# hwaranlee/kaldi-cnn

Measured on AMD Instinct MI355X. Metric: frames/sec fwd+bwd, Conv+Maxpool+FC stack, 4096-frame batch @1/2/4/8 GPU, higher is better.
Workload: dtype f32; 1 GPU; c2: Conv(40x11x3, 8x1, 128) -> Maxpool(1x1x4) -> FC(11616->1024), fwd+bwd+update; frames_per_gpu=4096, parallelism=dp1, global_batch=4096, conv_maxpool_fusion=True, conv_output_stored=False

## Files before the change

### experiments/fc_shapes.py

```python
import os, sys
ROOT = os.path.dirname(os.path.dirname(os.path.abspath(__file__)))
sys.path.insert(0, os.path.join(ROOT, "kaldi-cnn_amd"))
import torch
import kcnn

SHAPES = [("fwd", 4096, 1024, 11616, False, True),
          ("dgrad", 4096, 11616, 1024, False, False),
          ("wgrad", 1024, 11616, 4096, True, False)]


def main():
    calls = int(sys.argv[1]) if len(sys.argv) > 1 else 20
    kcnn.init(0)
    kcnn.set_gemm_mode(2)
    g = torch.Generator(device="cuda").manual_seed(5)
    for name, m, n, k, ta, tb in SHAPES:
        a = torch.randn((k, m) if ta else (m, k), device="cuda", generator=g)
        b = torch.randn((n, k) if tb else (k, n), device="cuda", generator=g) * 0.01
        c = torch.zeros(m, n, device="cuda")
        for _ in range(3):
            kcnn.gemm(a, b, c, ta, tb)
        torch.cuda.synchronize()
        e0, e1 = torch.cuda.Event(enable_timing=True), torch.cuda.Event(enable_timing=True)
        e0.record()
        for _ in range(calls):
            kcnn.gemm(a, b, c, ta, tb)
        e1.record()
        torch.cuda.synchronize()
        us = e0.elapsed_time(e1) * 1e3 / calls
        print(f"{name} {m}x{n}x{k}: {us:.1f} us per call, "
              f"{2 * m * n * k / us / 1e6:.1f} TFLOP/s", flush=True)


if __name__ == "__main__":
    main()
```

### include/kcnn.h

```cpp
#ifndef KCNN_KCNN_H_
#define KCNN_KCNN_H_

#include <stddef.h>
#include <stdint.h>

#include "cnsl-hip-kernels.h"

#ifdef __cplusplus
extern "C" {
#endif

const char *kcnn_last_error(void);
const char *kcnn_version(void);
unsigned long long kcnn_device_malloc_calls(void);
int kcnn_conv_fix_counts(unsigned long long *out, int reset);
int kcnn_init(int device);
int kcnn_set_stream(kcnn_stream_t stream);
int kcnn_synchronize(void);
int kcnn_set_literal_path(int literal);
int kcnn_set_profiling(int on);
int kcnn_set_fusion(int mode);
int kcnn_set_gemm_mode(int mode);
int kcnn_set_kernel_family(const char *name, int value);
int kcnn_get_kernel_family(const char *name);
int kcnn_gemm(int trans_a, int trans_b, int m, int n, int k, float alpha,
              const float *a, int lda, const float *b, int ldb, float beta,
              float *c, int ldc);
int kcnn_split_planes(const float *src, int rows, int cols, int ld, uint16_t *dst, int ldp,
                      int64_t ps);
int kcnn_gemm_planes(int trans_a, int trans_b, int m, int n, int k, float alpha,
                     const uint16_t *a, int lda, int64_t aps, const uint16_t *b, int ldb,
                     int64_t bps, float beta, float *c, int ldc);
int kcnn_profile_string(char *buf, size_t len);
int kcnn_reset_profile(void);
void kcnn_set_randn_seed(uint64_t seed);
int kcnn_selftest_fastdiv(void);

int kcnn_mat_conv2d(const float *in, MatrixDim in_dim, const float *kernel,
                    MatrixDim kernel_dim, int in_height, int in_width,
                    int in_channel, int kernel_height, int kernel_width,
                    int group, float *out, MatrixDim out_dim, int concat);
int kcnn_mat_add_mat_rep_vec(float *m, MatrixDim dim, const float *vec,
                             int vec_dim, int rep);
int kcnn_mat_flip_mat(const float *m, MatrixDim dim, int kernel_height,
                      int kernel_width, int in_channel, int group, float *flip,
                      MatrixDim flip_dim);
int kcnn_mat_padding_zero(const float *m, MatrixDim dim, int orig_height,
                          int orig_width, int orig_channel, int kernel_height,
                          int kernel_width, float *padmat, MatrixDim pad_dim);
int kcnn_mat_tp_block(const float *m, MatrixDim dim, int in_channel,
                      int block_size, float *out, MatrixDim out_dim);
int kcnn_mat_tp_inside_block(const float *m, MatrixDim dim, int group,
                             int block_size, float *out, MatrixDim out_dim);
int kcnn_mat_mod_permute_row(const float *m, MatrixDim dim, int in_channel,
                             int block_size, float *out, MatrixDim out_dim);
int kcnn_mat_mod_permute_channel(float *comp, MatrixDim dim, int comp_idx,
                                 int num_component, int in_height, int in_width,
                                 float *container, MatrixDim container_dim,
                                 int from_comp_to_container);
int kcnn_mat_maxpool_prop(const float *in, MatrixDim in_dim, int in_height,
                          int in_width, int pool_height_dim,
                          int pool_width_dim, int pool_channel_dim,
                          int overlap, int overlap2D, float *out,
                          MatrixDim out_dim);
int kcnn_mat_maxpool_backprop(const float *in_value, MatrixDim in_dim,
                              const float *out_value, MatrixDim ov_dim,
                              const float *out_deriv, MatrixDim od_dim,
                              float *in_deriv, MatrixDim id_dim, int in_height,
                              int in_width, int pool_height_dim,
                              int pool_width_dim, int pool_channel_dim,
                              int overlap, int overlap2D);

typedef struct kcnn_component kcnn_component;

kcnn_component *kcnn_component_new_from_string(const char *initializer_line);
kcnn_component *kcnn_component_read(const char *path);
int kcnn_component_write(const kcnn_component *c, const char *path, int binary);
kcnn_component *kcnn_component_copy(const kcnn_component *c);
void kcnn_component_free(kcnn_component *c);
int kcnn_component_type(const kcnn_component *c, char *buf, size_t len);
int kcnn_component_info(const kcnn_component *c, char *buf, size_t len);
int kcnn_component_input_dim(const kcnn_component *c);
int kcnn_component_output_dim(const kcnn_component *c);
int kcnn_component_context(const kcnn_component *c, int *offsets, int max_len);
int kcnn_component_nonlinear_stats(const kcnn_component *c, double *value_sum,
                                   double *deriv_sum, int max_len, int *len,
                                   double *count);
int kcnn_component_backprop_needs_input(const kcnn_component *c);
int kcnn_component_backprop_needs_output(const kcnn_component *c);
int kcnn_component_propagate(const kcnn_component *c, const float *in,
                             MatrixDim in_dim, float *out, MatrixDim out_dim,
                             int num_chunks);
int kcnn_component_backprop(kcnn_component *c, const float *in_value,
                            MatrixDim in_dim, const float *out_value,
                            MatrixDim ov_dim, const float *out_deriv,
                            MatrixDim od_dim, float *in_deriv,
                            MatrixDim id_dim, int num_chunks, int update);
int kcnn_component_param_dim(const kcnn_component *c, int which, int *rows,
                             int *cols);
int kcnn_component_get_param(const kcnn_component *c, int which, float *dst,
                             MatrixDim dst_dim);
int kcnn_component_set_param(kcnn_component *c, int which, const float *src,
                             MatrixDim src_dim);
float kcnn_component_learning_rate(const kcnn_component *c);
int kcnn_component_set_learning_rate(kcnn_component *c, float lr);
int kcnn_component_dot_product(const kcnn_component *a, const kcnn_component *b,
                               float *out);
int kcnn_component_set_zero(kcnn_component *c, int treat_as_gradient);
int kcnn_component_scale(kcnn_component *c, float scale);
int kcnn_component_add(kcnn_component *c, float alpha,
                       const kcnn_component *other);
int kcnn_component_perturb_params(kcnn_component *c, float stddev);
int kcnn_component_num_gradient_params(const kcnn_component *c);
int kcnn_component_compute_gradient(const kcnn_component *c,
                                    const float *in_value, MatrixDim in_dim,
                                    const float *out_deriv, MatrixDim od_dim,
                                    float *grad);
int kcnn_component_apply_gradient(kcnn_component *c, const float *grad,
                                  int num_sample);
int kcnn_component_backprop_gradient(const kcnn_component *c,
                                     const float *in_value, MatrixDim in_dim,
                                     const float *out_deriv, MatrixDim od_dim,
                                     float *in_deriv, MatrixDim id_dim,
                                     float *grad);
int kcnn_component_conv_flip_branch(const kcnn_component *c);
int kcnn_component_set_dropout_scale(kcnn_component *c, float scale);
int kcnn_component_dropout_seed(const kcnn_component *c, uint64_t *seed);
int kcnn_component_set_dropout_seed(kcnn_component *c, uint64_t seed);

int kcnn_comp_objf_and_deriv(const int32_t *rows, const int32_t *cols, const float *weights,
                             int num, const float *probs, MatrixDim p_dim, float *deriv,
                             MatrixDim d_dim, double *tot_objf, double *tot_weight);

int kcnn_comp_objf_accuracy(const int32_t *rows, const int32_t *cols, const float *weights,
                            int num, const float *probs, MatrixDim p_dim, double out[3]);

typedef struct kcnn_nnet kcnn_nnet;
kcnn_nnet *kcnn_nnet_new(const char *config);
kcnn_nnet *kcnn_nnet_read(const char *path);
int kcnn_nnet_write(const kcnn_nnet *n, const char *path, int binary);
kcnn_nnet *kcnn_nnet_copy(const kcnn_nnet *n, const float *scales, int num_scales,
                          int remove_dropout);
void kcnn_nnet_free(kcnn_nnet *n);
int kcnn_nnet_num_components(const kcnn_nnet *n);
kcnn_component *kcnn_nnet_component(kcnn_nnet *n, int i);
int kcnn_nnet_propagate(kcnn_nnet *n, const float *in, MatrixDim in_dim);
int kcnn_nnet_output(const kcnn_nnet *n, int i, const float **data,
                     MatrixDim *dim);
int kcnn_nnet_input_deriv(const kcnn_nnet *n, int i, const float **data,
                          MatrixDim *dim);
int kcnn_nnet_backprop_component(kcnn_nnet *n, int i, const float *out_deriv,
                                 MatrixDim od_dim, int mode, float *grad,
                                 int skip_first_dx);
int kcnn_nnet_backprop_split(kcnn_nnet *n, int i, const float *out_deriv, MatrixDim od_dim,
                             float *grad, int skip_first_dx, void (*between)(void *),
                             void *ctx);
int kcnn_nnet_backprop(kcnn_nnet *n, const float *out_deriv, MatrixDim od_dim);
int kcnn_nnet_backprop_xent(kcnn_nnet *n, const int32_t *rows, const int32_t *cols,
                            const float *weights, int num, int skip_first_dx);
int kcnn_nnet_objf_total(kcnn_nnet *n, double *out, int reset);
int kcnn_nnet_compute_prob(kcnn_nnet *n, const float *in, MatrixDim in_dim,
                           const int32_t *rows, const int32_t *cols,
                           const float *weights, int num);
int kcnn_nnet_prob_total(kcnn_nnet *n, double out[3], int reset);

int kcnn_nnet_left_context(const kcnn_nnet *n);
int kcnn_nnet_right_context(const kcnn_nnet *n);
int kcnn_nnet_compute(kcnn_nnet *n, const float *in, MatrixDim in_dim, const int32_t *lengths,
                      int num_utts, int pad_input, const float *priors, int num_priors,
                      float prior_scale, int apply_log, const float **data, MatrixDim *dim);

#ifdef __cplusplus
}
#endif
#endif
```

### kaldi-cnn_amd/kcnn.py

```python
from __future__ import annotations

import ctypes
import os

_HERE = os.path.dirname(os.path.abspath(__file__))
LIB_PATH = os.environ.get("KCNN_LIB") or os.path.join(_HERE, "libkcnn.so")
INCLUDE_DIR = os.path.join(os.path.dirname(_HERE), "include")


class KcnnError(RuntimeError):
    """A KALDI_ASSERT / KALDI_ERR / HIP error raised inside libkcnn.so."""


class MatrixDim(ctypes.Structure):
    _fields_ = [("rows", ctypes.c_int32), ("cols", ctypes.c_int32),
                ("stride", ctypes.c_int32)]

    def __repr__(self):
        return f"MatrixDim({self.rows}, {self.cols}, {self.stride})"


_lib = None


def lib():
    global _lib
    if _lib is None:
        import torch
        if not os.path.exists(LIB_PATH):
            raise KcnnError(f"{LIB_PATH} not built (run `make -C kaldi-cnn_amd` "
                            "or __graft_entry__.build())")
        L = ctypes.CDLL(LIB_PATH)
        L.kcnn_last_error.restype = ctypes.c_char_p
        L.kcnn_version.restype = ctypes.c_char_p
        if hasattr(L, "kcnn_device_malloc_calls"):
            L.kcnn_device_malloc_calls.restype = ctypes.c_ulonglong
        for name in ("kcnn_component_new_from_string", "kcnn_component_read",
                     "kcnn_component_copy"):
            getattr(L, name).restype = ctypes.c_void_p
        L.kcnn_component_new_from_string.argtypes = [ctypes.c_char_p]
        L.kcnn_component_read.argtypes = [ctypes.c_char_p]
        L.kcnn_component_copy.argtypes = [ctypes.c_void_p]
        L.kcnn_component_free.argtypes = [ctypes.c_void_p]
        L.kcnn_component_learning_rate.restype = ctypes.c_float
        L.kcnn_nnet_new.restype = ctypes.c_void_p
        L.kcnn_nnet_new.argtypes = [ctypes.c_char_p]
        if hasattr(L, "kcnn_nnet_read"):
            L.kcnn_nnet_read.restype = ctypes.c_void_p
            L.kcnn_nnet_read.argtypes = [ctypes.c_char_p]
            L.kcnn_nnet_write.argtypes = [ctypes.c_void_p, ctypes.c_char_p, ctypes.c_int]
            L.kcnn_nnet_copy.restype = ctypes.c_void_p
            L.kcnn_nnet_copy.argtypes = [ctypes.c_void_p, ctypes.c_void_p, ctypes.c_int,
                                         ctypes.c_int]
        L.kcnn_nnet_free.argtypes = [ctypes.c_void_p]
        L.kcnn_nnet_component.restype = ctypes.c_void_p
        L.kcnn_nnet_component.argtypes = [ctypes.c_void_p, ctypes.c_int]
        L.kcnn_set_stream.argtypes = [ctypes.c_void_p]
        L.kcnn_set_randn_seed.argtypes = [ctypes.c_uint64]
        _lib = L
    return _lib


def check(rc):
    if rc != 0:
        raise KcnnError(lib().kcnn_last_error().decode(errors="replace"))
    return rc


def declared_symbols():
    import re
    names = []
    for fn in sorted(os.listdir(INCLUDE_DIR)):
        if not fn.endswith(".h"):
            continue
        src = open(os.path.join(INCLUDE_DIR, fn)).read()
        src = re.sub(r"/\*.*?\*/", "", src, flags=re.S)
        names += re.findall(r"\b((?:hipF|kcnn)_[A-Za-z0-9_]+)\s*\(", src)
    return sorted(set(names))


_initialized_device = None


def init(device: int = 0):
    global _initialized_device
    import torch
    if not torch.cuda.is_available():
        raise KcnnError("no GPU: the kcnn product path has no CPU fallback")
    torch.cuda.set_device(device)
    check(lib().kcnn_init(device))
    sync_stream()
    _initialized_device = device


def sync_stream():
    import torch
    check(lib().kcnn_set_stream(ctypes.c_void_p(torch.cuda.current_stream().cuda_stream)))


def _ensure_init():
    if _initialized_device is None:
        import torch
        init(torch.cuda.current_device() if torch.cuda.is_available() else 0)


def set_literal_path(on: bool):
    check(lib().kcnn_set_literal_path(int(bool(on))))


def set_profiling(on: bool):
    check(lib().kcnn_set_profiling(int(bool(on))))


def set_fusion(mode):
    check(lib().kcnn_set_fusion(int(mode)))


def device_malloc_calls() -> int:
    return int(lib().kcnn_device_malloc_calls())


def conv_fix_counts(reset=False):
    if not hasattr(lib(), "kcnn_conv_fix_counts"):
        return None
    out = (ctypes.c_ulonglong * 3)()
    check(lib().kcnn_conv_fix_counts(out, int(bool(reset))))
    return tuple(int(v) for v in out)


def profile_string() -> str:
    buf = ctypes.create_string_buffer(1 << 16)
    check(lib().kcnn_profile_string(buf, len(buf)))
    return buf.value.decode()


def set_gemm_mode(mode: int):
    check(lib().kcnn_set_gemm_mode(int(mode)))


def set_kernel_family(name: str, value: int):
    check(lib().kcnn_set_kernel_family(name.encode(), int(value)))


def get_kernel_family(name: str) -> int:
    v = lib().kcnn_get_kernel_family(name.encode())
    if v < 0:
        raise KcnnError(f"unknown kernel family {name!r}")
    return v


def gemm(a, b, c, trans_a=False, trans_b=False, alpha=1.0, beta=0.0):
    m, n = c.shape
    am, k = (a.shape[1], a.shape[0]) if trans_a else (a.shape[0], a.shape[1])
    bk, bn = (b.shape[1], b.shape[0]) if trans_b else (b.shape[0], b.shape[1])
    if am != m or bk != k or bn != n:
        raise KcnnError(f"gemm: op(a) {am}x{k}, op(b) {bk}x{bn} do not make c {m}x{n}")
    for t in (a, b, c):
        dim(t)
    check(lib().kcnn_gemm(int(bool(trans_a)), int(bool(trans_b)), m, n, k,
                          ctypes.c_float(alpha), ctypes.c_void_p(a.data_ptr()), a.stride(0),
                          ctypes.c_void_p(b.data_ptr()), b.stride(0), ctypes.c_float(beta),
                          ctypes.c_void_p(c.data_ptr()), c.stride(0)))


def split_planes(x):
    import torch
    rows, cols = x.shape
    ldp = (cols + 7) // 8 * 8
    out = torch.zeros((3, rows, ldp), dtype=torch.int16, device=x.device)
    check(lib().kcnn_split_planes(ctypes.c_void_p(x.data_ptr()), rows, cols, x.stride(0),
                                  ctypes.c_void_p(out.data_ptr()), ldp,
                                  ctypes.c_int64(rows * ldp)))
    return out


def gemm_planes(ap, bp, c, k, trans_a=False, trans_b=False, alpha=1.0, beta=0.0):
    m, n = c.shape
    check(lib().kcnn_gemm_planes(int(bool(trans_a)), int(bool(trans_b)), m, n, k,
                                 ctypes.c_float(alpha), ctypes.c_void_p(ap.data_ptr()),
                                 ap.stride(1), ctypes.c_int64(ap.stride(0)),
                                 ctypes.c_void_p(bp.data_ptr()), bp.stride(1),
                                 ctypes.c_int64(bp.stride(0)), ctypes.c_float(beta),
                                 ctypes.c_void_p(c.data_ptr()), c.stride(0)))


def reset_profile():
    check(lib().kcnn_reset_profile())


def set_randn_seed(seed: int):
    lib().kcnn_set_randn_seed(ctypes.c_uint64(seed))


def synchronize():
    check(lib().kcnn_synchronize())


def dim(t) -> MatrixDim:
    assert t.dim() == 2, "matrices are 2-D"
    assert t.dtype.is_floating_point and t.element_size() == 4, t.dtype
    assert t.is_cuda, "device tensors only"
    assert t.shape[1] <= 1 or t.stride(1) == 1, "rows must be contiguous"
    stride = t.stride(0) if t.shape[0] > 1 else max(t.shape[1], 1)
    return MatrixDim(t.shape[0], t.shape[1], stride)


def ptr(t):
    return ctypes.c_void_p(t.data_ptr()) if t is not None else None


def empty(rows, cols, device=None):
    import torch
    return torch.empty((rows, cols), dtype=torch.float32,
                       device=device or "cuda")


def zeros(rows, cols, device=None):
    import torch
    return torch.zeros((rows, cols), dtype=torch.float32,
                       device=device or "cuda")



def Conv2D(this, kernel, in_height, in_width, in_channel, kernel_height,
           kernel_width, group, out=None, concat=True):
    _ensure_init()
    oh, ow = in_height - kernel_height + 1, in_width - kernel_width + 1
    if out is None:
        out = (empty(this.shape[0], oh * ow * group) if concat
               else empty(oh * ow * this.shape[0], group))
    check(lib().kcnn_mat_conv2d(ptr(this), dim(this), ptr(kernel), dim(kernel),
                                in_height, in_width, in_channel, kernel_height,
                                kernel_width, group, ptr(out), dim(out),
                                int(concat)))
    return out


def AddMatRepVec(this, vec, rep):
    _ensure_init()
    check(lib().kcnn_mat_add_mat_rep_vec(ptr(this), dim(this), ptr(vec),
                                         vec.numel(), rep))
    return this


def FlipMat(this, kernel_height, kernel_width, in_channel, group, flip=None):
    _ensure_init()
    if flip is None:
        flip = zeros(kernel_height * kernel_width * group, in_channel)
    check(lib().kcnn_mat_flip_mat(ptr(this), dim(this), kernel_height,
                                  kernel_width, in_channel, group, ptr(flip),
                                  dim(flip)))
    return flip


def PaddingZero(this, orig_height, orig_width, orig_channel, kernel_height,
                kernel_width, padmat=None):
    _ensure_init()
    ph, pw = orig_height + 2 * (kernel_height - 1), orig_width + 2 * (kernel_width - 1)
    if padmat is None:
        padmat = zeros(this.shape[0], ph * pw * orig_channel)
    check(lib().kcnn_mat_padding_zero(ptr(this), dim(this), orig_height,
                                      orig_width, orig_channel, kernel_height,
                                      kernel_width, ptr(padmat), dim(padmat)))
    return padmat


def TpBlock(this, in_channel, block_size, out=None):
    _ensure_init()
    if out is None:
        out = zeros(in_channel, this.shape[0] * block_size)
    check(lib().kcnn_mat_tp_block(ptr(this), dim(this), in_channel, block_size,
                                  ptr(out), dim(out)))
    return out


def TpInsideBlock(this, group, block_size, out=None):
    _ensure_init()
    if out is None:
        out = zeros(block_size * this.shape[0], group)
    check(lib().kcnn_mat_tp_inside_block(ptr(this), dim(this), group,
                                         block_size, ptr(out), dim(out)))
    return out


def ModPermuteRow(this, in_channel, block_size, out=None):
    _ensure_init()
    if out is None:
        out = zeros(this.shape[0], this.shape[1])
    check(lib().kcnn_mat_mod_permute_row(ptr(this), dim(this), in_channel,
                                         block_size, ptr(out), dim(out)))
    return out


def ModPermuteChannel(this, comp_idx, num_component, in_height, in_width,
                      container, from_comp_to_container):
    _ensure_init()
    check(lib().kcnn_mat_mod_permute_channel(
        ptr(this), dim(this), comp_idx, num_component, in_height, in_width,
        ptr(container), dim(container), int(bool(from_comp_to_container))))
    return container if from_comp_to_container else this


def Maxpool_prop(this, in_height, in_width, pool_height_dim, pool_width_dim,
                 pool_channel_dim, overlap, overlap2D, out):
    _ensure_init()
    check(lib().kcnn_mat_maxpool_prop(ptr(this), dim(this), in_height, in_width,
                                      pool_height_dim, pool_width_dim,
                                      pool_channel_dim, int(overlap),
                                      int(overlap2D), ptr(out), dim(out)))
    return out


def Maxpool_backprop(this, out_value, out_deriv, in_deriv, in_height, in_width,
                     pool_height_dim, pool_width_dim, pool_channel_dim,
                     overlap=False, overlap2D=False):
    _ensure_init()
    check(lib().kcnn_mat_maxpool_backprop(
        ptr(this), dim(this), ptr(out_value), dim(out_value), ptr(out_deriv),
        dim(out_deriv), ptr(in_deriv), dim(in_deriv), in_height, in_width,
        pool_height_dim, pool_width_dim, pool_channel_dim, int(overlap),
        int(overlap2D)))
    return in_deriv



PARAM_LINEAR, PARAM_BIAS, PARAM_PREV_GRAD = 0, 1, 2


class Component:

    def __init__(self, handle, owned=True, keep=None):
        if not handle:
            raise KcnnError(lib().kcnn_last_error().decode(errors="replace"))
        self._h = ctypes.c_void_p(handle)
        self._owned = owned
        self._keep = keep

    @classmethod
    def NewFromString(cls, initializer_line: str) -> "Component":
        _ensure_init()
        return cls(lib().kcnn_component_new_from_string(initializer_line.encode()))

    @classmethod
    def ReadNew(cls, path: str) -> "Component":
        _ensure_init()
        return cls(lib().kcnn_component_read(str(path).encode()))

    def Write(self, path: str, binary: bool = True):
        check(lib().kcnn_component_write(self._h, str(path).encode(), int(binary)))

    def Copy(self) -> "Component":
        return Component(lib().kcnn_component_copy(self._h))

    def __del__(self):
        try:
            if getattr(self, "_owned", False) and self._h:
                lib().kcnn_component_free(self._h)
                self._h = None
        except Exception:
            pass

    def _str(self, fn) -> str:
        buf = ctypes.create_string_buffer(4096)
        check(fn(self._h, buf, len(buf)))
        return buf.value.decode()

    def SplitGradient(self) -> bool:
        return self.Type() != "ConvolutionComponent"

    def Type(self) -> str:
        return self._str(lib().kcnn_component_type)

    def Info(self) -> str:
        return self._str(lib().kcnn_component_info)

    def InputDim(self) -> int:
        return lib().kcnn_component_input_dim(self._h)

    def OutputDim(self) -> int:
        return lib().kcnn_component_output_dim(self._h)

    def BackpropNeedsInput(self) -> bool:
        return bool(lib().kcnn_component_backprop_needs_input(self._h))

    def BackpropNeedsOutput(self) -> bool:
        return bool(lib().kcnn_component_backprop_needs_output(self._h))

    def Context(self):
        buf = (ctypes.c_int * 256)()
        n = lib().kcnn_component_context(self._h, buf, 256)
        if n < 0:
            check(1)
        return list(buf[:n])

    def _span(self):
        ctx = self.Context()
        return ctx[-1] - ctx[0]

    def Propagate(self, inp, out=None, num_chunks=None):
        span = self._span()
        if num_chunks is None:
            num_chunks = inp.shape[0] // (span + 1)
        if out is None:
            out = empty(inp.shape[0] - num_chunks * span, self.OutputDim())
        check(lib().kcnn_component_propagate(self._h, ptr(inp), dim(inp),
                                             ptr(out), dim(out), num_chunks))
        return out

    def NonlinearStats(self):
        import numpy as np
        n = self.InputDim()
        vs, ds = np.zeros(n, np.float64), np.zeros(n, np.float64)
        cnt = ctypes.c_double()
        k = ctypes.c_int()
        check(lib().kcnn_component_nonlinear_stats(
            self._h, vs.ctypes.data_as(ctypes.c_void_p), ds.ctypes.data_as(ctypes.c_void_p),
            n, ctypes.byref(k), ctypes.byref(cnt)))
        return vs[:k.value], ds[:k.value], cnt.value

    def Backprop(self, in_value, out_value, out_deriv, in_deriv=None,
                 update=True, num_chunks=None, need_in_deriv=True):
        span = self._span()
        if num_chunks is None:
            num_chunks = out_deriv.shape[0]
        if in_deriv is None and need_in_deriv:
            in_deriv = empty(out_deriv.shape[0] + num_chunks * span, self.InputDim())
        if out_value is None:
            out_value = out_deriv
        if in_value is None:
            in_value = in_deriv if in_deriv is not None else out_deriv
        idim = dim(in_deriv) if in_deriv is not None else MatrixDim(0, 0, 0)
        check(lib().kcnn_component_backprop(
            self._h, ptr(in_value), dim(in_value), ptr(out_value),
            dim(out_value), ptr(out_deriv), dim(out_deriv), ptr(in_deriv), idim,
            num_chunks, int(update)))
        return in_deriv

    def ParamDim(self, which):
        r, c = ctypes.c_int(), ctypes.c_int()
        check(lib().kcnn_component_param_dim(self._h, which, ctypes.byref(r),
                                             ctypes.byref(c)))
        return r.value, c.value
# ... 295 lines not shown
```

### kaldi-cnn_amd/src/capi/kcnn-capi.cc

```cpp
#include "kcnn.h"

#include <stdlib.h>
#include <string.h>

#include <algorithm>
#include <fstream>
#include <sstream>
#include <string>
#include <utility>
#include <vector>

#include "../cnslmat/hip-util.h"
#include "../kaldi-lite/cu-device.h"
#include "../kaldi-lite/cu-kernels-lite.h"
#include "../kaldi-lite/cu-matrix.h"
#include "../kaldi-lite/kaldi-io.h"
#include "../nnet0/nnet-component-nnet0.h"
#include "../nnet2/nnet-component.h"
#include "../nnet2/nnet-kernels.h"
#include "nnet-stack.h"
#include "xent-labels.h"

using namespace kaldi;
using namespace kaldi::nnet2;

struct kcnn_nnet {
  kcnn::NnetStack stack;
  template <typename... Args>
  explicit kcnn_nnet(Args &&...args) : stack(std::forward<Args>(args)...) {}
};

namespace {
thread_local std::string g_err;

int fail(const char *what) {
  g_err = what;
  return -1;
}

template <typename F>
int guard(F f) {
  try {
    f();
    return 0;
  } catch (const std::exception &e) {
    return fail(e.what());
  } catch (...) {
    return fail("unknown C++ exception");
  }
}

CuSubMatrix<BaseFloat> view(const float *p, MatrixDim d) {
  return CuSubMatrix<BaseFloat>(const_cast<float *>(p), d.rows, d.cols, d.stride);
}

void borrow(CuMatrix<BaseFloat> *m, const float *p, MatrixDim d) {
  m->Borrow(const_cast<float *>(p), d.rows, d.cols, d.stride);
}

ChunkInfo chunk_info(int cols, int rows, int num_chunks) {
  if (num_chunks <= 0) num_chunks = rows;
  KALDI_ASSERT(rows > 0 && rows % num_chunks == 0);
  return ChunkInfo(cols, num_chunks, 0, rows / num_chunks - 1);
}

void component_chunks(const Component *c, MatrixDim in_dim, MatrixDim out_dim,
                      int num_chunks, ChunkInfo *ii, ChunkInfo *oi) {
  const std::vector<int32> ctx = c->Context();
  if (num_chunks <= 0) num_chunks = out_dim.rows;
  KALDI_ASSERT(out_dim.rows > 0 && out_dim.rows % num_chunks == 0 &&
               in_dim.rows % num_chunks == 0);
  const int ocs = out_dim.rows / num_chunks;
  KALDI_ASSERT(in_dim.rows / num_chunks == ocs + ctx.back() - ctx.front());
  *oi = ChunkInfo(out_dim.cols, num_chunks, 0, ocs - 1);
  if (ctx.front() == 0 && ctx.back() == 0) {
    *ii = ChunkInfo(in_dim.cols, num_chunks, 0, ocs - 1);
  } else {
    *oi = ChunkInfo(out_dim.cols, num_chunks, -ctx.front(), ocs - 1 - ctx.front());
    *ii = ChunkInfo(in_dim.cols, num_chunks, 0, ocs - 1 + ctx.back() - ctx.front());
  }
}

void copy_out(std::string s, char *buf, size_t len) {
  if (!buf || !len) return;
  strncpy(buf, s.c_str(), len - 1);
  buf[len - 1] = '\0';
}

UpdatableComponent *updatable(const kcnn_component *c) {
  KALDI_ASSERT(c && c->c);
  UpdatableComponent *u = dynamic_cast<UpdatableComponent *>(c->c);
  if (!u) KALDI_ERR << c->c->Type() << " has no parameters";
  return u;
}

void param_ref(const kcnn_component *c, int which, float **data, MatrixDim *dim) {
  using cnsl::nnet0::ConvolutionComponent;
  using cnsl::nnet0::FullyConnectedComponent;
  CuMatrixBase<BaseFloat> *m = nullptr;
  CuVectorBase<BaseFloat> *v = nullptr;
  if (auto *cc = dynamic_cast<ConvolutionComponent *>(c->c)) {
    if (which == 0) m = &cc->LinearParamsMutable();
    else if (which == 1) v = &cc->BiasParamsMutable();
    else if (which == 2) m = &cc->PrevGradMutable();
  } else if (auto *fc = dynamic_cast<FullyConnectedComponent *>(c->c)) {
    if (which == 0) m = &fc->LinearParamsMutable();
    else if (which == 1) v = &fc->BiasParamsMutable();
    else if (which == 2) m = &fc->PrevGradMutable();
  } else if (auto *af = dynamic_cast<AffineComponent *>(c->c)) {
    if (which == 0) m = &af->LinearParamsMutable();
    else if (which == 1) v = &af->BiasParamsMutable();
  }
  if (m) {
    *data = m->Data();
    *dim = m->Dim();
  } else if (v) {
    *data = v->Data();
    dim->rows = 1; dim->cols = v->Dim(); dim->stride = v->Dim();
  } else {
    KALDI_ERR << c->c->Type() << " has no parameter #" << which;
  }
}

void copy2d(float *dst, MatrixDim dd, const float *src, MatrixDim sd) {
  KALDI_ASSERT(dd.rows == sd.rows && dd.cols == sd.cols);
  if (dd.rows == 0 || dd.cols == 0) return;
  CU_SAFE_CALL(hipMemcpy2DAsync(dst, sizeof(float) * dd.stride, src,
                                sizeof(float) * sd.stride,
                                sizeof(float) * dd.cols, dd.rows,
                                hipMemcpyDeviceToDevice,
                                CuDevice::Instantiate().Stream()));
}

kcnn::NnetStack &stack(const kcnn_nnet *n) { return const_cast<kcnn_nnet *>(n)->stack; }

void matrix_out(const CuMatrix<BaseFloat> &m, const float **data, MatrixDim *dim) {
  *data = m.Data();
  *dim = m.Dim();
}
}

extern "C" {

const char *kcnn_last_error(void) { return g_err.c_str(); }
const char *kcnn_version(void) { return "kcnn-mi355x 0.1 (gfx950)"; }
unsigned long long kcnn_device_malloc_calls(void) {
  return (unsigned long long)CuDevice::Instantiate().MallocCalls();
}

int kcnn_init(int device) {
  return guard([&] { CuDevice::Instantiate().SelectGpuId("yes", device); });
}
int kcnn_set_stream(kcnn_stream_t stream) {
  return guard([&] {
    CuDevice::Instantiate().SetStream(reinterpret_cast<hipStream_t>(stream));
  });
}
int kcnn_synchronize(void) {
  return guard([&] { CuDevice::Instantiate().Synchronize(); });
}
int kcnn_set_literal_path(int literal) {
  cnsl::nnet0::SetLiteralPath(literal != 0);
  return 0;
}
int kcnn_set_fusion(int on) {
  if (on < 0 || on > 2) return fail("kcnn_set_fusion: mode is 0, 1 or 2");
  kcnn::set_fusion_mode(on);
  return 0;
}
int kcnn_set_gemm_mode(int mode) {
  if (mode < 0 || mode > 2) return fail("kcnn_set_gemm_mode: mode is 0, 1 or 2");
  CuDevice::Instantiate().SetGemmMode(mode);
  return 0;
}
int kcnn_set_kernel_family(const char *name, int value) {
  const int f = kcnn::family_by_name(name);
  if (f < 0) return fail("kcnn_set_kernel_family: unknown family");
  if (kcnn::set_family(static_cast<kcnn::Family>(f), value) != 0)
    return fail("kcnn_set_kernel_family: value out of range");
  return 0;
}
int kcnn_get_kernel_family(const char *name) {
  const int f = kcnn::family_by_name(name);
  return f < 0 ? -1 : kcnn::family(static_cast<kcnn::Family>(f));
}
int kcnn_gemm(int trans_a, int trans_b, int m, int n, int k, float alpha,
              const float *a, int lda, const float *b, int ldb, float beta,
              float *c, int ldc) {
  return guard([&] {
    if (m < 0 || n < 0 || k < 0) KALDI_ERR << "kcnn_gemm: negative dimension";
    const int ar = trans_a ? k : m, ac = trans_a ? m : k;
    const int br = trans_b ? n : k, bc = trans_b ? k : n;
    if (lda < ac || ldb < bc || ldc < n) KALDI_ERR << "kcnn_gemm: leading dimension too small";
    CuSubMatrix<BaseFloat> A(const_cast<float *>(a), ar, ac, lda);
    CuSubMatrix<BaseFloat> B(const_cast<float *>(b), br, bc, ldb);
    CuSubMatrix<BaseFloat> C(c, m, n, ldc);
    C.AddMatMat(alpha, A, trans_a ? kTrans : kNoTrans, B, trans_b ? kTrans : kNoTrans, beta);
  });
}
int kcnn_split_planes(const float *src, int rows, int cols, int ld, uint16_t *dst, int ldp,
                      int64_t ps) {
  return guard([&] {
    CuDevice &d = CuDevice::Instantiate();
    const int rc = kl_split_planes(src, rows, cols, ld, dst, ldp, ps,
                                   reinterpret_cast<kcnn_stream_t>(d.Stream()));
    if (rc) KALDI_ERR << "kcnn_split_planes: " << hipGetErrorString((hipError_t)rc);
  });
}
int kcnn_gemm_planes(int trans_a, int trans_b, int m, int n, int k, float alpha,
                     const uint16_t *a, int lda, int64_t aps, const uint16_t *b, int ldb,
                     int64_t bps, float beta, float *c, int ldc) {
  return guard([&] {
    CuDevice &d = CuDevice::Instantiate();
    const size_t wsb = kl_gemm_planes_workspace_bytes(m, n, k);
    CuScratch ws_s(wsb);
    void *ws = ws_s.p;
    const int rc = kl_gemm_planes(trans_a, trans_b, m, n, k, alpha, a, lda, aps, b, ldb, bps,
                                  beta, c, ldc, ws, wsb,
                                  reinterpret_cast<kcnn_stream_t>(d.Stream()));
    if (rc) KALDI_ERR << "kcnn_gemm_planes: " << hipGetErrorString((hipError_t)rc);
  });
}
int kcnn_set_profiling(int on) {
  CuDevice::Instantiate().SetProfiling(on != 0);
  return 0;
}
int kcnn_profile_string(char *buf, size_t len) {
  return guard([&] { copy_out(CuDevice::Instantiate().ProfileString(), buf, len); });
}
int kcnn_reset_profile(void) {
  return guard([&] {
    CuDevice &d = CuDevice::Instantiate();
    (void)d.ProfileString();
    d.ResetProfile();
  });
}
void kcnn_set_randn_seed(uint64_t seed) { SetRandnSeed(seed); }

int kcnn_selftest_fastdiv(void) {
  const uint32_t divs[] = {1, 2, 3, 5, 7, 8, 11, 24, 33, 40, 128, 363, 440,
                           1320, 11616, 46464, 65535, 1000003, 0x7fffffffu};
  uint64_t state = 12345;
  for (uint32_t d : divs) {
    kcnn::FastDiv f(d);
    for (int t = 0; t < 20000; t++) {
      state = state * 6364136223846793005ull + 1442695040888963407ull;
      uint32_t n = (uint32_t)(state >> 33);
      if (t < 64) n = (uint32_t)t;
      if (t >= 64 && t < 128) n = 0x7fffffffu - (uint32_t)(t - 64);
      uint32_t q, r;
      f.divmod(n, q, r);
      if (q != n / d || r != n % d) {
        std::ostringstream ss;
        ss << "FastDiv(" << d << ") failed at n=" << n << ": " << q << "," << r;
        return fail(ss.str().c_str());
      }
    }
  }
  return 0;
}

int kcnn_mat_conv2d(const float *in, MatrixDim in_dim, const float *kernel,
                    MatrixDim kernel_dim, int in_height, int in_width,
                    int in_channel, int kernel_height, int kernel_width,
                    int group, float *out, MatrixDim out_dim, int concat) {
  return guard([&] {
    auto x = view(in, in_dim), k = view(kernel, kernel_dim), o = view(out, out_dim);
    x.Conv2D(k, in_height, in_width, in_channel, kernel_height, kernel_width,
             group, &o, concat != 0);
  });
}
int kcnn_mat_add_mat_rep_vec(float *m, MatrixDim dim, const float *vec,
                             int vec_dim, int rep) {
  return guard([&] {
    auto x = view(m, dim);
    CuSubVector<BaseFloat> v(const_cast<float *>(vec), vec_dim);
    x.AddMatRepVec(v, rep);
  });
}
int kcnn_mat_flip_mat(const float *m, MatrixDim dim, int kernel_height,
                      int kernel_width, int in_channel, int group, float *flip,
                      MatrixDim flip_dim) {
  return guard([&] {
    auto x = view(m, dim);
    CuMatrix<BaseFloat> f;
    borrow(&f, flip, flip_dim);
    x.FlipMat(kernel_height, kernel_width, in_channel, group, &f);
  });
}
int kcnn_mat_padding_zero(const float *m, MatrixDim dim, int orig_height,
                          int orig_width, int orig_channel, int kernel_height,
                          int kernel_width, float *padmat, MatrixDim pad_dim) {
  return guard([&] {
    auto x = view(m, dim);
    CuMatrix<BaseFloat> p;
    borrow(&p, padmat, pad_dim);
    x.PaddingZero(orig_height, orig_width, orig_channel, kernel_height,
                  kernel_width, &p);
  });
}
int kcnn_mat_tp_block(const float *m, MatrixDim dim, int in_channel,
                      int block_size, float *out, MatrixDim out_dim) {
  return guard([&] {
    auto x = view(m, dim);
    CuMatrix<BaseFloat> o;
    borrow(&o, out, out_dim);
    x.TpBlock(in_channel, block_size, &o);
  });
}
int kcnn_mat_tp_inside_block(const float *m, MatrixDim dim, int group,
                             int block_size, float *out, MatrixDim out_dim) {
  return guard([&] {
    auto x = view(m, dim);
    CuMatrix<BaseFloat> o;
    borrow(&o, out, out_dim);
    x.TpInsideBlock(group, block_size, &o);
  });
}
int kcnn_mat_mod_permute_channel(float *comp, MatrixDim dim, int comp_idx,
                                 int num_component, int in_height, int in_width,
                                 float *container, MatrixDim container_dim,
                                 int from_comp_to_container) {
  return guard([&] {
    auto c = view(comp, dim);
    auto k = view(container, container_dim);
    c.ModPermuteChannel(comp_idx, num_component, in_height, in_width, &k,
                        from_comp_to_container != 0);
  });
}
int kcnn_mat_mod_permute_row(const float *m, MatrixDim dim, int in_channel,
                             int block_size, float *out, MatrixDim out_dim) {
  return guard([&] {
    auto x = view(m, dim);
    CuMatrix<BaseFloat> o;
    borrow(&o, out, out_dim);
    x.ModPermuteRow(in_channel, block_size, &o);
  });
}
int kcnn_mat_maxpool_prop(const float *in, MatrixDim in_dim, int in_height,
                          int in_width, int pool_height_dim, int pool_width_dim,
                          int pool_channel_dim, int overlap, int overlap2D,
                          float *out, MatrixDim out_dim) {
  return guard([&] {
    auto x = view(in, in_dim), o = view(out, out_dim);
    x.Maxpool_prop(in_height, in_width, pool_height_dim, pool_width_dim,
                   pool_channel_dim, overlap != 0, overlap2D != 0, &o);
  });
}
int kcnn_mat_maxpool_backprop(const float *in_value, MatrixDim in_dim,
                              const float *out_value, MatrixDim ov_dim,
                              const float *out_deriv, MatrixDim od_dim,
                              float *in_deriv, MatrixDim id_dim, int in_height,
                              int in_width, int pool_height_dim,
                              int pool_width_dim, int pool_channel_dim,
                              int overlap, int overlap2D) {
  return guard([&] {
    auto x = view(in_value, in_dim), y = view(out_value, ov_dim),
         dy = view(out_deriv, od_dim);
    CuMatrix<BaseFloat> dx;
    borrow(&dx, in_deriv, id_dim);
    x.Maxpool_backprop(y, dy, &dx, in_height, in_width, pool_height_dim,
                       pool_width_dim, pool_channel_dim, overlap != 0,
                       overlap2D != 0);
  });
}

kcnn_component *kcnn_component_new_from_string(const char *line) {
  kcnn_component *h = nullptr;
  guard([&] { h = new kcnn_component{Component::NewFromString(line)}; });
  return h;
}
kcnn_component *kcnn_component_read(const char *path) {
  kcnn_component *h = nullptr;
  guard([&] {
    std::ifstream is(path, std::ios::binary);
    if (!is) KALDI_ERR << "cannot open " << path;
    bool binary = false;
    if (!InitKaldiInputStream(is, &binary)) KALDI_ERR << "bad Kaldi header in " << path;
    h = new kcnn_component{Component::ReadNew(is, binary)};
  });
  return h;
}
int kcnn_component_write(const kcnn_component *c, const char *path, int binary) {
  return guard([&] {
    std::ofstream os(path, std::ios::binary);
    if (!os) KALDI_ERR << "cannot open " << path << " for writing";
    InitKaldiOutputStream(os, binary != 0);
    c->c->Write(os, binary != 0);
    if (!os) KALDI_ERR << "write failed: " << path;
  });
}
kcnn_component *kcnn_component_copy(const kcnn_component *c) {
  kcnn_component *h = nullptr;
  guard([&] { h = new kcnn_component{c->c->Copy()}; });
  return h;
}
void kcnn_component_free(kcnn_component *c) {
  if (!c) return;
  delete c->c;
  delete c;
}
int kcnn_component_type(const kcnn_component *c, char *buf, size_t len) {
  return guard([&] { copy_out(c->c->Type(), buf, len); });
}
int kcnn_component_info(const kcnn_component *c, char *buf, size_t len) {
  return guard([&] { copy_out(c->c->Info(), buf, len); });
}
int kcnn_component_input_dim(const kcnn_component *c) { return c->c->InputDim(); }
int kcnn_component_output_dim(const kcnn_component *c) { return c->c->OutputDim(); }
int kcnn_component_context(const kcnn_component *c, int *offsets, int max_len) {
  int n = -1;
  guard([&] {
    const std::vector<int32> ctx = c->c->Context();
    n = (int)ctx.size();
    for (int k = 0; k < n && k < max_len; k++) offsets[k] = ctx[k];
  });
  return n;
}
int kcnn_component_nonlinear_stats(const kcnn_component *c, double *value_sum,
                                   double *deriv_sum, int max_len, int *len,
                                   double *count) {
  return guard([&] {
    auto *nl = dynamic_cast<const kaldi::nnet2::NonlinearComponent *>(c->c);
    if (!nl) KALDI_ERR << c->c->Type() << " is not a NonlinearComponent";
    Vector<double> v, d;
    nl->GetValueSum(&v);
    nl->GetDerivSum(&d);
    *len = v.Dim();
    for (int k = 0; k < v.Dim() && k < max_len; k++) {
      value_sum[k] = v(k);
      deriv_sum[k] = d(k);
    }
    *count = nl->Count();
  });
}
int kcnn_component_backprop_needs_input(const kcnn_component *c) {
  return c->c->BackpropNeedsInput();
}
int kcnn_component_backprop_needs_output(const kcnn_component *c) {
  return c->c->BackpropNeedsOutput();
}

int kcnn_component_propagate(const kcnn_component *c, const float *in,
                             MatrixDim in_dim, float *out, MatrixDim out_dim,
                             int num_chunks) {
  return guard([&] {
    auto x = view(in, in_dim), y = view(out, out_dim);
    ChunkInfo ii, oi;
    component_chunks(c->c, in_dim, out_dim, num_chunks, &ii, &oi);
    c->c->Propagate(ii, oi, x, &y);
  });
}

int kcnn_component_backprop(kcnn_component *c, const float *in_value,
                            MatrixDim in_dim, const float *out_value,
                            MatrixDim ov_dim, const float *out_deriv,
                            MatrixDim od_dim, float *in_deriv,
                            MatrixDim id_dim, int num_chunks, int update) {
  return guard([&] {
    auto x = view(in_value, in_dim), y = view(out_value, ov_dim),
         dy = view(out_deriv, od_dim);
    ChunkInfo ii, oi;
    component_chunks(c->c, in_dim, od_dim, num_chunks, &ii, &oi);
    CuMatrix<BaseFloat> dx;
    if (in_deriv) borrow(&dx, in_deriv, id_dim);
    Component *to_update = update ? c->c : nullptr;
    c->c->Backprop(ii, oi, x, y, dy, to_update, in_deriv ? &dx : nullptr);
  });
}

int kcnn_component_param_dim(const kcnn_component *c, int which, int *rows,
                             int *cols) {
  return guard([&] {
    float *p;
    MatrixDim d;
// ... 269 lines not shown
```

### kaldi-cnn_amd/src/kaldi-lite/cu-gemm-f16x3.hip

```cpp
#include <atomic>
#include <hip/hip_runtime.h>
#include <stdint.h>

#include <algorithm>
#include <mutex>
#include <type_traits>

#include "cnslmat/f16-split.h"
#include "cnslmat/hip-util.h"
#include "cnslmat/momentum-step.h"
#include "cnslmat/pool-stats-dev.h"
#include "cnslmat/pool-stats.h"
#include "kaldi-lite/cu-kernels-lite.h"

namespace {

using kcnn::COLMAX_ROWS;
using kcnn::PoolCountSmem;
using kcnn::pool_colmax_block;
using kcnn::pool_count_block;
using kcnn::f16x3::f16x8;
using kcnn::f16x3::f32x16;
using kcnn::f16x3::NONFINITE;
using kcnn::f16x3::SKIP;
using kcnn::f16x3::scale_exp;
using kcnn::f16x3::split2h;
using kcnn::f16x3::mfma;
typedef short s16x4 __attribute__((ext_vector_type(4)));
typedef short s16x8 __attribute__((ext_vector_type(8)));
typedef __attribute__((address_space(3))) s16x4 lds_s16x4;

constexpr int BM = 256, BN = 128, BK = 32, NT = 512;
constexpr int ROWB = BK * 2;
constexpr int A_PLANE = BM * ROWB;
constexpr int B_PLANE = BN * ROWB;
constexpr int BUF = 2 * (A_PLANE + B_PLANE);
constexpr int LDS_BYTES = 2 * BUF + (BM + BN) * 8;

struct GemmF16Args {
  const float *A, *B;
  float *C;
  float *part;
  uint32_t *rflag;
  uint32_t gen;
  const uint32_t *amax, *bmax;
  const uint32_t *amin, *bmin;
  const uint32_t *acnt, *bcnt;
  const float *bias;
  int M, N, K, lda, ldb, ldc;
  int bvec;
  MomentumEpi mom;
  int kps, ksplit, tiles_m, tiles_n;
  int nwhole;
  int fix_local;
  uint32_t *fix_report;
  float alpha, beta;
};

constexpr int GM = 4;
__device__ __forceinline__ void tile_rc(const GemmF16Args &p, int t, int &tm, int &tn) {
  const int gsz = GM * p.tiles_n;
  const int g = t / gsz, r = t - g * gsz;
  const int m0 = g * GM;
  const int gm = min(p.tiles_m - m0, GM);
  tm = m0 + r % gm;
  tn = r / gm;
}
__device__ __forceinline__ int tile_index(const GemmF16Args &p, int tm, int tn) {
  const int g = tm / GM, m0 = g * GM;
  const int gm = min(p.tiles_m - m0, GM);
  return g * GM * p.tiles_n + tn * gm + (tm - m0);
}
__device__ __forceinline__ bool block_tile(const GemmF16Args &p, int &split, int &tm, int &tn) {
  const bool whole = (int)blockIdx.x < p.nwhole;
  const int b = whole ? (int)blockIdx.x : (int)blockIdx.x - p.nwhole;
  const int nb = whole ? p.nwhole : (int)gridDim.x - p.nwhole;
  const int ks = whole ? 1 : p.ksplit;
  const int xcd = b & 7, q = nb >> 3, rr = nb & 7;
  const int lid = (xcd < rr ? xcd * (q + 1) : rr * (q + 1) + (xcd - rr) * q) + (b >> 3);
  split = lid % ks;
  tile_rc(p, (whole ? 0 : p.nwhole) + lid / ks, tm, tn);
  return whole;
}
__device__ __forceinline__ bool in_split_tile(const GemmF16Args &p, int r, int c) {
  return p.nwhole == 0 || tile_index(p, r / BM, c / BN) >= p.nwhole;
}

__device__ __forceinline__ int swz(int r, int c) {
  return r * ROWB + ((c ^ ((r >> 2) & 3)) << 4);
}
template <int R>
__device__ __forceinline__ int tswz(int k, int col) {
  return k * (R * 2) + ((((col >> 3) ^ ((k & 3) << 2))) << 4) + ((col & 7) << 1);
}

enum { LK = 0, LR = 1, LT = 2 };

template <int R, int MODE>
struct Loader {
  static constexpr int KPT = MODE == LK ? 8 : MODE == LR ? R * BK / NT : R * BK / (NT * 4);
  static constexpr int UNITS = MODE == LK ? R * 4 : MODE == LR ? R * BK / KPT : NT;
  static constexpr int UPT = (UNITS + NT - 1) / NT;
  static constexpr int NE = MODE == LT ? 4 : UPT;
  static_assert(UNITS % NT == 0, "tile shape");
  static_assert(MODE != LR || KPT % 8 == 0, "tile shape");
  static_assert(MODE != LT || (R / 4) * (BK / KPT) == NT, "tile shape");
  static constexpr int NV = MODE == LT ? 4 * KPT : KPT;
  float v[UPT][NV];
  int e[NE];

  __device__ static __forceinline__ int row_of(int i, int tid) {
    if constexpr (MODE == LT) return 4 * (tid % (R / 4)) + i;
    const int unit = tid + i * NT;
    return MODE == LK ? unit >> 2 : unit % R;
  }
  __device__ __forceinline__ void init_exp(const int *sexp, int tid) {
#pragma unroll
    for (int i = 0; i < NE; ++i) {
      const int s = sexp[row_of(i, tid)];
      e[i] = s == SKIP ? 0 : s;
    }
  }

  __device__ __forceinline__ void load(__amdgpu_buffer_rsrc_t rs, int ld, int vrows, int kk,
                                       int tid) {
    constexpr unsigned OOB = 0x80000000u;
#pragma unroll
    for (int u = 0; u < UPT; ++u) {
      const int unit = tid + u * NT;
      if constexpr (MODE == LK) {
        const int r = unit >> 2, k = kk + (unit & 3) * 8;
        const unsigned off = r < vrows ? (unsigned)(r * ld + k) * 4u : OOB;
        const auto a = __builtin_amdgcn_raw_buffer_load_b128(rs, off, 0, 0);
        const auto b = __builtin_amdgcn_raw_buffer_load_b128(rs, off + 16u, 0, 0);
#pragma unroll
        for (int j = 0; j < 4; ++j) {
          v[u][j] = __uint_as_float(a[j]);
          v[u][4 + j] = __uint_as_float(b[j]);
        }
      } else if constexpr (MODE == LR) {
        const int r = unit % R, k = kk + (unit / R) * KPT;
#pragma unroll
        for (int j = 0; j < KPT; ++j) {
          const unsigned off = r < vrows ? (unsigned)((k + j) * ld + r) * 4u : OOB;
          v[u][j] = __uint_as_float(__builtin_amdgcn_raw_buffer_load_b32(rs, off, 0, 0));
        }
      } else {
        const int rq = unit % (R / 4), k = kk + (unit / (R / 4)) * KPT;
#pragma unroll
        for (int j = 0; j < KPT; ++j) {
          const unsigned off = 4 * rq < vrows ? (unsigned)((k + j) * ld + 4 * rq) * 4u : OOB;
          const auto a = __builtin_amdgcn_raw_buffer_load_b128(rs, off, 0, 0);
#pragma unroll
          for (int i = 0; i < 4; ++i) v[u][4 * j + i] = __uint_as_float(a[i]);
        }
      }
    }
  }

  template <int PL, bool RAG>
  __device__ __forceinline__ void store(char *lds, int tid, int kv, float m1) const {
#pragma unroll
    for (int u = 0; u < UPT; ++u) {
      const int unit = tid + u * NT;
      float x[NV];
#pragma unroll
      for (int j = 0; j < NV; ++j) x[j] = v[u][j];
      if constexpr (MODE == LT) {
        const int rq = unit % (R / 4), kq = unit / (R / 4);
        if (RAG && kv < BK) {
#pragma unroll
          for (int j = 0; j < KPT; ++j)
            if (kq * KPT + j >= kv)
#pragma unroll
              for (int i = 0; i < 4; ++i) x[4 * j + i] = 0.0f;
        }
#pragma unroll
        for (int j = 0; j < KPT; ++j) {
          uint32_t h0, l0, h1, l1;
          split2h(x[4 * j], x[4 * j + 1], e[0], e[1], h0, l0, m1);
          split2h(x[4 * j + 2], x[4 * j + 3], e[2], e[3], h1, l1, m1);
          const int o = tswz<R>(kq * KPT + j, 4 * rq);
          *reinterpret_cast<uint2 *>(lds + o) = make_uint2(h0, h1);
          *reinterpret_cast<uint2 *>(lds + PL + o) = make_uint2(l0, l1);
        }
      } else {
        int r, c0, kb;
        if constexpr (MODE == LK) {
          r = unit >> 2;
          c0 = unit & 3;
          kb = c0 * 8;
        } else {
          r = unit % R;
          c0 = (unit / R) * (KPT / 8);
          kb = (unit / R) * KPT;
        }
        if (RAG && kv < BK) {
#pragma unroll
          for (int j = 0; j < KPT; ++j)
            if (kb + j >= kv) x[j] = 0.0f;
        }
#pragma unroll
        for (int cc = 0; cc < KPT / 8; ++cc) {
          uint32_t h[4], l[4];
#pragma unroll
          for (int i = 0; i < 4; ++i)
            split2h(x[cc * 8 + 2 * i], x[cc * 8 + 2 * i + 1], e[u], e[u], h[i], l[i], m1);
          const int off = swz(r, c0 + cc);
          *reinterpret_cast<uint4 *>(lds + off) = make_uint4(h[0], h[1], h[2], h[3]);
          *reinterpret_cast<uint4 *>(lds + PL + off) = make_uint4(l[0], l[1], l[2], l[3]);
        }
      }
    }
  }

  static constexpr int NPIECE = MODE == LT ? 2 * KPT : UPT * (KPT / 2);
  template <int PL, bool RAG>
  __device__ __forceinline__ void piece(char *lds, int tid, int pc, int kv, uint32_t (&ph)[4],
                                        uint32_t (&pl)[4], float m1) const {
    if constexpr (MODE == LT) {
      const int j = pc >> 1, hf = pc & 1;
      const int unit = tid;
      const int rq = unit % (R / 4), kq = unit / (R / 4);
      float x0 = v[0][4 * j + 2 * hf], x1 = v[0][4 * j + 2 * hf + 1];
      if (RAG && kv < BK) {
        asm volatile("");
        if (kq * KPT + j >= kv) x0 = x1 = 0.0f;
      }
      split2h(x0, x1, e[2 * hf], e[2 * hf + 1], ph[hf], pl[hf], m1);
      if (hf == 1) {
        const int o = tswz<R>(kq * KPT + j, 4 * rq);
        *reinterpret_cast<uint2 *>(lds + o) = make_uint2(ph[0], ph[1]);
        *reinterpret_cast<uint2 *>(lds + PL + o) = make_uint2(pl[0], pl[1]);
      }
    } else {
      constexpr int PPU = KPT / 2;
      const int u = pc / PPU, q = pc % PPU;
      const int unit = tid + u * NT;
      int r, c0, kb;
      if constexpr (MODE == LK) {
        r = unit >> 2;
        c0 = unit & 3;
        kb = c0 * 8;
      } else {
        r = unit % R;
        c0 = (unit / R) * (KPT / 8);
        kb = (unit / R) * KPT;
      }
      float x0 = v[u][2 * q], x1 = v[u][2 * q + 1];
      if (RAG && kv < BK) {
        asm volatile("");
        if (kb + 2 * q >= kv) x0 = 0.0f;
        if (kb + 2 * q + 1 >= kv) x1 = 0.0f;
      }
      split2h(x0, x1, e[u], e[u], ph[q & 3], pl[q & 3], m1);
      if ((q & 3) == 3) {
        const int off = swz(r, c0 + (q >> 2));
        *reinterpret_cast<uint4 *>(lds + off) = make_uint4(ph[0], ph[1], ph[2], ph[3]);
        *reinterpret_cast<uint4 *>(lds + PL + off) = make_uint4(pl[0], pl[1], pl[2], pl[3]);
      }
    }
  }
  static constexpr int NRD = MODE == LT ? 2 : 1;

  __device__ static __forceinline__ f16x8 frag(const char *plane, int rb, int s, int lane) {
    if constexpr (MODE != LT) {
      return *reinterpret_cast<const f16x8 *>(plane + swz(rb + (lane & 31), 2 * s + (lane >> 5)));
    } else {
      const int g = lane >> 4, q = (lane >> 2) & 3, pp = lane & 3;
      const int k = 16 * s + 8 * (g >> 1) + q;
      const int col = rb + 16 * (g & 1) + 4 * pp;
      const s16x4 lo = __builtin_amdgcn_ds_read_tr16_b64_v4i16(
          (lds_s16x4 *)(plane + tswz<R>(k, col)));
      const s16x4 hi = __builtin_amdgcn_ds_read_tr16_b64_v4i16(
          (lds_s16x4 *)(plane + tswz<R>(k + 4, col)));
      const s16x8 c = __builtin_shufflevector(lo, hi, 0, 1, 2, 3, 4, 5, 6, 7);
      return __builtin_bit_cast(f16x8, c);
    }
  }
};


__device__ __forceinline__ int tile_scales(const GemmF16Args &p, int *sexp, float *sw, int row0,
                                           int col0, int tid) {
  int skip = 0, spr = 0;
  for (int i = tid; i < BM + BN; i += NT) {
    int s = 0;
    float w = 0.0f;
    if (i < BM) {
      if (row0 + i < p.M) {
        const uint32_t m = p.amax[row0 + i];
        s = scale_exp(m);
        w = m == 0 ? -__builtin_inff() : kcnn::f16x3::spread_weight(p.acnt[row0 + i]);
      }
    } else if (col0 + i - BM < p.N) {
      const uint32_t m = p.bmax[col0 + i - BM];
      s = scale_exp(m);
      w = m == 0 ? -__builtin_inff() : kcnn::f16x3::spread_weight(p.bcnt[col0 + i - BM]);
    }
    sexp[i] = s;
    sw[i] = w;
    skip |= s == SKIP;
    spr |= w > 0.0f;
  }
  const int any_skip = __syncthreads_or(skip) != 0;
  return any_skip | (__syncthreads_or(spr) != 0 ? 2 : 0);
}

__device__ __forceinline__ float wave_dot(const GemmF16Args &p, bool a_kc, bool b_kc, int row,
                                          int col, int lane) {
  const int64_t sa = a_kc ? 1 : p.lda, sb = b_kc ? 1 : p.ldb;
  const float *qa = (a_kc ? p.A + (int64_t)row * p.lda : p.A + row) + lane * sa;
  const float *qb = (b_kc ? p.B + (int64_t)col * p.ldb : p.B + col) + lane * sb;
  const int64_t da = 64 * sa, db = 64 * sb;
  float s[4] = {0.0f, 0.0f, 0.0f, 0.0f};
  int k = lane;
#pragma unroll 1
  for (; k + 192 < p.K; k += 256) {
    float x[4], y[4];
#pragma unroll
    for (int j = 0; j < 4; ++j) {
      x[j] = qa[j * da];
      y[j] = qb[j * db];
    }
#pragma unroll
    for (int j = 0; j < 4; ++j) s[j] = fmaf(x[j], y[j], s[j]);
    qa += 4 * da;
    qb += 4 * db;
  }
#pragma unroll 1
  for (; k < p.K; k += 64) {
    s[0] = fmaf(*qa, *qb, s[0]);
    qa += da;
    qb += db;
  }
  float t = (s[0] + s[1]) + (s[2] + s[3]);
#pragma unroll
  for (int d = 32; d >= 1; d >>= 1) t += __shfl_xor(t, d);
  return t;
}
__device__ __forceinline__ float store_value(const GemmF16Args &p, float v, float *o, int col) {
  float r = p.beta == 0.0f ? p.alpha * v : p.alpha * v + p.beta * *o;
  if (p.bias) r += p.bias[col];
  return r;
}
__device__ __forceinline__ void emit(const GemmF16Args &p, int row, int col, float v) {
  if (p.mom.W) {
    float *w = p.mom.W + (int64_t)row * p.mom.ldw + col;
    float *q = p.mom.prev + (int64_t)row * p.mom.ldp + col;
    float wv = *w, pv = *q;
    kcnn::momentum_step(p.alpha * v, pv, wv, p.mom.momentum, p.mom.a_wd, p.mom.a_g);
    *q = pv;
    *w = wv;
    return;
  }
  float *o = p.C + (int64_t)row * p.ldc + col;
  *o = store_value(p, v, o, col);
}
template <typename Decode, typename Put>
__device__ __forceinline__ void fix_rejected(const GemmF16Args &p, bool a_kc, bool b_kc,
                                             uint64_t mine, int lane, Decode decode, Put put) {
  for (;;) {
    const uint64_t who = __ballot(mine != 0);
    if (who == 0) break;
    const int l = __builtin_ctzll(who);
    const uint32_t lo = __builtin_amdgcn_readlane((uint32_t)mine, l);
    const uint32_t hi = __builtin_amdgcn_readlane((uint32_t)(mine >> 32), l);
    const uint64_t bits = ((uint64_t)hi << 32) | lo;
    const int n = __builtin_ctzll(bits);
    int row, col;
    decode(l, n, row, col);
    const float v = wave_dot(p, a_kc, b_kc, row, col, lane);
    if (lane == 0) put(l, n, row, col, v);
    if (lane == l) mine &= mine - 1;
  }
}
template <typename Decode>
__device__ __forceinline__ void fix_rejected(const GemmF16Args &p, bool a_kc, bool b_kc,
                                             uint64_t mine, int lane, Decode decode) {
  fix_rejected(p, a_kc, b_kc, mine, lane, decode,
               [&](int, int, int row, int col, float v) { emit(p, row, col, v); });
}

template <bool A_KC, bool B_KC>
__device__ __forceinline__ void tile_epilogue(const GemmF16Args &p, const int *sexp,
                                              const float *sw, const f32x16 (&acc)[2][2],
                                              int split, bool whole, int row0, int col0,
                                              int flags, int tid, char *lds) {
  const int lane = tid & 63, wave = tid >> 6, wm = wave >> 1, wn = wave & 1;
  const int half2 = lane >> 5;
  const bool partial = p.ksplit > 1 && !whole;
  const bool skip = flags & 1;
  const bool check = (flags & 2) && !partial;
  const int np4 = (p.N + 3) & ~3;
  float *slab = partial ? p.part + (int64_t)split * p.M * np4 : p.C;
  const int ldo = partial ? np4 : p.ldc;
  uint64_t rej = 0;
  auto fix = [&]() {
    fix_rejected(p, A_KC, B_KC, rej, lane, [&](int l, int n, int &row, int &col) {
      const int i = n >> 5, j = (n >> 4) & 1, g = n & 15;
      row = row0 + wm * 64 + i * 32 + (g & 3) + 8 * (g >> 2) + 4 * (l >> 5);
      col = col0 + wn * 64 + j * 32 + (l & 31);
    });
  };
  const bool staged = row0 + BM <= p.M && col0 + BN <= p.N && !skip &&
                      (partial || p.mom.W || ((ldo & 3) | ((uintptr_t)slab & 15)) == 0);
  if (staged) {
    __syncthreads();
    constexpr int SR = 68;
    float *st = reinterpret_cast<float *>(lds) + wave * 32 * SR;
#pragma unroll
    for (int i = 0; i < 2; ++i) {
#pragma unroll
      for (int j = 0; j < 2; ++j) {
        const int cl = wn * 64 + j * 32 + (lane & 31);
        const int ec = sexp[BM + cl];
        const float wc = check ? sw[BM + cl] : 0.0f;
        const bool bcheck =
            check && (__ballot(wc > 0.0f || sw[wm * 64 + i * 32 + (lane & 31)] > 0.0f) != 0);
#pragma unroll
        for (int g = 0; g < 16; ++g) {
          const int rr = (g & 3) + 8 * (g >> 2) + 4 * half2;
          const int rl = wm * 64 + i * 32 + rr;
          if (bcheck) {
            const float thr = wc + sw[rl];
            if (thr != 0.0f && !(fabsf(acc[i][j][g]) >= thr))
              rej |= (uint64_t)1 << ((2 * i + j) * 16 + g);
          }
          st[rr * SR + j * 32 + (lane & 31)] =
              __builtin_amdgcn_ldexpf(acc[i][j][g], -(sexp[rl] + ec));
        }
      }
      if (check) {
        const uint64_t mine = (rej >> (32 * i)) & 0xffffffffull;
        fix_rejected(
            p, A_KC, B_KC, mine, lane,
            [&](int l, int n, int &row, int &col) {
              const int j = (n >> 4) & 1, g = n & 15;
              row = row0 + wm * 64 + i * 32 + (g & 3) + 8 * (g >> 2) + 4 * (l >> 5);
              col = col0 + wn * 64 + j * 32 + (l & 31);
            },
            [&](int l, int n, int, int, float v) {
              const int j = (n >> 4) & 1, g = n & 15;
              const int rr = (g & 3) + 8 * (g >> 2) + 4 * (l >> 5);
              st[rr * SR + j * 32 + (l & 31)] = v;
            });
      }
#pragma unroll
      for (int k = 0; k < 8; ++k) {
        const int f = lane + 64 * k, rr = f >> 4, c4 = f & 15;
        const float4 v = *reinterpret_cast<const float4 *>(st + rr * SR + 4 * c4);
        const int row = row0 + wm * 64 + i * 32 + rr, col = col0 + wn * 64 + 4 * c4;
        if (!partial && p.mom.W) {
          float4 *wq = reinterpret_cast<float4 *>(p.mom.W + (int64_t)row * p.mom.ldw + col);
          float4 *pq = reinterpret_cast<float4 *>(p.mom.prev + (int64_t)row * p.mom.ldp + col);
          float4 w4 = *wq, q4 = *pq;
          const MomentumEpi &m = p.mom;
          kcnn::momentum_step(p.alpha * v.x, q4.x, w4.x, m.momentum, m.a_wd, m.a_g);
          kcnn::momentum_step(p.alpha * v.y, q4.y, w4.y, m.momentum, m.a_wd, m.a_g);
          kcnn::momentum_step(p.alpha * v.z, q4.z, w4.z, m.momentum, m.a_wd, m.a_g);
          kcnn::momentum_step(p.alpha * v.w, q4.w, w4.w, m.momentum, m.a_wd, m.a_g);
          *pq = q4;
          *wq = w4;
          continue;
        }
        float4 *o = reinterpret_cast<float4 *>(slab + (int64_t)row * ldo + col);
        if (partial) {
          *o = v;
          continue;
        }
        float4 w = make_float4(p.alpha * v.x, p.alpha * v.y, p.alpha * v.z, p.alpha * v.w);
        if (p.beta != 0.0f) {
          const float4 c = *o;
          w = make_float4(p.alpha * v.x + p.beta * c.x, p.alpha * v.y + p.beta * c.y,
                          p.alpha * v.z + p.beta * c.z, p.alpha * v.w + p.beta * c.w);
        }
        if (p.bias) {
          w.x += p.bias[col];
          w.y += p.bias[col + 1];
          w.z += p.bias[col + 2];
          w.w += p.bias[col + 3];
        }
        *o = w;
      }
    }
    return;
  }
#pragma unroll
  for (int i = 0; i < 2; ++i)
#pragma unroll
    for (int j = 0; j < 2; ++j) {
      const int cl = wn * 64 + j * 32 + (lane & 31);
      const int col = col0 + cl;
      const int ec = sexp[BM + cl];
      if (col >= p.N || ec == SKIP) continue;
      const float wc = check ? sw[BM + cl] : 0.0f;
      const bool bcheck =
          check && (__ballot(wc > 0.0f || sw[wm * 64 + i * 32 + (lane & 31)] > 0.0f) != 0);
#pragma unroll
      for (int g = 0; g < 16; ++g) {
        const int rl = wm * 64 + i * 32 + (g & 3) + 8 * (g >> 2) + 4 * half2;
        const int row = row0 + rl;
        const int er = sexp[rl];
        if (row >= p.M || er == SKIP) continue;
        if (bcheck) {
          const float thr = wc + sw[rl];
          if (thr != 0.0f && !(fabsf(acc[i][j][g]) >= thr)) {
            rej |= (uint64_t)1 << ((2 * i + j) * 16 + g);
            continue;
          }
        }
        const float v = __builtin_amdgcn_ldexpf(acc[i][j][g], -(er + ec));
        if (partial) slab[(int64_t)row * ldo + col] = v;
        else emit(p, row, col, v);
      }
    }
  if (check) fix();
  if (skip && split == 0) {
    for (int e = tid; e < BM * BN; e += NT) {
      const int rl = e / BN, cl = e - rl * BN;
      const int row = row0 + rl, col = col0 + cl;
      if (row >= p.M || col >= p.N) continue;
      if (sexp[rl] != SKIP && sexp[BM + cl] != SKIP) continue;
      float sum = 0.0f;
      for (int k = 0; k < p.K; ++k) {
        const float a = A_KC ? p.A[(int64_t)row * p.lda + k] : p.A[(int64_t)k * p.lda + row];
        const float b = B_KC ? p.B[(int64_t)col * p.ldb + k] : p.B[(int64_t)k * p.ldb + col];
        sum = fmaf(a, b, sum);
      }
      emit(p, row, col, sum);
    }
  }
}

template <int AM, int BMODE, bool RAG>
__global__ __launch_bounds__(NT, 1) void gemm_f16x3_kernel(GemmF16Args p) {
  constexpr bool A_KC = AM == LK, B_KC = BMODE == LK;
  extern __shared__ __attribute__((aligned(16))) char lds[];
  int *sexp = reinterpret_cast<int *>(lds + 2 * BUF);
  float *sw = reinterpret_cast<float *>(sexp + BM + BN);
  const int tid = threadIdx.x;
  const float m1 = kcnn::f16x3::opaque_m1();
  const int lane = tid & 63, wave = __builtin_amdgcn_readfirstlane(tid >> 6);
  const int wm = wave >> 1, wn = wave & 1;
  int split, tm, tn;
  const bool whole = block_tile(p, split, tm, tn);
  const int row0 = tm * BM, col0 = tn * BN;
  const int kbeg = whole ? 0 : split * p.kps;
  const int kend = whole ? p.K : min(p.K, kbeg + p.kps);
  const int T = kend > kbeg ? (kend - kbeg + BK - 1) / BK : 0;
  const int klast = kend - kbeg - (T - 1) * BK;

  const int flags = tile_scales(p, sexp, sw, row0, col0, tid);

  const float *baseA = A_KC ? p.A + (int64_t)row0 * p.lda : p.A + (int64_t)kbeg * p.lda + row0;
  const float *baseB = B_KC ? p.B + (int64_t)col0 * p.ldb : p.B + (int64_t)kbeg * p.ldb + col0;
  const int vra = p.M - row0, vrb = p.N - col0;
  const int64_t endA = A_KC ? ((int64_t)(vra - 1) * p.lda + p.K) * 4
                            : ((int64_t)(p.K - 1 - kbeg) * p.lda + vra) * 4;
  const int64_t endB = B_KC ? ((int64_t)(vrb - 1) * p.ldb + p.K) * 4
                            : ((int64_t)(p.K - 1 - kbeg) * p.ldb + vrb) * 4;
  const __amdgpu_buffer_rsrc_t rsA = __builtin_amdgcn_make_buffer_rsrc(
      (void *)baseA, (short)0, (int)(endA < 0x7fffffff ? endA : 0x7fffffff), 0x00020000);
  const __amdgpu_buffer_rsrc_t rsB = __builtin_amdgcn_make_buffer_rsrc(
      (void *)baseB, (short)0, (int)(endB < 0x7fffffff ? endB : 0x7fffffff), 0x00020000);
  auto kk = [&](int t, bool kc) { return (kc ? kbeg : 0) + min(t, T - 1) * BK; };

  using LA = Loader<BM, AM>;
  using LB = Loader<BN, BMODE>;
  LA la[2];
  LB lb[2];
  f32x16 acc[2][2];
#pragma unroll
  for (int i = 0; i < 2; ++i)
#pragma unroll
    for (int j = 0; j < 2; ++j)
#pragma unroll
      for (int g = 0; g < 16; ++g) acc[i][j][g] = 0.0f;
  la[0].init_exp(sexp, tid);
  la[1].init_exp(sexp, tid);
  lb[0].init_exp(sexp + BM, tid);
  lb[1].init_exp(sexp + BM, tid);

  if (T > 0) {
    la[0].load(rsA, p.lda, vra, kk(0, A_KC), tid);
    lb[0].load(rsB, p.ldb, vrb, kk(0, B_KC), tid);
    la[0].template store<A_PLANE, RAG>(lds, tid, T == 1 ? klast : BK, m1);
    lb[0].template store<B_PLANE, RAG>(lds + 2 * A_PLANE, tid, T == 1 ? klast : BK, m1);
    __builtin_amdgcn_sched_barrier(0);
    la[1].load(rsA, p.lda, vra, kk(1, A_KC), tid);
    lb[1].load(rsB, p.ldb, vrb, kk(1, B_KC), tid);
    __builtin_amdgcn_sched_barrier(0);
    la[0].load(rsA, p.lda, vra, kk(2, A_KC), tid);
    lb[0].load(rsB, p.ldb, vrb, kk(2, B_KC), tid);
    __syncthreads();

    const int ar = wm * 64, br = wn * 64;
    auto half_step = [&](const char *bufA, int s) {
      const char *bufB = bufA + 2 * A_PLANE;
      f16x8 a[2][2], bb[2][2];
#pragma unroll
      for (int i = 0; i < 2; ++i)
#pragma unroll
        for (int pl = 0; pl < 2; ++pl) {
          a[i][pl] = LA::frag(bufA + pl * A_PLANE, ar + 32 * i, s, lane);
          bb[i][pl] = LB::frag(bufB + pl * B_PLANE, br + 32 * i, s, lane);
        }
#pragma unroll
      for (int i = 0; i < 2; ++i)
#pragma unroll
        for (int j = 0; j < 2; ++j) {
          f32x16 x = acc[i][j];
          x = mfma(a[i][1], bb[j][0], x);
          x = mfma(a[i][0], bb[j][1], x);
          x = mfma(a[i][0], bb[j][0], x);
          acc[i][j] = x;
        }
    };
    const bool late = wave < 4;
    auto step = [&](int t, LA &lan, LB &lbn) {
      if (t < T) {
        const char *buf = lds + (t & 1) * BUF;
        char *nA = lds + ((t + 1) & 1) * BUF;
        const int kv = t + 2 == T ? klast : BK;
        half_step(buf, 0);
        if (!late && t + 1 < T) {
          lan.template store<A_PLANE, RAG>(nA, tid, kv, m1);
          lbn.template store<B_PLANE, RAG>(nA + 2 * A_PLANE, tid, kv, m1);
        }
        half_step(buf, 1);
        if (late && t + 1 < T) {
          lan.template store<A_PLANE, RAG>(nA, tid, kv, m1);
          lbn.template store<B_PLANE, RAG>(nA + 2 * A_PLANE, tid, kv, m1);
        }
      }
      lan.load(rsA, p.lda, vra, kk(t + 3, A_KC), tid);
      lbn.load(rsB, p.ldb, vrb, kk(t + 3, B_KC), tid);
      __syncthreads();
    };
    for (int t = 0; t < T; t += 2) {
      step(t, la[1], lb[1]);
      step(t + 1, la[0], lb[0]);
    }
  }

  tile_epilogue<A_KC, B_KC>(p, sexp, sw, acc, split, whole, row0, col0, flags, tid, lds);
}

template <int AM, int BMODE, bool RAG>
__global__ __launch_bounds__(NT, 1) void gemm_f16x3_fast_kernel(GemmF16Args p) {
  constexpr bool A_KC = AM == LK, B_KC = BMODE == LK;
  extern __shared__ __attribute__((aligned(16))) char lds[];
  int *sexp = reinterpret_cast<int *>(lds + 2 * BUF);
  float *sw = reinterpret_cast<float *>(sexp + BM + BN);
  const int tid = threadIdx.x;
  const float m1 = kcnn::f16x3::opaque_m1();
  const int lane = tid & 63, wave = __builtin_amdgcn_readfirstlane(tid >> 6);
  const int wm = wave >> 1, wn = wave & 1;
  int split, tm, tn;
  const bool whole = block_tile(p, split, tm, tn);
  const int row0 = tm * BM, col0 = tn * BN;
  const int kbeg = whole ? 0 : split * p.kps;
  const int kend = whole ? p.K : min(p.K, kbeg + p.kps);
  const int T = kend > kbeg ? (kend - kbeg + BK - 1) / BK : 0;
  const int klast = kend - kbeg - (T - 1) * BK;

  const float *baseA = A_KC ? p.A + (int64_t)row0 * p.lda : p.A + (int64_t)kbeg * p.lda + row0;
  const float *baseB = B_KC ? p.B + (int64_t)col0 * p.ldb : p.B + (int64_t)kbeg * p.ldb + col0;
  const int vra = p.M - row0, vrb = p.N - col0;
  const int64_t endA = A_KC ? ((int64_t)(vra - 1) * p.lda + p.K) * 4
                            : ((int64_t)(p.K - 1 - kbeg) * p.lda + vra) * 4;
  const int64_t endB = B_KC ? ((int64_t)(vrb - 1) * p.ldb + p.K) * 4
                            : ((int64_t)(p.K - 1 - kbeg) * p.ldb + vrb) * 4;
  const __amdgpu_buffer_rsrc_t rsA = __builtin_amdgcn_make_buffer_rsrc(
      (void *)baseA, (short)0, (int)(endA < 0x7fffffff ? endA : 0x7fffffff), 0x00020000);
  const __amdgpu_buffer_rsrc_t rsB = __builtin_amdgcn_make_buffer_rsrc(
      (void *)baseB, (short)0, (int)(endB < 0x7fffffff ? endB : 0x7fffffff), 0x00020000);
  auto kk = [&](int t, bool kc) { return (kc ? kbeg : 0) + min(t, T - 1) * BK; };

  using LA = Loader<BM, AM>;
  using LB = Loader<BN, BMODE>;
  LA la[2];
  LB lb[2];
  f32x16 acc[2][2];
#pragma unroll
  for (int i = 0; i < 2; ++i)
#pragma unroll
    for (int j = 0; j < 2; ++j)
#pragma unroll
      for (int g = 0; g < 16; ++g) acc[i][j][g] = 0.0f;

  const int ar = wm * 64, br = wn * 64;
  f16x8 fa0[2][2], fb0[2][2], fa1[2][2], fb1[2][2];
  auto read_frag = [&](const char *buf, int s, int r, f16x8 (&fa)[2][2], f16x8 (&fb)[2][2]) {
    if (r < 4) {
      const int i = r >> 1, pl = r & 1;
      fa[i][pl] = LA::frag(buf + pl * A_PLANE, ar + 32 * i, s, lane);
    } else {
      const int i = (r - 4) >> 1, pl = (r - 4) & 1;
      fb[i][pl] = LB::frag(buf + 2 * A_PLANE + pl * B_PLANE, br + 32 * i, s, lane);
    }
  };
  auto mfma_n = [&](int n, const f16x8 (&fa)[2][2], const f16x8 (&fb)[2][2]) {
    const int i = n / 6, j = (n / 3) & 1, pr = n % 3;
    constexpr int PA[3] = {1, 0, 0}, PB[3] = {0, 1, 0};
    acc[i][j] = mfma(fa[i][PA[pr]], fb[j][PB[pr]], acc[i][j]);
  };

  constexpr int PRIO = 1;
  if (PRIO && wave >= 4) __builtin_amdgcn_s_setprio(1);
  if (T > 0) {
    la[0].load(rsA, p.lda, vra, kk(0, A_KC), tid);
    lb[0].load(rsB, p.ldb, vrb, kk(0, B_KC), tid);
    la[1].load(rsA, p.lda, vra, kk(1, A_KC), tid);
    lb[1].load(rsB, p.ldb, vrb, kk(1, B_KC), tid);
  }
  __builtin_amdgcn_sched_barrier(0);
  const int flags = tile_scales(p, sexp, sw, row0, col0, tid);
  la[0].init_exp(sexp, tid);
  la[1].init_exp(sexp, tid);
  lb[0].init_exp(sexp + BM, tid);
  lb[1].init_exp(sexp + BM, tid);
  if (T > 0) {
    la[0].template store<A_PLANE, RAG>(lds, tid, T == 1 ? klast : BK, m1);
    lb[0].template store<B_PLANE, RAG>(lds + 2 * A_PLANE, tid, T == 1 ? klast : BK, m1);
    __builtin_amdgcn_sched_barrier(0);
    la[0].load(rsA, p.lda, vra, kk(2, A_KC), tid);
    lb[0].load(rsB, p.ldb, vrb, kk(2, B_KC), tid);
    __syncthreads();
#pragma unroll
    for (int r = 0; r < 8; ++r) read_frag(lds, 0, r, fa0, fb0);

    auto step = [&](int t, LA &lan, LB &lbn, auto more_c) {
      const char *buf = lds + (t & 1) * BUF;
      char *nbuf = lds + ((t + 1) & 1) * BUF;
      constexpr bool more = decltype(more_c)::value;
      const int kv = t + 2 == T ? klast : BK;
      uint32_t ph[4], pl[4];
#pragma unroll
      for (int n = 0; n < 12; ++n) {
        mfma_n(n, fa0, fb0);
        if (more) {
          if (n < LA::NPIECE)
            lan.template piece<A_PLANE, RAG>(nbuf, tid, n, kv, ph, pl, m1);
          else if (n - LA::NPIECE < LB::NPIECE)
            lbn.template piece<B_PLANE, RAG>(nbuf + 2 * A_PLANE, tid, n - LA::NPIECE, kv, ph, pl, m1);
        }
        if (n >= 2 && n < 10) read_frag(buf, 1, n - 2, fa1, fb1);
        __builtin_amdgcn_sched_barrier(0);
      }
      __syncthreads();
#pragma unroll
      for (int n = 0; n < 12; ++n) {
        mfma_n(n, fa1, fb1);
        if (n == 1) lan.load(rsA, p.lda, vra, kk(t + 3, A_KC), tid);
        if (n == 3) lbn.load(rsB, p.ldb, vrb, kk(t + 3, B_KC), tid);
        if (more && n >= 2 && n < 10) read_frag(nbuf, 0, n - 2, fa0, fb0);
        __builtin_amdgcn_sched_barrier(0);
      }
    };
    int t = 0;
    for (; t + 2 < T; t += 2) {
      step(t, la[1], lb[1], std::true_type{});
      step(t + 1, la[0], lb[0], std::true_type{});
    }
    if (t + 1 < T) {
      step(t, la[1], lb[1], std::true_type{});
      step(t + 1, la[0], lb[0], std::false_type{});
    } else {
      step(t, la[1], lb[1], std::false_type{});
    }
  }

  tile_epilogue<A_KC, B_KC>(p, sexp, sw, acc, split, whole, row0, col0, flags, tid, lds);
}

struct StatOp {
  const float *X;
  uint32_t *out;
  uint32_t *part;
  int rows, cols, ld, mode, vec;
  int blocks;
  int rpb;
  int cb, rbk, rb;
  int fblocks;
  uint32_t *clear;
};
__device__ __forceinline__ const float *X_row(const StatOp &o, int r) {
  return o.X + (int64_t)r * o.ld;
}

__device__ __forceinline__ void mm4(uint32_t &m, uint32_t &n, float4 q) {
  const uint32_t a = __float_as_uint(q.x) & 0x7fffffffu, b = __float_as_uint(q.y) & 0x7fffffffu,
                 c = __float_as_uint(q.z) & 0x7fffffffu, d = __float_as_uint(q.w) & 0x7fffffffu;
  m = max(max(m, a), max(max(b, c), d));
  n = min(min(n, a - 1u), min(min(b - 1u, c - 1u), d - 1u));
}
__device__ __forceinline__ void mm1(uint32_t &m, uint32_t &n, float x) {
  const uint32_t a = __float_as_uint(x) & 0x7fffffffu;
  m = max(m, a);
  n = min(n, a - 1u);
}

__device__ __forceinline__ uint32_t count_small_row(const StatOp &o, const float *x, float bound,
                                                    int c, int step) {
  uint32_t n = 0;
  for (; c < o.cols; c += step)
#pragma unroll
    for (int i = 0; i < 4; ++i)
      if (c + i < o.cols) {
        const float a = fabsf(x[c + i]);
        n += (a < bound && a != 0.0f) ? 1u : 0u;
      }
  return n;
}

constexpr int RV = 18;
__device__ __forceinline__ void stats_rows(const StatOp &o, int blk, uint32_t *red) {
  const int lane = threadIdx.x & 63, wave = threadIdx.x >> 6;
  const bool wide = o.rpb == 1;
  const int r = wide ? blk : blk * 4 + wave;
  if (r >= o.rows) return;
  const float *x = X_row(o, r);
  const int step = wide ? 1024 : 256;
  const int c0 = (wide ? threadIdx.x : lane) * 4;
  const bool held = o.vec && o.cols <= RV * step;
  float4 q[RV];
  uint32_t m = 0, n = 0xffffffffu;
  if (held) {
#pragma unroll
    for (int j = 0; j < RV; ++j) {
      const int c = c0 + j * step;
      if (c + 4 <= o.cols) {
        q[j] = *reinterpret_cast<const float4 *>(x + c);
      } else {
        q[j].x = c < o.cols ? x[c] : 0.0f;
        q[j].y = c + 1 < o.cols ? x[c + 1] : 0.0f;
        q[j].z = c + 2 < o.cols ? x[c + 2] : 0.0f;
        q[j].w = 0.0f;
      }
    }
#pragma unroll
    for (int j = 0; j < RV; ++j) mm4(m, n, q[j]);
  } else {
    int c = c0;
    if (o.vec) {
      for (; c + 3 * step + 4 <= o.cols; c += 4 * step) {
        float4 v[4];
#pragma unroll
        for (int j = 0; j < 4; ++j) v[j] = *reinterpret_cast<const float4 *>(x + c + j * step);
#pragma unroll
        for (int j = 0; j < 4; ++j) mm4(m, n, v[j]);
      }
      for (; c + 4 <= o.cols; c += step) mm4(m, n, *reinterpret_cast<const float4 *>(x + c));
    }
    for (; c < o.cols; c += step)
#pragma unroll
      for (int i = 0; i < 4; ++i)
        if (c + i < o.cols) mm1(m, n, x[c + i]);
  }
#pragma unroll
  for (int d = 32; d >= 1; d >>= 1) {
    m = max(m, (uint32_t)__shfl_xor((int)m, d));
    n = min(n, (uint32_t)__shfl_xor((int)n, d));
  }
  if (wide) {
    if (lane == 0) {
      red[wave] = m;
      red[4 + wave] = n;
    }
    __syncthreads();
    m = max(max(red[0], red[1]), max(red[2], red[3]));
    n = min(min(red[4], red[5]), min(red[6], red[7]));
  }
  uint32_t cnt = 0;
  if (kcnn::f16x3::spread(m, n + 1u)) {
    const float bound = kcnn::f16x3::small_bound(m);
    if (held) {
      auto small = [&](float v) { return (fabsf(v) < bound && v != 0.0f) ? 1u : 0u; };
#pragma unroll
      for (int j = 0; j < RV; ++j)
        cnt += small(q[j].x) + small(q[j].y) + small(q[j].z) + small(q[j].w);
    } else {
      cnt = count_small_row(o, x, bound, c0, step);
    }
#pragma unroll
    for (int d = 32; d >= 1; d >>= 1) cnt += (uint32_t)__shfl_xor((int)cnt, d);
    if (wide) {
      __syncthreads();
      if (lane == 0) red[8 + wave] = cnt;
      __syncthreads();
      cnt = red[8] + red[9] + red[10] + red[11];
    }
  }
  if (wide ? threadIdx.x == 0 : lane == 0) {
    o.out[r] = m;
    o.out[o.rows + r] = n + 1u;
    o.out[2 * (size_t)o.rows + r] = cnt;
  }
}

__device__ __forceinline__ void stats_cols(const StatOp &o, int blk) {
  const int cbi = blk % o.cb, rci = blk / o.cb;
  const int c0 = cbi * 1024 + threadIdx.x * 4;
  const int r0 = rci * o.rb, rend = min(o.rows, r0 + o.rb);
  if (c0 >= o.cols) return;
  const bool v4 = o.vec && c0 + 4 <= o.cols;
  uint32_t cm[4] = {0u, 0u, 0u, 0u};
  uint32_t cn[4] = {0xffffffffu, 0xffffffffu, 0xffffffffu, 0xffffffffu};
  auto load = [&](int r) {
    const float *x = X_row(o, r) + c0;
    if (v4) return *reinterpret_cast<const float4 *>(x);
    float4 q;
    q.x = x[0];
    q.y = c0 + 1 < o.cols ? x[1] : 0.0f;
    q.z = c0 + 2 < o.cols ? x[2] : 0.0f;
    q.w = c0 + 3 < o.cols ? x[3] : 0.0f;
    return q;
  };
  auto take = [&](float4 q) {
    mm1(cm[0], cn[0], q.x);
    mm1(cm[1], cn[1], q.y);
    mm1(cm[2], cn[2], q.z);
    mm1(cm[3], cn[3], q.w);
  };
  int r = r0;
  for (; r + 8 <= rend; r += 8) {
    float4 q[8];
#pragma unroll
    for (int j = 0; j < 8; ++j) q[j] = load(r + j);
#pragma unroll
    for (int j = 0; j < 8; ++j) take(q[j]);
  }
  for (; r < rend; ++r) take(load(r));
  uint32_t *dst = o.part + (size_t)rci * o.cols + c0;
  uint32_t *dsn = dst + (size_t)o.rbk * o.cols;
#pragma unroll
  for (int i = 0; i < 4; ++i)
    if (c0 + i < o.cols) {
      dst[i] = cm[i];
      dsn[i] = cn[i];
    }
}

struct StatOps {
  StatOp o[3];
  PoolColDeferred pc;
  int pcx, pcy, pcn;
};
template <typename Count>
__device__ __forceinline__ int pick_op(const StatOps &s, int blk, Count count, int &local) {
  const int n0 = count(s.o[0]), n1 = count(s.o[1]);
  if (blk < n0) { local = blk; return 0; }
  if (blk < n0 + n1) { local = blk - n0; return 1; }
  local = blk - n0 - n1;
  return 2;
}
__host__ __device__ inline int ncount_blocks(const StatOp &o);
__host__ __device__ inline int nfinal_blocks(const StatOp &o) {
  return o.mode == 1 && o.blocks ? o.fblocks : 0;
}

__global__ __launch_bounds__(256) void stats_kernel(StatOps s) {
  __shared__ uint32_t red[12];
  if (s.o[0].clear && blockIdx.x == 0 && threadIdx.x < 2) s.o[0].clear[threadIdx.x] = 0u;
  const int nb3 = s.o[0].blocks + s.o[1].blocks + s.o[2].blocks;
  if ((int)blockIdx.x >= nb3) {
    const int k = blockIdx.x - nb3;
    pool_colmax_block(s.pc.pcol, s.pc.nblk, s.pc.npool, s.pc.colblk, k % s.pcx, k / s.pcx);
    return;
  }
  int blk;
  const int w = pick_op(s, blockIdx.x, [](const StatOp &o) { return o.blocks; }, blk);
  const StatOp &o = s.o[w];
  if (o.mode == 0) stats_rows(o, blk, red);
  else stats_cols(o, blk);
}

__global__ __launch_bounds__(256) void stats_finalize_kernel(StatOps s) {
  __shared__ uint32_t red[2][4][64];
  __shared__ PoolCountSmem psm;
  const int nf3 = nfinal_blocks(s.o[0]) + nfinal_blocks(s.o[1]) + nfinal_blocks(s.o[2]);
  if ((int)blockIdx.x >= nf3) {
    pool_count_block(s.pc.P, s.pc.ps, s.pc.R, s.pc.npool, s.pc.vec, s.pc.rowblk, s.pc.colblk,
                     blockIdx.x - nf3, s.pcn, psm);
    return;
  }
  int blk;
  const StatOp &o = s.o[pick_op(s, blockIdx.x, [](const StatOp &q) { return nfinal_blocks(q); }, blk)];
  const int lane = threadIdx.x & 63, grp = threadIdx.x >> 6;
  const int c = blk * 64 + lane;
  uint32_t m = 0, n = 0xffffffffu;
  if (c < o.cols) {
    const uint32_t *pm = o.part + c, *pn = o.part + (size_t)o.rbk * o.cols + c;
    int q = grp;
    for (; q + 28 < o.rbk; q += 32) {
      uint32_t a[8], b[8];
#pragma unroll
      for (int j = 0; j < 8; ++j) {
        a[j] = pm[(size_t)(q + 4 * j) * o.cols];
        b[j] = pn[(size_t)(q + 4 * j) * o.cols];
      }
#pragma unroll
      for (int j = 0; j < 8; ++j) {
        m = max(m, a[j]);
        n = min(n, b[j]);
      }
    }
    for (; q < o.rbk; q += 4) {
      m = max(m, pm[(size_t)q * o.cols]);
      n = min(n, pn[(size_t)q * o.cols]);
    }
  }
  red[0][grp][lane] = m;
  red[1][grp][lane] = n;
  __syncthreads();
  m = max(max(red[0][0][lane], red[0][1][lane]), max(red[0][2][lane], red[0][3][lane]));
  n = min(min(red[1][0][lane], red[1][1][lane]), min(red[1][2][lane], red[1][3][lane]));
  if (grp == 0 && c < o.cols) {
    o.out[c] = m;
    o.out[o.cols + c] = n + 1u;
    o.out[2 * (size_t)o.cols + c] = 0;
  }
}

constexpr int CNT_ROWS = 64;
__host__ __device__ inline int ncount_blocks(const StatOp &o) {
  return o.mode == 1 && o.blocks ? ((o.cols + 63) / 64) * ((o.rows + CNT_ROWS - 1) / CNT_ROWS) : 0;
}
__global__ __launch_bounds__(256) void stats_count_kernel(StatOps s) {
  int blk;
  const StatOp &o = s.o[pick_op(s, blockIdx.x, [](const StatOp &q) { return ncount_blocks(q); }, blk)];
  const int ncb = (o.cols + 63) / 64;
  const int cb = blk % ncb, rc = blk / ncb;
  const int lane = threadIdx.x & 63, wave = threadIdx.x >> 6;
  const int c = cb * 64 + lane;
  bool spr = false;
  float bound = 0.0f;
  if (c < o.cols) {
    const uint32_t mx = o.out[c];
    spr = kcnn::f16x3::spread(mx, o.out[o.cols + c]);
    if (spr) bound = kcnn::f16x3::small_bound(mx);
  }
  if (__ballot(spr) == 0) return;
  const int r0 = rc * CNT_ROWS, r1 = min(o.rows, r0 + CNT_ROWS);
  uint32_t cnt = 0;
  if (spr) {
    float v[CNT_ROWS / 4];
#pragma unroll
    for (int i = 0; i < CNT_ROWS / 4; ++i) {
      const int r = r0 + wave + 4 * i;
      v[i] = r < r1 ? fabsf(X_row(o, r)[c]) : 0.0f;
    }
#pragma unroll
    for (int i = 0; i < CNT_ROWS / 4; ++i) cnt += (v[i] < bound && v[i] != 0.0f) ? 1u : 0u;
  }
  if (cnt) atomicAdd(o.out + 2 * (size_t)o.cols + c, cnt);
}

StatOp stat_op(const float *X, int rows, int cols, int ld, int mode, uint32_t *out,
               uint32_t *part) {
  StatOp o{};
  o.X = X; o.out = out; o.part = part;
  o.rows = rows; o.cols = cols; o.ld = ld; o.mode = mode;
  o.vec = ld % 4 == 0 && (uintptr_t)X % 16 == 0;
  if (rows <= 0 || cols <= 0) return o;
  if (mode == 0) {
    o.rpb = cols >= 2048 ? 1 : 4;
    o.blocks = (rows + o.rpb - 1) / o.rpb;
  } else {
    o.cb = (cols + 1023) / 1024;
    o.rbk = std::max(1, std::min(256, std::min((rows + 15) / 16, (1024 + o.cb - 1) / o.cb)));
    o.rb = (rows + o.rbk - 1) / o.rbk;
    o.rbk = (rows + o.rb - 1) / o.rb;
    o.blocks = o.cb * o.rbk;
    o.fblocks = (cols + 63) / 64;
  }
  return o;
}
size_t stat_part_words(int rows, int cols, int mode) {
  if (mode == 0) return 0;
  const StatOp o = stat_op(nullptr, rows, cols, cols, 1, nullptr, nullptr);
  return 2 * (size_t)o.rbk * cols;
}
int stats_launch3(const StatOps &ops, hipStream_t st) {
  for (const StatOp &o : ops.o)
    if (o.blocks == 0 && o.out) {
      const size_t n = o.mode == 0 ? (size_t)std::max(o.rows, 0) : (size_t)std::max(o.cols, 0);
      if (n && hipMemsetAsync(o.out, 0, 3 * n * 4, st) != hipSuccess) return (int)hipGetLastError();
    }
  int nb = 0, nf = 0, nc = 0;
  for (const StatOp &o : ops.o) {
    nb += o.blocks;
    nf += nfinal_blocks(o);
    nc += ncount_blocks(o);
  }
  nb += ops.pcx * ops.pcy;
  nf += ops.pcn;
  if (nb == 0) return 0;
  hipLaunchKernelGGL(stats_kernel, dim3(nb), dim3(256), 0, st, ops);
  int rc = kcnn::launch_status();
  if (rc || nf == 0) return rc;
  hipLaunchKernelGGL(stats_finalize_kernel, dim3(nf), dim3(256), 0, st, ops);
  rc = kcnn::launch_status();
  if (rc || nc == 0) return rc;
  hipLaunchKernelGGL(stats_count_kernel, dim3(nc), dim3(256), 0, st, ops);
  return kcnn::launch_status();
}
int stats_launch(const StatOp &a, const StatOp &b, hipStream_t st) {
  StatOps ops{};
  ops.o[0] = a;
  ops.o[1] = b;
  ops.o[2] = StatOp{};
  return stats_launch3(ops, st);
}

constexpr int REJ_LOCAL = 4;
__device__ __forceinline__ uint32_t reduce_quad(const GemmF16Args &p, int64_t e, int nq, int np4,
                                                int64_t plane, int &r, int &c, bool store) {
  const int N = p.N;
  r = (int)(e / nq);
  c = (int)(e - (int64_t)r * nq) * 4;
  const float *q = p.part + (int64_t)r * np4 + c;
  float4 v = *reinterpret_cast<const float4 *>(q);
  float4 w = p.ksplit > 1 ? *reinterpret_cast<const float4 *>(q + plane) : v;
  const uint32_t ar = p.amax[r], cr = p.acnt[r];
  uint32_t bm[4], cc[4];
  if (p.bvec) {
    const uint4 x = *reinterpret_cast<const uint4 *>(p.bmax + c);
    const uint4 y = *reinterpret_cast<const uint4 *>(p.bcnt + c);
    bm[0] = x.x; bm[1] = x.y; bm[2] = x.z; bm[3] = x.w;
    cc[0] = y.x; cc[1] = y.y; cc[2] = y.z; cc[3] = y.w;
  } else {
#pragma unroll
    for (int i = 0; i < 4; ++i) {
      bm[i] = c + i < N ? p.bmax[c + i] : NONFINITE;
      cc[i] = c + i < N ? p.bcnt[c + i] : 0u;
    }
  }
  float4 w4 = make_float4(0.0f, 0.0f, 0.0f, 0.0f), q4 = w4;
  float4 *wp = nullptr, *qp = nullptr;
  if (p.mom.W && store) {
    wp = reinterpret_cast<float4 *>(p.mom.W + (int64_t)r * p.mom.ldw + c);
    qp = reinterpret_cast<float4 *>(p.mom.prev + (int64_t)r * p.mom.ldp + c);
    if (c + 4 <= N) {
      w4 = *wp;
      q4 = *qp;
    }
  }
  float bv[4] = {0.0f, 0.0f, 0.0f, 0.0f};
  if (p.bias && store) {
    if (c + 4 <= N && ((uintptr_t)p.bias & 15) == 0) {
      const float4 b4 = *reinterpret_cast<const float4 *>(p.bias + c);
      bv[0] = b4.x; bv[1] = b4.y; bv[2] = b4.z; bv[3] = b4.w;
    } else {
#pragma unroll
      for (int i = 0; i < 4; ++i) bv[i] = c + i < N ? p.bias[c + i] : 0.0f;
    }
  }
  if (p.ksplit > 1) {
    v.x += w.x; v.y += w.y; v.z += w.z; v.w += w.w;
    for (int k = 2; k < p.ksplit; ++k) {
      w = *reinterpret_cast<const float4 *>(q + k * plane);
      v.x += w.x; v.y += w.y; v.z += w.z; v.w += w.w;
    }
  }
  if (ar >= NONFINITE) return 0;
  const float sv[4] = {v.x, v.y, v.z, v.w};
  const bool any = (cr | cc[0] | cc[1] | cc[2] | cc[3]) != 0 && ar != 0;
  float *o = p.C + (int64_t)r * p.ldc + c;
  const bool fin = max(max(bm[0], bm[1]), max(bm[2], bm[3])) < NONFINITE;
  if (p.mom.W && !any && fin) {
    if (store) {
      const MomentumEpi &m = p.mom;
      kcnn::momentum_step(p.alpha * sv[0], q4.x, w4.x, m.momentum, m.a_wd, m.a_g);
      kcnn::momentum_step(p.alpha * sv[1], q4.y, w4.y, m.momentum, m.a_wd, m.a_g);
      kcnn::momentum_step(p.alpha * sv[2], q4.z, w4.z, m.momentum, m.a_wd, m.a_g);
      kcnn::momentum_step(p.alpha * sv[3], q4.w, w4.w, m.momentum, m.a_wd, m.a_g);
      *qp = q4;
      *wp = w4;
    }
    return 0;
  }
  if (!p.mom.W && !any && fin && ((p.ldc & 3) | ((uintptr_t)p.C & 15)) == 0) {
    if (store) {
      float4 ov = make_float4(0.0f, 0.0f, 0.0f, 0.0f);
      if (p.beta != 0.0f) ov = *reinterpret_cast<const float4 *>(o);
      const float oi[4] = {ov.x, ov.y, ov.z, ov.w};
      float wv[4];
#pragma unroll
      for (int i = 0; i < 4; ++i) {
        wv[i] = p.beta == 0.0f ? p.alpha * sv[i] : p.alpha * sv[i] + p.beta * oi[i];
        if (p.bias) wv[i] += bv[i];
      }
      *reinterpret_cast<float4 *>(o) = make_float4(wv[0], wv[1], wv[2], wv[3]);
    }
    return 0;
  }
  float thr[4] = {0.0f, 0.0f, 0.0f, 0.0f};
  if (any) {
    const int er = scale_exp(ar);
#pragma unroll
    for (int i = 0; i < 4; ++i) {
      if (bm[i] >= NONFINITE || bm[i] == 0 || (cr | cc[i]) == 0) continue;
      thr[i] = __builtin_amdgcn_ldexpf(
          kcnn::f16x3::spread_weight(cr) + kcnn::f16x3::spread_weight(cc[i]),
          -(er + scale_exp(bm[i])));
    }
  }
  uint32_t rej = 0;
#pragma unroll
  for (int i = 0; i < 4; ++i) {
    if (bm[i] >= NONFINITE) continue;
    if (thr[i] != 0.0f && !(fabsf(sv[i]) >= thr[i])) {
      rej |= 1u << i;
      continue;
    }
    if (store) emit(p, r, c + i, sv[i]);
  }
  return rej;
}

__global__ __launch_bounds__(256) void gemm_f16x3_reduce_kernel(GemmF16Args p, int a_kc,
                                                                int b_kc) {
  const int np4 = (p.N + 3) & ~3, nq = np4 >> 2;
  const int64_t total = (int64_t)p.M * nq;
  const int64_t plane = (int64_t)p.M * np4;
  const int lane = threadIdx.x & 63;
  for (int64_t e = blockIdx.x * (int64_t)blockDim.x + threadIdx.x; e < total;
       e += (int64_t)gridDim.x * blockDim.x) {
    int r = (int)(e / nq), c = (int)(e - (int64_t)r * nq) * 4;
    const uint32_t rej = in_split_tile(p, r, c) ? reduce_quad(p, e, nq, np4, plane, r, c, true) : 0u;
    const int n = __builtin_popcountll(__ballot(rej & 1)) + __builtin_popcountll(__ballot(rej & 2)) +
                  __builtin_popcountll(__ballot(rej & 4)) + __builtin_popcountll(__ballot(rej & 8));
    const bool defer = n > REJ_LOCAL && !p.fix_local;
    if (lane == 0) {
      p.rflag[e >> 6] = defer ? 1u : 0u;
      if (defer) p.rflag[(total + 63) >> 6] = p.gen;
      if (n > REJ_LOCAL && p.fix_report) *p.fix_report = 1u;
    }
    if (n == 0 || defer) continue;
    fix_rejected(p, a_kc != 0, b_kc != 0, rej, lane, [&](int l, int bit, int &row, int &col) {
      row = __builtin_amdgcn_readlane(r, l);
      col = __builtin_amdgcn_readlane(c, l) + bit;
    });
  }
}

constexpr int FIX_DEPTH = 16;
constexpr int FIX_GRID = 1024;
__global__ __launch_bounds__(256) void gemm_f16x3_fixup_kernel(GemmF16Args p, int a_kc,
                                                               int b_kc, int rows) {
  __shared__ int list[256];
  __shared__ int nlist;
  __shared__ float4 quarter[4][64];
  const int np4 = (p.N + 3) & ~3, nq = np4 >> 2;
  const int64_t total = (int64_t)p.M * nq;
  const int64_t plane = (int64_t)p.M * np4;
  const int64_t nslots = (total + 63) >> 6;
  const int lane = threadIdx.x & 63, wave = threadIdx.x >> 6;
  if (p.rflag[nslots] != p.gen) return;
  for (int64_t base = 0; base < nslots; base += (int64_t)gridDim.x * blockDim.x) {
    if (threadIdx.x == 0) nlist = 0;
    __syncthreads();
    const int64_t slot = base + (int64_t)threadIdx.x * gridDim.x + blockIdx.x;
    if (slot < nslots && p.rflag[slot] != 0) list[atomicAdd(&nlist, 1)] = (int)threadIdx.x;
    __syncthreads();
    const int n = nlist;
    for (int j = 0; j < n; ++j) {
      const int64_t e0 = (base + (int64_t)list[j] * gridDim.x + blockIdx.x) << 6;
      const int64_t e = e0 + lane;
      int r = e < total ? (int)(e / nq) : 0;
      int c = e < total ? (int)(e - (int64_t)r * nq) * 4 : 0;
      const bool valid = e < total && in_split_tile(p, r, c);
      const uint32_t rej = valid ? reduce_quad(p, e, nq, np4, plane, r, c, false) : 0u;
      if (!rows) {
        const uint64_t mine = (lane & 3) == wave ? rej : 0u;
        fix_rejected(p, a_kc != 0, b_kc != 0, mine, lane, [&](int l, int bit, int &row, int &col) {
          row = __builtin_amdgcn_readlane(r, l);
          col = __builtin_amdgcn_readlane(c, l) + bit;
        });
        __syncthreads();
        continue;
      }
      const int kq = (p.K + 3) >> 2;
      const int k0 = wave * kq, k1 = min(p.K, k0 + kq);
      const int64_t sa = a_kc ? 1 : p.lda;
      const float *qa = a_kc ? p.A + (int64_t)r * p.lda + k0 : p.A + (int64_t)k0 * p.lda + r;
      const float *qb = p.B + (int64_t)k0 * p.ldb + c;
      float4 acc[4];
#pragma unroll
      for (int i = 0; i < 4; ++i) acc[i] = make_float4(0.0f, 0.0f, 0.0f, 0.0f);
      int k = k0;
#pragma unroll 1
      for (; k + FIX_DEPTH <= k1; k += FIX_DEPTH) {
        float x[FIX_DEPTH];
        float4 y[FIX_DEPTH];
#pragma unroll
        for (int i = 0; i < FIX_DEPTH; ++i) {
          x[i] = qa[i * sa];
          y[i] = *reinterpret_cast<const float4 *>(qb + (int64_t)i * p.ldb);
        }
#pragma unroll
        for (int i = 0; i < FIX_DEPTH; ++i) {
          float4 &t = acc[i & 3];
          t.x = fmaf(x[i], y[i].x, t.x);
          t.y = fmaf(x[i], y[i].y, t.y);
          t.z = fmaf(x[i], y[i].z, t.z);
          t.w = fmaf(x[i], y[i].w, t.w);
        }
        qa += FIX_DEPTH * sa;
        qb += (int64_t)FIX_DEPTH * p.ldb;
      }
#pragma unroll 1
      for (; k < k1; ++k) {
        const float x = *qa;
        const float4 y = *reinterpret_cast<const float4 *>(qb);
        acc[0].x = fmaf(x, y.x, acc[0].x);
        acc[0].y = fmaf(x, y.y, acc[0].y);
        acc[0].z = fmaf(x, y.z, acc[0].z);
        acc[0].w = fmaf(x, y.w, acc[0].w);
        qa += sa;
        qb += p.ldb;
      }
      float4 q;
      q.x = (acc[0].x + acc[1].x) + (acc[2].x + acc[3].x);
      q.y = (acc[0].y + acc[1].y) + (acc[2].y + acc[3].y);
      q.z = (acc[0].z + acc[1].z) + (acc[2].z + acc[3].z);
      q.w = (acc[0].w + acc[1].w) + (acc[2].w + acc[3].w);
      quarter[wave][lane] = q;
      __syncthreads();
      if (wave == 0 && rej) {
        const float4 q0 = quarter[0][lane], q1 = quarter[1][lane], q2 = quarter[2][lane],
                     q3 = quarter[3][lane];
        const float v[4] = {((q0.x + q1.x) + q2.x) + q3.x, ((q0.y + q1.y) + q2.y) + q3.y,
                            ((q0.z + q1.z) + q2.z) + q3.z, ((q0.w + q1.w) + q2.w) + q3.w};
#pragma unroll
        for (int i = 0; i < 4; ++i)
          if (rej >> i & 1) emit(p, r, c + i, v[i]);
      }
      __syncthreads();
    }
    __syncthreads();
  }
}

int choose_ksplit(int64_t tiles, int M, int N, int K, int *nwhole = nullptr) {
  auto round = [](int k) { return 0.0458 * k + 11.1; };
  int best = 1, best_w = 0;
  double best_t = (double)((tiles + 255) / 256) * round(K);
  for (int s = 2; s <= 4 && K / s >= 1024; ++s) {
    const int ks = (K + s - 1) / s;
    for (int64_t w = 0; w < tiles; w += 256) {
      const int64_t rest = tiles - w;
      const double t = (double)(w / 256) * round(K) + (double)((rest * s + 255) / 256) * round(ks) +
                       (double)(s + 1) * M * N * 4.0 / 4.0e6 * (double)rest / (double)tiles;
      if (t < best_t) { best_t = t; best = s; best_w = (int)w; }
    }
  }
  if (nwhole) *nwhole = best > 1 ? best_w : 0;
  return best;
}

template <int AM, int BMODE, bool RAG>
void launch_t(const GemmF16Args &a, unsigned blocks, hipStream_t st) {
  if constexpr (AM != LR && BMODE != LR) {
    static bool attr = [] {
      return hipFuncSetAttribute(
                 reinterpret_cast<const void *>(&gemm_f16x3_fast_kernel<AM, BMODE, RAG>),
                 hipFuncAttributeMaxDynamicSharedMemorySize, LDS_BYTES) == hipSuccess;
    }();
    (void)attr;
    hipLaunchKernelGGL((gemm_f16x3_fast_kernel<AM, BMODE, RAG>), dim3(blocks), dim3(NT),
                       LDS_BYTES, st, a);
  } else {
    static bool attr = [] {
      return hipFuncSetAttribute(
                 reinterpret_cast<const void *>(&gemm_f16x3_kernel<AM, BMODE, RAG>),
                 hipFuncAttributeMaxDynamicSharedMemorySize, LDS_BYTES) == hipSuccess;
    }();
    (void)attr;
    hipLaunchKernelGGL((gemm_f16x3_kernel<AM, BMODE, RAG>), dim3(blocks), dim3(NT), LDS_BYTES,
                       st, a);
  }
}
template <bool RAG>
void launch_r(int am, int bm, const GemmF16Args &a, unsigned blocks, hipStream_t st) {
  if (am == LK && bm == LK) launch_t<LK, LK, RAG>(a, blocks, st);
  else if (am == LK && bm == LT) launch_t<LK, LT, RAG>(a, blocks, st);
  else if (am == LK) launch_t<LK, LR, RAG>(a, blocks, st);
  else if (am == LT && bm == LK) launch_t<LT, LK, RAG>(a, blocks, st);
  else if (am == LT && bm == LT) launch_t<LT, LT, RAG>(a, blocks, st);
  else if (am == LT) launch_t<LT, LR, RAG>(a, blocks, st);
  else if (bm == LK) launch_t<LR, LK, RAG>(a, blocks, st);
  else if (bm == LT) launch_t<LR, LT, RAG>(a, blocks, st);
  else launch_t<LR, LR, RAG>(a, blocks, st);
}
void launch(int am, int bm, const GemmF16Args &a, unsigned blocks, hipStream_t st) {
  if (a.K % BK) launch_r<true>(am, bm, a, blocks, st);
  else launch_r<false>(am, bm, a, blocks, st);
}

size_t align16(size_t b) { return (b + 15) & ~(size_t)15; }
size_t slab_bytes(int s, int M, int N) {
  return align16(sizeof(float) * (size_t)s * M * ((N + 3) & ~3));
}
size_t flag_bytes(int M, int N) {
  return align16(sizeof(uint32_t) * (((size_t)M * ((N + 3) / 4) + 63) / 64 + 1));
}
size_t partial_bytes(int M, int N, int K) {
  const int64_t tiles = (int64_t)((M + BM - 1) / BM) * ((N + BN - 1) / BN);
  const int s = choose_ksplit(tiles, M, N, K);
  return s > 1 ? slab_bytes(s, M, N) + flag_bytes(M, N) : 0;
}

}

extern "C" int kl_absmax_rows(const float *X, int rows, int cols, int ld, uint32_t *rmax,
                              kcnn_stream_t stream) {
  if (rows < 0 || cols < 0 || ld < cols || !rmax) return (int)hipErrorInvalidValue;
  return stats_launch(stat_op(X, rows, cols, ld, 0, rmax, nullptr), StatOp{},
                      kcnn::as_stream(stream));
}
extern "C" size_t kl_absmax_cols_words(int rows, int cols) {
  if (rows <= 0 || cols <= 0) return 0;
  return stat_part_words(rows, cols, 1);
}
extern "C" int kl_absmax_cols(const float *X, int rows, int cols, int ld, uint32_t *cmax,
                              uint32_t *part, kcnn_stream_t stream) {
  if (rows < 0 || cols < 0 || ld < cols || !cmax) return (int)hipErrorInvalidValue;
  if (rows > 0 && cols > 0 && !part) return (int)hipErrorInvalidValue;
  return stats_launch(stat_op(X, rows, cols, ld, 1, cmax, part), StatOp{},
                      kcnn::as_stream(stream));
}

extern "C" int kl_absmax_rows_cols(const float *R, int rows, int cols, int ld, uint32_t *rmax,
                                   const float *Q, int qrows, int qcols, int ldq, uint32_t *cmax,
                                   uint32_t *part, uint32_t *clear, kcnn_stream_t stream) {
  if (rows < 0 || cols < 0 || ld < cols || !rmax || qrows < 0 || qcols < 0 || ldq < qcols ||
      !cmax)
    return (int)hipErrorInvalidValue;
  if (qrows > 0 && qcols > 0 && !part) return (int)hipErrorInvalidValue;
  StatOp q = stat_op(Q, qrows, qcols, ldq, 1, cmax, part);
  q.clear = clear;
  const StatOp r = stat_op(R, rows, cols, ld, 0, rmax, nullptr);
  if (clear && q.blocks + r.blocks == 0) {
    const hipError_t e = hipMemsetAsync(clear, 0, 8, kcnn::as_stream(stream));
    if (e != hipSuccess) return (int)e;
  }
  return stats_launch(q, r, kcnn::as_stream(stream));
}

extern "C" int kl_gemm_stats3(const float *X0, int rows0, int cols0, int ld0, int mode0,
                              uint32_t *out0, uint32_t *part0, const float *X1, int rows1,
                              int cols1, int ld1, int mode1, uint32_t *out1, uint32_t *part1,
                              const float *X2, int rows2, int cols2, int ld2, int mode2,
                              uint32_t *out2, uint32_t *part2, void *pool_cols,
                              kcnn_stream_t stream) {
  StatOps ops{};
  if (pool_cols) {
    ops.pc = *static_cast<const PoolColDeferred *>(pool_cols);
    const int ncq = ops.pc.npool % 4 == 0 ? ops.pc.npool / 4 : ops.pc.npool;
    ops.pcx = (ncq + 255) / 256;
    ops.pcy = (ops.pc.nblk + COLMAX_ROWS - 1) / COLMAX_ROWS;
    ops.pcn = std::min(ops.pc.R, 256);
  }
  const float *X[3] = {X0, X1, X2};
  const int rows[3] = {rows0, rows1, rows2}, cols[3] = {cols0, cols1, cols2};
  const int ld[3] = {ld0, ld1, ld2}, mode[3] = {mode0, mode1, mode2};
  uint32_t *out[3] = {out0, out1, out2}, *part[3] = {part0, part1, part2};
  for (int i = 0; i < 3; ++i) {
    ops.o[i] = StatOp{};
    if (!X[i]) continue;
    if (rows[i] < 0 || cols[i] < 0 || ld[i] < cols[i] || !out[i] || (mode[i] != 0 && mode[i] != 1) ||
        (mode[i] == 1 && rows[i] > 0 && cols[i] > 0 && !part[i]))
      return (int)hipErrorInvalidValue;
    ops.o[i] = stat_op(X[i], rows[i], cols[i], ld[i], mode[i], out[i], mode[i] ? part[i] : nullptr);
  }
  return stats_launch3(ops, kcnn::as_stream(stream));
}

extern "C" size_t kl_gemm_f16x3_workspace_bytes(int M, int N, int K) {
  return partial_bytes(M, N, K);
}
constexpr int FIX_SITES = 256;
struct FixSites {
  std::mutex mu;
  uint32_t *flags = nullptr;
  uint32_t *dflags = nullptr;
  int64_t key[FIX_SITES][6];
  int n = 0;
  bool failed = false;
};
static uint32_t *fix_site(int M, int N, int K, int ta, int tb, int mom, uint32_t **dev) {
  static FixSites fs;
  std::lock_guard<std::mutex> lk(fs.mu);
  if (!fs.flags && !fs.failed) {
    void *h = nullptr, *d = nullptr;
    if (hipHostMalloc(&h, FIX_SITES * sizeof(uint32_t), hipHostMallocMapped | hipHostMallocCoherent) ==
            hipSuccess &&
        hipHostGetDevicePointer(&d, h, 0) == hipSuccess) {
      fs.flags = static_cast<uint32_t *>(h);
      fs.dflags = static_cast<uint32_t *>(d);
    } else {
      (void)hipGetLastError();
      fs.failed = true;
    }
  }
  if (!fs.flags) return nullptr;
  const int64_t k[6] = {M, N, K, ta, tb, mom};
  int i = 0;
  for (; i < fs.n; ++i)
    if (std::equal(k, k + 6, fs.key[i])) break;
  if (i == fs.n) {
    if (fs.n == FIX_SITES) return nullptr;
    std::copy(k, k + 6, fs.key[fs.n++]);
    __atomic_store_n(fs.flags + i, 1u, __ATOMIC_RELAXED);
  }
  *dev = fs.dflags + i;
  return fs.flags + i;
}

static int gemm_f16x3_st(int transA, int transB, int M, int N, int K, float alpha,
                         const float *A, int lda, const float *B, int ldb, float beta, float *C,
                         int ldc, const uint32_t *amax, const uint32_t *bmax, const float *bias,
                         void *ws, size_t ws_bytes, kcnn_stream_t stream,
                         const MomentumEpi *mom = nullptr) {
  if (M < 0 || N < 0 || K < 0) return (int)hipErrorInvalidValue;
  if (M == 0 || N == 0 || K == 0) return (int)hipErrorNotSupported;
  const bool a_kc = !transA, b_kc = transB != 0;
  if ((a_kc && (lda % 4 || (uintptr_t)A % 16)) || (b_kc && (ldb % 4 || (uintptr_t)B % 16)))
    return (int)hipErrorNotSupported;
  hipStream_t st = kcnn::as_stream(stream);
  GemmF16Args a{};
  a.A = A; a.B = B; a.C = C; a.amax = amax; a.bmax = bmax; a.bias = bias;
  if (mom) a.mom = *mom;
  a.amin = amax + M;
  a.acnt = amax + 2 * (size_t)M;
  a.bmin = bmax + N;
  a.bcnt = bmax + 2 * (size_t)N;
  a.bvec = N % 4 == 0 && (uintptr_t)a.bmax % 16 == 0 && (uintptr_t)a.bcnt % 16 == 0;
  a.M = M; a.N = N; a.K = K; a.lda = lda; a.ldb = ldb; a.ldc = ldc;
  a.alpha = alpha; a.beta = beta;
  a.tiles_m = (M + BM - 1) / BM;
  a.tiles_n = (N + BN - 1) / BN;
  const int64_t tiles = (int64_t)a.tiles_m * a.tiles_n;
  int nwhole = 0;
  int s = choose_ksplit(tiles, M, N, K, &nwhole);
  const size_t need = s > 1 ? slab_bytes(s, M, N) + flag_bytes(M, N) : 0;
  if (need > ws_bytes || !ws) s = 1;
  if (s > 1) {
    a.part = static_cast<float *>(ws);
    a.rflag = reinterpret_cast<uint32_t *>(static_cast<char *>(ws) + slab_bytes(s, M, N));
    static std::atomic<uint32_t> calls{0};
    a.gen = ++calls;
    if (a.gen == 0) a.gen = ++calls;
  }
  a.ksplit = s;
  a.kps = ((K + s - 1) / s + BK - 1) / BK * BK;
  auto fits = [&](bool kc, int ld, int R, int span) {
    if (kc) return (int64_t)R * ld * 4 + (int64_t)(K + 2 * BK) * 4 < ((int64_t)1 << 31);
    return (int64_t)(span + 2 * BK) * ld * 4 + (int64_t)R * 4 < ((int64_t)1 << 31);
  };
  if (!fits(a_kc, lda, BM, a.kps) || !fits(b_kc, ldb, BN, a.kps)) return (int)hipErrorNotSupported;
  if (s == 1 || !fits(a_kc, lda, BM, K) || !fits(b_kc, ldb, BN, K)) nwhole = 0;
  a.nwhole = nwhole;
  const int64_t nb = nwhole + (tiles - nwhole) * s;
  if (nb >= ((int64_t)1 << 31)) return (int)hipErrorNotSupported;
  auto mode = [](bool kc, const float *ptr, int ld) {
    if (kc) return (int)LK;
    return ld % 4 == 0 && (uintptr_t)ptr % 16 == 0 ? (int)LT : (int)LR;
  };
  bool fix_launch = true;
  if (s > 1) {
    uint32_t *dev = nullptr;
    uint32_t *site = fix_site(M, N, K, transA != 0, transB != 0, a.mom.W != nullptr, &dev);
    if (site) {
      fix_launch = __atomic_load_n(site, __ATOMIC_RELAXED) != 0;
      __atomic_store_n(site, 0u, __ATOMIC_RELAXED);
      a.fix_report = dev;
      a.fix_local = fix_launch ? 0 : 1;
    }
  }
  launch(mode(a_kc, A, lda), mode(b_kc, B, ldb), a, (unsigned)nb, st);
  int rc = kcnn::launch_status();
  if (rc || s == 1) return rc;
  hipLaunchKernelGGL(gemm_f16x3_reduce_kernel, dim3(kcnn::grid_for((int64_t)M * ((N + 3) / 4))),
                     dim3(256), 0, st, a, a_kc ? 1 : 0, b_kc ? 1 : 0);
  rc = kcnn::launch_status();
  if (rc || !fix_launch) return rc;
  const int rows = !b_kc && ldb % 4 == 0 && (uintptr_t)B % 16 == 0 && N % 4 == 0;
  const int64_t slots = ((int64_t)M * ((N + 3) / 4) + 63) / 64;
  hipLaunchKernelGGL(gemm_f16x3_fixup_kernel,
                     dim3((unsigned)std::min<int64_t>(FIX_GRID, (slots + 15) / 16)), dim3(256), 0, st,
                     a, a_kc ? 1 : 0, b_kc ? 1 : 0, rows);
  return kcnn::launch_status();
}
extern "C" int kl_gemm_f16x3_st(int transA, int transB, int M, int N, int K, float alpha,
                                const float *A, int lda, const float *B, int ldb, float beta,
                                float *C, int ldc, const uint32_t *amax, const uint32_t *bmax,
                                void *ws, size_t ws_bytes, kcnn_stream_t stream) {
  return gemm_f16x3_st(transA, transB, M, N, K, alpha, A, lda, B, ldb, beta, C, ldc, amax, bmax,
                       nullptr, ws, ws_bytes, stream);
}

namespace {
size_t stats_ws_words(int M, int N, int K, int transA, int transB) {
  const size_t pa = transA ? stat_part_words(K, M, 1) : 0;
  const size_t pb = transB ? 0 : stat_part_words(K, N, 1);
  return 3 * ((size_t)M + N) + 4 + pa + pb;
}
}
extern "C" size_t kl_gemm_f16x3_full_workspace_bytes(int M, int N, int K) {
  size_t w = 0;
  for (int ta = 0; ta < 2; ++ta)
    for (int tb = 0; tb < 2; ++tb) w = std::max(w, stats_ws_words(M, N, K, ta, tb));
  return partial_bytes(M, N, K) + align16(sizeof(uint32_t) * w);
}
extern "C" int kl_gemm_f16x3(int transA, int transB, int M, int N, int K, float alpha,
                             const float *A, int lda, const float *B, int ldb, float beta,
                             float *C, int ldc, void *ws, size_t ws_bytes,
                             kcnn_stream_t stream) {
  return kl_gemm_f16x3_given(transA, transB, M, N, K, alpha, A, lda, B, ldb, beta, C, ldc,
                             nullptr, nullptr, ws, ws_bytes, stream);
}
extern "C" int kl_gemm_f16x3_given(int transA, int transB, int M, int N, int K, float alpha,
                                   const float *A, int lda, const float *B, int ldb, float beta,
                                   float *C, int ldc, const uint32_t *amax_given,
                                   const uint32_t *bmax_given, void *ws, size_t ws_bytes,
                                   kcnn_stream_t stream) {
  return kl_gemm_f16x3_bias(transA, transB, M, N, K, alpha, A, lda, B, ldb, beta, C, ldc,
                            amax_given, bmax_given, nullptr, ws, ws_bytes, stream);
}
static int gemm_f16x3_full(int transA, int transB, int M, int N, int K, float alpha,
                           const float *A, int lda, const float *B, int ldb, float beta,
                           float *C, int ldc, const uint32_t *amax_given,
                           const uint32_t *bmax_given, const float *bias, void *ws,
                           size_t ws_bytes, kcnn_stream_t stream, const MomentumEpi *mom) {
  if (M < 0 || N < 0 || K < 0) return (int)hipErrorInvalidValue;
  if (M == 0 || N == 0 || K == 0) return (int)hipErrorNotSupported;
  const size_t pb = partial_bytes(M, N, K);
  if (!ws || ws_bytes < kl_gemm_f16x3_full_workspace_bytes(M, N, K))
    return (int)hipErrorInvalidValue;
  uint32_t *amax = reinterpret_cast<uint32_t *>(static_cast<char *>(ws) + pb);
  uint32_t *bmax = amax + 3 * (size_t)M;
  uint32_t *parta = bmax + 3 * (size_t)N + 4;
  uint32_t *partb = parta + (transA ? stat_part_words(K, M, 1) : 0);
  const StatOp sa = amax_given ? StatOp{}
                    : transA   ? stat_op(A, K, M, lda, 1, amax, parta)
                               : stat_op(A, M, K, lda, 0, amax, nullptr);
  const StatOp sb = bmax_given ? StatOp{}
                    : transB   ? stat_op(B, N, K, ldb, 0, bmax, nullptr)
                               : stat_op(B, K, N, ldb, 1, bmax, partb);
  if (!amax_given || !bmax_given) {
    const int rc = amax_given ? stats_launch(sb, StatOp{}, kcnn::as_stream(stream))
                              : stats_launch(sa, sb, kcnn::as_stream(stream));
    if (rc) return rc;
  }
  return gemm_f16x3_st(transA, transB, M, N, K, alpha, A, lda, B, ldb, beta, C, ldc,
                       amax_given ? amax_given : amax, bmax_given ? bmax_given : bmax, bias,
                       pb ? ws : nullptr, pb, stream, mom);
}
extern "C" int kl_gemm_f16x3_bias(int transA, int transB, int M, int N, int K, float alpha,
                                  const float *A, int lda, const float *B, int ldb, float beta,
                                  float *C, int ldc, const uint32_t *amax_given,
                                  const uint32_t *bmax_given, const float *bias, void *ws,
                                  size_t ws_bytes, kcnn_stream_t stream) {
  return gemm_f16x3_full(transA, transB, M, N, K, alpha, A, lda, B, ldb, beta, C, ldc,
                         amax_given, bmax_given, bias, ws, ws_bytes, stream, nullptr);
}
extern "C" int kl_gemm_f16x3_momentum(int transA, int transB, int M, int N, int K,
                                      const float *A, int lda, const float *B, int ldb,
                                      const uint32_t *amax_given, const uint32_t *bmax_given,
                                      float *W, int ldw, float *prev, int ldp, float momentum,
                                      float a_wd, float a_g, void *ws, size_t ws_bytes,
                                      kcnn_stream_t stream) {
  if (!W || !prev || ldw % 4 || ldp % 4 || (uintptr_t)W % 16 || (uintptr_t)prev % 16)
    return (int)hipErrorNotSupported;
  MomentumEpi m;
  m.W = W; m.prev = prev; m.ldw = ldw; m.ldp = ldp;
  m.momentum = momentum; m.a_wd = a_wd; m.a_g = a_g;
  return gemm_f16x3_full(transA, transB, M, N, K, 1.0f, A, lda, B, ldb, 0.0f, nullptr, ldw,
                         amax_given, bmax_given, nullptr, ws, ws_bytes, stream, &m);
}
```

### kaldi-cnn_amd/src/kaldi-lite/cu-kernels-lite.h

```cpp
#ifndef KCNN_KALDI_LITE_CU_KERNELS_LITE_H_
#define KCNN_KALDI_LITE_CU_KERNELS_LITE_H_

#include <stddef.h>
#include <stdint.h>

#include "cnsl-hip-kernels.h"

#ifdef __cplusplus
extern "C" {
#endif
int kl_set(float *d, MatrixDim dim, float v, kcnn_stream_t st);
int kl_scale(float *d, MatrixDim dim, float a, kcnn_stream_t st);
int kl_add(float *d, MatrixDim dim, float a, kcnn_stream_t st);
int kl_add_mat(float alpha, const float *A, MatrixDim ad, int transA,
               float beta, float *D, MatrixDim dd, kcnn_stream_t st);
int kl_copy_rows_from_vec(const float *v, float *D, MatrixDim dd,
                          kcnn_stream_t st);
int kl_sum_partials(const float *parts, int S, int m, int n, float beta,
                    float *C, MatrixDim cd, kcnn_stream_t st);
size_t kl_col_sum_workspace_bytes(MatrixDim md);
int kl_col_sum(const float *M, MatrixDim md, float alpha, float beta, float *v,
               void *ws, kcnn_stream_t st);
size_t kl_gemm_x6_workspace_bytes(int M, int N, int K);
int kl_gemm_x6(int transA, int transB, int M, int N, int K, float alpha,
               const float *A, int lda, const float *B, int ldb, float beta,
               float *C, int ldc, void *ws, size_t ws_bytes, kcnn_stream_t st);
int kl_absmax_rows(const float *X, int rows, int cols, int ld, uint32_t *rmax,
                   kcnn_stream_t st);
size_t kl_absmax_cols_words(int rows, int cols);
int kl_absmax_cols(const float *X, int rows, int cols, int ld, uint32_t *cmax, uint32_t *part,
                   kcnn_stream_t st);
int kl_absmax_rows_cols(const float *R, int rows, int cols, int ld, uint32_t *rmax,
                        const float *Q, int qrows, int qcols, int ldq, uint32_t *cmax,
                        uint32_t *part, uint32_t *clear, kcnn_stream_t stream);
int kl_gemm_stats3(const float *X0, int rows0, int cols0, int ld0, int mode0, uint32_t *out0,
                   uint32_t *part0, const float *X1, int rows1, int cols1, int ld1, int mode1,
                   uint32_t *out1, uint32_t *part1, const float *X2, int rows2, int cols2,
                   int ld2, int mode2, uint32_t *out2, uint32_t *part2, void *pool_cols,
                   kcnn_stream_t stream);
size_t kl_gemm_f16x3_workspace_bytes(int M, int N, int K);
int kl_gemm_f16x3_st(int transA, int transB, int M, int N, int K, float alpha,
                     const float *A, int lda, const float *B, int ldb, float beta, float *C,
                     int ldc, const uint32_t *amax, const uint32_t *bmax, void *ws,
                     size_t ws_bytes, kcnn_stream_t st);
size_t kl_gemm_f16x3_full_workspace_bytes(int M, int N, int K);
int kl_gemm_f16x3(int transA, int transB, int M, int N, int K, float alpha,
                  const float *A, int lda, const float *B, int ldb, float beta, float *C,
                  int ldc, void *ws, size_t ws_bytes, kcnn_stream_t st);
int kl_gemm_f16x3_given(int transA, int transB, int M, int N, int K, float alpha,
                        const float *A, int lda, const float *B, int ldb, float beta, float *C,
                        int ldc, const uint32_t *amax, const uint32_t *bmax, void *ws,
                        size_t ws_bytes, kcnn_stream_t st);
int kl_gemm_f16x3_bias(int transA, int transB, int M, int N, int K, float alpha,
                       const float *A, int lda, const float *B, int ldb, float beta, float *C,
                       int ldc, const uint32_t *amax_given, const uint32_t *bmax_given,
                       const float *bias, void *ws, size_t ws_bytes, kcnn_stream_t stream);
int kl_gemm_f16x3_momentum(int transA, int transB, int M, int N, int K, const float *A,
                           int lda, const float *B, int ldb, const uint32_t *amax_given,
                           const uint32_t *bmax_given, float *W, int ldw, float *prev, int ldp,
                           float momentum, float a_wd, float a_g, void *ws, size_t ws_bytes,
                           kcnn_stream_t stream);
int kl_split_planes(const float *src, int rows, int cols, int ld, uint16_t *dst, int ldp,
                    int64_t ps, kcnn_stream_t st);
size_t kl_gemm_planes_workspace_bytes(int M, int N, int K);
int kl_gemm_planes(int transA, int transB, int M, int N, int K, float alpha,
                   const uint16_t *A, int lda, int64_t aps, const uint16_t *B, int ldb,
                   int64_t bps, float beta, float *C, int ldc, void *ws, size_t ws_bytes,
                   kcnn_stream_t st);
int kl_dot(const float *A, MatrixDim ad, const float *B, MatrixDim bd,
           int transB, double *out_dev, kcnn_stream_t st);
#ifdef __cplusplus
}
#endif
#endif
```

### kaldi-cnn_amd/src/kaldi-lite/cu-matrix.cc

```cpp
#include "cu-matrix.h"

#include <math.h>
#include <stdint.h>
#include <stdlib.h>
#include <string.h>

#include <limits>
#include <mutex>
#include <sstream>

#include "cu-device.h"
#include "cu-kernels-lite.h"
#include "../cnslmat/pool-stats.h"
#include "kaldi-io.h"

namespace kaldi {

namespace {
inline kcnn_stream_t S() {
  return reinterpret_cast<kcnn_stream_t>(CuDevice::Instantiate().Stream());
}
inline MatrixIndexT PaddedStride(MatrixIndexT cols) {
  return (cols + 15) / 16 * 16;
}
::MatrixDim VecDim(MatrixIndexT n) {
  ::MatrixDim d;
  d.rows = 1; d.cols = n; d.stride = n;
  return d;
}

std::mutex g_rng_mu;
uint64_t g_rng_state = 20261015ull;
uint64_t splitmix64() {
  uint64_t z = (g_rng_state += 0x9E3779B97F4A7C15ull);
  z = (z ^ (z >> 30)) * 0xBF58476D1CE4E5B9ull;
  z = (z ^ (z >> 27)) * 0x94D049BB133111EBull;
  return z ^ (z >> 31);
}
}

void SetRandnSeed(uint64_t seed) {
  std::lock_guard<std::mutex> lk(g_rng_mu);
  g_rng_state = seed;
}

uint64_t RandU64() {
  std::lock_guard<std::mutex> lk(g_rng_mu);
  return splitmix64();
}

void RandnFill(float *dst, size_t n) {
  std::lock_guard<std::mutex> lk(g_rng_mu);
  for (size_t i = 0; i < n; i += 2) {
    const double u1 = ((splitmix64() >> 11) + 1.0) * (1.0 / 9007199254740993.0);
    const double u2 = (splitmix64() >> 11) * (1.0 / 9007199254740992.0);
    const double r = sqrt(-2.0 * log(u1));
    dst[i] = (float)(r * cos(2.0 * M_PI * u2));
    if (i + 1 < n) dst[i + 1] = (float)(r * sin(2.0 * M_PI * u2));
  }
}

template <typename Real>
void MatrixBase<Real>::Write(std::ostream &os, bool binary) const {
  if (binary) {
    WriteToken(os, binary, sizeof(Real) == 4 ? "FM" : "DM");
    WriteBasicType(os, binary, (int32)rows_);
    WriteBasicType(os, binary, (int32)cols_);
    os.write(reinterpret_cast<const char *>(data_.data()),
             sizeof(Real) * data_.size());
  } else {
    if (cols_ == 0) {
      os << " [ ]\n";
    } else {
      os << " [";
      os.precision(std::numeric_limits<Real>::max_digits10);
      for (MatrixIndexT i = 0; i < rows_; i++) {
        os << "\n  ";
        for (MatrixIndexT j = 0; j < cols_; j++) os << (*this)(i, j) << " ";
      }
      os << "]\n";
    }
  }
  if (os.fail()) KALDI_ERR << "failed to write matrix";
}

template <typename Real>
void MatrixBase<Real>::Read(std::istream &is, bool binary) {
  if (binary) {
    std::string tok;
    ReadToken(is, binary, &tok);
    if (tok != (sizeof(Real) == 4 ? "FM" : "DM"))
      KALDI_ERR << "expected matrix token FM, got " << tok;
    int32 r, c;
    ReadBasicType(is, binary, &r);
    ReadBasicType(is, binary, &c);
    if (r < 0 || c < 0) KALDI_ERR << "bad matrix size " << r << " x " << c;
    Resize(r, c);
    is.read(reinterpret_cast<char *>(data_.data()), sizeof(Real) * data_.size());
    if (is.fail()) KALDI_ERR << "failed to read matrix data";
    return;
  }
  std::string tok;
  is >> tok;
  if (tok != "[") KALDI_ERR << "expected '[' reading text matrix, got " << tok;
  std::vector<std::vector<Real>> rows;
  std::string line;
  std::getline(is, line);
  bool done = false;
  {
    std::istringstream ls(line);
    std::string t;
    while (ls >> t) {
      if (t == "]") { done = true; break; }
      KALDI_ERR << "unexpected '" << t << "' after '['";
    }
  }
  while (!done && std::getline(is, line)) {
    std::istringstream ls(line);
    std::vector<Real> row;
    std::string t;
    while (ls >> t) {
      if (t == "]") { done = true; break; }
      float v;
      if (!ConvertStringToReal(t, &v)) KALDI_ERR << "bad matrix element " << t;
      row.push_back((Real)v);
    }
    if (!row.empty()) rows.push_back(row);
  }
  if (!done) KALDI_ERR << "unterminated text matrix";
  const MatrixIndexT r = (MatrixIndexT)rows.size();
  const MatrixIndexT c = r ? (MatrixIndexT)rows[0].size() : 0;
  Resize(r, c);
  for (MatrixIndexT i = 0; i < r; i++) {
    if ((MatrixIndexT)rows[i].size() != c) KALDI_ERR << "ragged text matrix";
    for (MatrixIndexT j = 0; j < c; j++) (*this)(i, j) = rows[i][j];
  }
}

template <typename Real>
void VectorBase<Real>::Write(std::ostream &os, bool binary) const {
  if (binary) {
    WriteToken(os, binary, sizeof(Real) == 4 ? "FV" : "DV");
    WriteBasicType(os, binary, (int32)data_.size());
    os.write(reinterpret_cast<const char *>(data_.data()),
             sizeof(Real) * data_.size());
  } else {
    os.precision(std::numeric_limits<Real>::max_digits10);
    os << " [ ";
    for (auto v : data_) os << v << " ";
    os << "]\n";
  }
  if (os.fail()) KALDI_ERR << "failed to write vector";
}

template <typename Real>
void VectorBase<Real>::Read(std::istream &is, bool binary) {
  if (binary) {
    std::string tok;
    ReadToken(is, binary, &tok);
    if (tok != (sizeof(Real) == 4 ? "FV" : "DV"))
      KALDI_ERR << "expected vector token FV, got " << tok;
    int32 d;
    ReadBasicType(is, binary, &d);
    if (d < 0) KALDI_ERR << "bad vector size " << d;
    Resize(d);
    is.read(reinterpret_cast<char *>(data_.data()), sizeof(Real) * d);
    if (is.fail()) KALDI_ERR << "failed to read vector data";
    return;
  }
  std::string tok;
  is >> tok;
  if (tok != "[") KALDI_ERR << "expected '[' reading text vector, got " << tok;
  data_.clear();
  while (is >> tok) {
    if (tok == "]") return;
    char *end = nullptr;
    const double v = strtod(tok.c_str(), &end);
    if (tok.empty() || *end != '\0') KALDI_ERR << "bad vector element " << tok;
    data_.push_back((Real)v);
  }
  KALDI_ERR << "unterminated text vector";
}

template <typename Real>
void CuMatrixBase<Real>::SetZero() {
  if (num_rows_ == 0 || num_cols_ == 0) return;
  CU_SAFE_CALL(hipMemset2DAsync(data_, sizeof(Real) * stride_, 0,
                                sizeof(Real) * num_cols_, num_rows_,
                                CuDevice::Instantiate().Stream()));
}
template <typename Real>
void CuMatrixBase<Real>::Set(Real v) { CNSL_SAFE_CALL(kl_set(data_, Dim(), v, S())); }
template <typename Real>
void CuMatrixBase<Real>::Add(Real v) { CNSL_SAFE_CALL(kl_add(data_, Dim(), v, S())); }
template <typename Real>
void CuMatrixBase<Real>::Scale(Real v) { CNSL_SAFE_CALL(kl_scale(data_, Dim(), v, S())); }

template <typename Real>
void CuMatrixBase<Real>::SetRandn() {
  Matrix<Real> h(num_rows_, num_cols_);
  RandnFill(h.Data(), (size_t)num_rows_ * num_cols_);
  CopyFromMat(h);
}

template <typename Real>
void CuMatrixBase<Real>::CopyFromMat(const CuMatrixBase<Real> &src,
                                     MatrixTransposeType trans) {
  if (trans == kNoTrans) {
    KALDI_ASSERT(src.NumRows() == num_rows_ && src.NumCols() == num_cols_);
    if (num_rows_ == 0 || num_cols_ == 0) return;
    CU_SAFE_CALL(hipMemcpy2DAsync(data_, sizeof(Real) * stride_, src.Data(),
                                  sizeof(Real) * src.Stride(),
                                  sizeof(Real) * num_cols_, num_rows_,
                                  hipMemcpyDeviceToDevice,
                                  CuDevice::Instantiate().Stream()));
  } else {
    KALDI_ASSERT(src.NumCols() == num_rows_ && src.NumRows() == num_cols_);
    CNSL_SAFE_CALL(kl_add_mat(1.0f, src.Data(), src.Dim(), 1, 0.0f, data_, Dim(), S()));
  }
}

template <typename Real>
void CuMatrixBase<Real>::CopyFromMat(const MatrixBase<Real> &src) {
  KALDI_ASSERT(src.NumRows() == num_rows_ && src.NumCols() == num_cols_);
  if (num_rows_ == 0 || num_cols_ == 0) return;
  CU_SAFE_CALL(hipMemcpy2DAsync(data_, sizeof(Real) * stride_, src.Data(),
                                sizeof(Real) * src.Stride(),
                                sizeof(Real) * num_cols_, num_rows_,
                                hipMemcpyHostToDevice,
                                CuDevice::Instantiate().Stream()));
  CuDevice::Instantiate().Synchronize();
}

template <typename Real>
void CuMatrixBase<Real>::CopyToMat(MatrixBase<Real> *dst) const {
  if (dst->NumRows() != num_rows_ || dst->NumCols() != num_cols_)
    dst->Resize(num_rows_, num_cols_);
  if (num_rows_ == 0 || num_cols_ == 0) return;
  CU_SAFE_CALL(hipMemcpy2DAsync(dst->Data(), sizeof(Real) * dst->Stride(),
                                data_, sizeof(Real) * stride_,
                                sizeof(Real) * num_cols_, num_rows_,
                                hipMemcpyDeviceToHost,
                                CuDevice::Instantiate().Stream()));
  CuDevice::Instantiate().Synchronize();
}

template <typename Real>
void CuMatrixBase<Real>::AddMat(Real alpha, const CuMatrixBase<Real> &A,
                                MatrixTransposeType trans) {
  if (trans == kNoTrans)
    KALDI_ASSERT(A.NumRows() == num_rows_ && A.NumCols() == num_cols_);
  else
    KALDI_ASSERT(A.NumCols() == num_rows_ && A.NumRows() == num_cols_);
  CNSL_SAFE_CALL(kl_add_mat(alpha, A.Data(), A.Dim(), trans == kTrans, 1.0f,
                            data_, Dim(), S()));
}

static thread_local const CuGemmStatsHint *g_stats_hints = nullptr;

CuGemmStatsHint::CuGemmStatsHint(const float *data, MatrixIndexT rows, MatrixIndexT cols,
                                 MatrixIndexT stride, const uint32_t *rmax,
                                 const uint32_t *cmax)
    : rowmax(rmax), colmax(cmax), data_(data), rows_(rows), cols_(cols), stride_(stride),
      prev_(g_stats_hints) {
  g_stats_hints = this;
}
CuGemmStatsHint::~CuGemmStatsHint() { g_stats_hints = prev_; }
const CuGemmStatsHint *CuGemmStatsHint::Find(const float *data, MatrixIndexT rows,
                                             MatrixIndexT cols, MatrixIndexT stride) {
  for (const CuGemmStatsHint *h = g_stats_hints; h; h = h->prev_)
    if (h->data_ == data && h->rows_ == rows && h->cols_ == cols && h->stride_ == stride)
      return h;
  return nullptr;
}

static const uint32_t *hint_cols(const CuGemmStatsHint *h, kcnn_stream_t st) {
  if (h->pending) CNSL_SAFE_CALL(kcnn_pool_cols_complete(h->pending, st));
  return h->colmax;
}

CuGemmBackpropStats::CuGemmBackpropStats(const CuMatrixBase<float> &dy,
                                         const CuMatrixBase<float> &W, bool cols,
                                         const CuMatrixBase<float> *in) {
  CuDevice &dev = CuDevice::Instantiate();
  const int N = dy.NumRows(), O = dy.NumCols(), I = W.NumCols();
  if (dev.GemmMode() != 2 || N == 0 || O == 0 || I == 0 || W.NumRows() != O) return;
  {
    const CuGemmStatsHint *hd = CuGemmStatsHint::Find(dy.Data(), N, O, dy.Stride());
    const CuGemmStatsHint *hw = CuGemmStatsHint::Find(W.Data(), O, I, W.Stride());
    if (hd && hd->rowmax && (!cols || hd->colmax) && hw && hw->colmax && !hw->pending) return;
  }
  const size_t pd = cols ? kl_absmax_cols_words(N, O) : 0, pw = kl_absmax_cols_words(O, I);
  const size_t words = 3 * ((size_t)N + O + I) + pd + pw;
  ws_ = dev.Malloc(words * 4);
  uint32_t *rows_d = static_cast<uint32_t *>(ws_), *cols_d = rows_d + 3 * (size_t)N,
           *cols_w = cols_d + 3 * (size_t)O, *part_d = cols_w + 3 * (size_t)I,
           *part_w = part_d + pd;
  PoolColDeferred *pc = nullptr;
  if (cols && in) {
    const CuGemmStatsHint *h =
        CuGemmStatsHint::Find(in->Data(), in->NumRows(), in->NumCols(), in->Stride());
    if (h && h->pending && h->pending->pending) pc = h->pending;
  }
  CNSL_SAFE_CALL(kl_gemm_stats3(dy.Data(), N, O, dy.Stride(), 0, rows_d, nullptr,
                                cols ? dy.Data() : nullptr, N, O, dy.Stride(), 1, cols_d, part_d,
                                W.Data(), O, I, W.Stride(), 1, cols_w, part_w, pc,
                                reinterpret_cast<kcnn_stream_t>(dev.Stream())));
  if (pc) pc->pending = 0;
  hint_d_ = new CuGemmStatsHint(dy.Data(), N, O, dy.Stride(), rows_d, cols ? cols_d : nullptr);
  hint_w_ = new CuGemmStatsHint(W.Data(), O, I, W.Stride(), nullptr, cols_w);
}
CuGemmBackpropStats::~CuGemmBackpropStats() {
  delete hint_w_;
  delete hint_d_;
  if (ws_) CuDevice::Instantiate().Free(ws_);
}

template <typename Real>
bool CuMatrixBase<Real>::GemmF16x3(Real alpha, const CuMatrixBase<Real> &A,
                                   const CuMatrixBase<Real> &Ap, MatrixTransposeType transA,
                                   const CuMatrixBase<Real> &B, const CuMatrixBase<Real> &Bp,
                                   MatrixTransposeType transB, Real beta, const Real *bias) {
  const MatrixIndexT m = num_rows_, n = num_cols_;
  const MatrixIndexT k = transA == kNoTrans ? A.NumCols() : A.NumRows();
  CuDevice &dev0 = CuDevice::Instantiate();
  const CuGemmStatsHint *ha = CuGemmStatsHint::Find(A.Data(), A.NumRows(), A.NumCols(),
                                                    A.Stride());
  const CuGemmStatsHint *hb = CuGemmStatsHint::Find(B.Data(), B.NumRows(), B.NumCols(),
                                                    B.Stride());
  const uint32_t *ag = ha ? (transA == kNoTrans ? ha->rowmax : hint_cols(ha, S())) : nullptr;
  const uint32_t *bg = hb ? (transB == kNoTrans ? hint_cols(hb, S()) : hb->rowmax) : nullptr;
  const size_t wsf = kl_gemm_f16x3_full_workspace_bytes(m, n, k);
  void *wf = dev0.Malloc(wsf);
  const int rc = kl_gemm_f16x3_bias(transA == kTrans, transB == kTrans, m, n, k, alpha,
                                    Ap.Data(), Ap.Stride(), Bp.Data(), Bp.Stride(), beta, data_,
                                    stride_, ag, bg, bias, wf, wsf, S());
  dev0.Free(wf);
  if (rc == (int)hipErrorNotSupported) return false;
  CNSL_SAFE_CALL(rc);
  return true;
}

template <typename Real>
bool CuMatrixBase<Real>::AddMatMatMomentum(const CuMatrixBase<Real> &A,
                                           MatrixTransposeType transA,
                                           const CuMatrixBase<Real> &B,
                                           MatrixTransposeType transB, CuMatrixBase<Real> *prev,
                                           Real momentum, Real a_wd, Real a_g) {
  const MatrixIndexT m = num_rows_, n = num_cols_;
  const MatrixIndexT k = transA == kNoTrans ? A.NumCols() : A.NumRows();
  CuDevice &dev0 = CuDevice::Instantiate();
  auto aligned = [](const CuMatrixBase<Real> &X) {
    return X.Stride() % 4 == 0 && reinterpret_cast<uintptr_t>(X.Data()) % 16 == 0;
  };
  if (dev0.GemmMode() != 2 || m == 0 || n == 0 || k == 0 || !aligned(A) || !aligned(B) ||
      !aligned(*this) || !aligned(*prev))
    return false;
  KALDI_ASSERT((transA == kNoTrans ? A.NumRows() : A.NumCols()) == m &&
               (transB == kNoTrans ? B.NumCols() : B.NumRows()) == n &&
               (transB == kNoTrans ? B.NumRows() : B.NumCols()) == k &&
               prev->NumRows() == m && prev->NumCols() == n);
  CuProfileScope prof("AddMatMat");
  const CuGemmStatsHint *ha = CuGemmStatsHint::Find(A.Data(), A.NumRows(), A.NumCols(),
                                                    A.Stride());
  const CuGemmStatsHint *hb = CuGemmStatsHint::Find(B.Data(), B.NumRows(), B.NumCols(),
                                                    B.Stride());
  const uint32_t *ag = ha ? (transA == kNoTrans ? ha->rowmax : hint_cols(ha, S())) : nullptr;
  const uint32_t *bg = hb ? (transB == kNoTrans ? hint_cols(hb, S()) : hb->rowmax) : nullptr;
  const size_t wsf = kl_gemm_f16x3_full_workspace_bytes(m, n, k);
  void *wf = dev0.Malloc(wsf);
  const int rc = kl_gemm_f16x3_momentum(transA == kTrans, transB == kTrans, m, n, k, A.Data(),
                                        A.Stride(), B.Data(), B.Stride(), ag, bg, data_, stride_,
                                        prev->Data(), prev->Stride(), momentum, a_wd, a_g, wf,
                                        wsf, S());
  dev0.Free(wf);
  if (rc == (int)hipErrorNotSupported) return false;
  CNSL_SAFE_CALL(rc);
  return true;
}

template <typename Real>
void CuMatrixBase<Real>::AddMatMatBias(Real alpha, const CuMatrixBase<Real> &A,
                                       MatrixTransposeType transA, const CuMatrixBase<Real> &B,
                                       MatrixTransposeType transB,
                                       const CuVectorBase<Real> &bias) {
  const MatrixIndexT k = transA == kNoTrans ? A.NumCols() : A.NumRows();
  KALDI_ASSERT(bias.Dim() == num_cols_);
  CuDevice &dev0 = CuDevice::Instantiate();
  auto aligned = [](const CuMatrixBase<Real> &X) {
    return X.Stride() % 4 == 0 && reinterpret_cast<uintptr_t>(X.Data()) % 16 == 0;
  };
  if (dev0.GemmMode() == 2 && num_rows_ > 0 && num_cols_ > 0 && k > 0 && aligned(A) &&
      aligned(B)) {
    KALDI_ASSERT((transA == kNoTrans ? A.NumRows() : A.NumCols()) == num_rows_ &&
                 (transB == kNoTrans ? B.NumCols() : B.NumRows()) == num_cols_ &&
                 (transB == kNoTrans ? B.NumRows() : B.NumCols()) == k);
    CuProfileScope prof("AddMatMat");
    if (GemmF16x3(alpha, A, A, transA, B, B, transB, 0.0f, bias.Data())) return;
  }
  CopyRowsFromVec(bias);
  AddMatMat(alpha, A, transA, B, transB, 1.0f);
}

template <typename Real>
void CuMatrixBase<Real>::AddMatMat(Real alpha, const CuMatrixBase<Real> &A,
                                   MatrixTransposeType transA,
                                   const CuMatrixBase<Real> &B,
                                   MatrixTransposeType transB, Real beta) {
  const MatrixIndexT m = transA == kNoTrans ? A.NumRows() : A.NumCols();
  const MatrixIndexT k = transA == kNoTrans ? A.NumCols() : A.NumRows();
  const MatrixIndexT kb = transB == kNoTrans ? B.NumRows() : B.NumCols();
  const MatrixIndexT n = transB == kNoTrans ? B.NumCols() : B.NumRows();
  KALDI_ASSERT(k == kb && m == num_rows_ && n == num_cols_);
  if (m == 0 || n == 0) return;
  if (k == 0) { if (beta != 1.0f) Scale(beta); return; }
  CuProfileScope prof("AddMatMat");
  CuDevice &dev0 = CuDevice::Instantiate();
  const int mode = dev0.GemmMode();
  if (mode >= 1) {
    auto aligned = [](const CuMatrixBase<Real> &X) {
      return X.Stride() % 4 == 0 && reinterpret_cast<uintptr_t>(X.Data()) % 16 == 0;
    };
    CuMatrix<Real> Acopy, Bcopy;
    const CuMatrixBase<Real> *Ap = &A, *Bp = &B;
    if ((transA == kNoTrans || mode == 2) && !aligned(A)) { Acopy = A; Ap = &Acopy; }
    if ((transB == kTrans || mode == 2) && !aligned(B)) { Bcopy = B; Bp = &Bcopy; }
    if (mode == 2 && GemmF16x3(alpha, A, *Ap, transA, B, *Bp, transB, beta, nullptr)) return;
    const size_t wsb = kl_gemm_x6_workspace_bytes(m, n, k);
    void *ws = wsb ? dev0.Malloc(wsb) : nullptr;
    const int rc = kl_gemm_x6(transA == kTrans, transB == kTrans, m, n, k, alpha,
                              Ap->Data(), Ap->Stride(), Bp->Data(), Bp->Stride(), beta,
                              data_, stride_, ws, wsb, S());
    if (ws) dev0.Free(ws);
    if (rc == (int)hipErrorInvalidValue)
      KALDI_ERR << "AddMatMat: " << m << " x " << n << " x " << k
                << " is outside the bf16x6 GEMM's limits; select rocBLAS sgemm with "
                   "kcnn_set_kernel_family(\"gemm\", 0)";
    CNSL_SAFE_CALL(rc);
    return;
  }
  const rocblas_operation opB =
      transB == kTrans ? rocblas_operation_transpose : rocblas_operation_none;
  const rocblas_operation opA =
      transA == kTrans ? rocblas_operation_transpose : rocblas_operation_none;
  int nsplit = 1;
  const int64_t tiles = (int64_t)((m + 255) / 256) * ((n + 255) / 256);
  if (tiles < 128 && k >= 4096) {
    for (int s : {4, 2})
      if (k % s == 0 && k / s >= 1024 && tiles * s <= 512) { nsplit = s; break; }
  }
  if (nsplit > 1) {
    CuDevice &dev = CuDevice::Instantiate();
    const int S_ = nsplit;
    const int kc = k / S_;
    const rocblas_stride sA = transA == kNoTrans ? kc : (rocblas_stride)kc * A.Stride();
    const rocblas_stride sB = transB == kNoTrans ? (rocblas_stride)kc * B.Stride() : kc;
    float *part = static_cast<float *>(dev.Malloc(sizeof(float) * (size_t)S_ * m * n));
    const float zero = 0.0f;
    rocblas_status st = rocblas_sgemm_strided_batched(
        dev.GetBlasHandle(), opB, opA, n, m, kc, &alpha, B.Data(), B.Stride(),
        sB, A.Data(), A.Stride(), sA, &zero, part, n, (rocblas_stride)m * n, S_);
    int rc = st == rocblas_status_success
                 ? kl_sum_partials(part, S_, m, n, beta, data_, Dim(), S())
                 : -1;
    dev.Free(part);
    if (st != rocblas_status_success)
      KALDI_ERR << "rocblas_sgemm_strided_batched failed with status " << (int)st;
    CNSL_SAFE_CALL(rc);
    return;
  }
  rocblas_status st = rocblas_sgemm(
      CuDevice::Instantiate().GetBlasHandle(), opB, opA, n, m, k, &alpha,
      B.Data(), B.Stride(), A.Data(), A.Stride(), &beta, data_, stride_);
  if (st != rocblas_status_success)
    KALDI_ERR << "rocblas_sgemm failed with status " << (int)st;
}

template <typename Real>
void CuMatrixBase<Real>::CopyRowsFromVec(const CuVectorBase<Real> &v) {
  KALDI_ASSERT(v.Dim() == num_cols_);
  CNSL_SAFE_CALL(kl_copy_rows_from_vec(v.Data(), data_, Dim(), S()));
}
template <typename Real>
void CuMatrixBase<Real>::CopyRowsFromVec(const VectorBase<Real> &v) {
  CuVector<Real> tmp;
  tmp = v;
  CopyRowsFromVec(tmp);
}

template <typename Real>
Real CuMatrixBase<Real>::Sum() const {
  Matrix<Real> h;
  CopyToMat(&h);
  double s = 0;
  for (MatrixIndexT i = 0; i < h.NumRows(); i++)
    for (MatrixIndexT j = 0; j < h.NumCols(); j++) s += h(i, j);
  return (Real)s;
}

template <typename Real>
CuSubMatrix<Real> CuMatrixBase<Real>::Range(MatrixIndexT ro, MatrixIndexT nr,
                                            MatrixIndexT co,
                                            MatrixIndexT nc) const {
  KALDI_ASSERT(ro >= 0 && co >= 0 && nr >= 0 && nc >= 0 &&
               ro + nr <= num_rows_ && co + nc <= num_cols_);
  return CuSubMatrix<Real>(data_ + (int64)ro * stride_ + co, nr, nc, stride_);
}
template <typename Real>
CuSubMatrix<Real> CuMatrixBase<Real>::RowRange(MatrixIndexT ro,
                                               MatrixIndexT nr) const {
  return Range(ro, nr, 0, num_cols_);
}
template <typename Real>
CuSubMatrix<Real> CuMatrixBase<Real>::ColRange(MatrixIndexT co,
                                               MatrixIndexT nc) const {
  return Range(0, num_rows_, co, nc);
}

template <typename Real>
void CuMatrixBase<Real>::Write(std::ostream &os, bool binary) const {
  Matrix<Real> h;
  CopyToMat(&h);
  h.Write(os, binary);
}

template <typename Real>
void CuMatrix<Real>::Destroy() {
  if (this->data_ && !borrowed_) CuDevice::Instantiate().Free(this->data_);
  this->data_ = nullptr;
  this->num_rows_ = this->num_cols_ = this->stride_ = 0;
  borrowed_ = false;
}

template <typename Real>
void CuMatrix<Real>::Resize(MatrixIndexT rows, MatrixIndexT cols,
                            MatrixResizeType resize_type) {
  KALDI_ASSERT(rows >= 0 && cols >= 0);
  if (rows == this->num_rows_ && cols == this->num_cols_) {
    if (resize_type == kSetZero) this->SetZero();
    return;
  }
  if (borrowed_)
    KALDI_ERR << "cannot resize a matrix bound to external memory from "
              << this->num_rows_ << "x" << this->num_cols_ << " to " << rows
              << "x" << cols;
  if (resize_type == kCopyData) {
    CuMatrix<Real> tmp(rows, cols, kSetZero);
    const MatrixIndexT r = std::min(rows, this->num_rows_);
    const MatrixIndexT c = std::min(cols, this->num_cols_);
    if (r > 0 && c > 0) tmp.Range(0, r, 0, c).CopyFromMat(this->Range(0, r, 0, c));
    Swap(&tmp);
    return;
  }
  Destroy();
  if (rows == 0 || cols == 0) return;
  const MatrixIndexT stride = PaddedStride(cols);
  this->data_ = static_cast<Real *>(
      CuDevice::Instantiate().Malloc(sizeof(Real) * (size_t)rows * stride));
  this->num_rows_ = rows;
  this->num_cols_ = cols;
  this->stride_ = stride;
  if (resize_type == kSetZero) this->SetZero();
}

template <typename Real>
void CuMatrix<Real>::Swap(CuMatrix<Real> *o) {
  std::swap(this->data_, o->data_);
  std::swap(this->num_rows_, o->num_rows_);
  std::swap(this->num_cols_, o->num_cols_);
  std::swap(this->stride_, o->stride_);
  std::swap(borrowed_, o->borrowed_);
}

template <typename Real>
void CuMatrix<Real>::Borrow(Real *data, MatrixIndexT rows, MatrixIndexT cols,
                            MatrixIndexT stride) {
  Destroy();
  this->data_ = data;
  this->num_rows_ = rows;
  this->num_cols_ = cols;
  this->stride_ = stride;
  borrowed_ = true;
}

template <typename Real>
CuMatrix<Real> &CuMatrix<Real>::operator=(const CuMatrixBase<Real> &o) {
  if (static_cast<const CuMatrixBase<Real> *>(this) == &o) return *this;
  Resize(o.NumRows(), o.NumCols(), kUndefined);
  this->CopyFromMat(o);
  return *this;
}
template <typename Real>
CuMatrix<Real> &CuMatrix<Real>::operator=(const CuMatrix<Real> &o) {
  return *this = static_cast<const CuMatrixBase<Real> &>(o);
}
template <typename Real>
CuMatrix<Real> &CuMatrix<Real>::operator=(const MatrixBase<Real> &o) {
  Resize(o.NumRows(), o.NumCols(), kUndefined);
  this->CopyFromMat(o);
  return *this;
}

template <typename Real>
void CuMatrix<Real>::Read(std::istream &is, bool binary) {
  Matrix<Real> h;
  h.Read(is, binary);
  *this = h;
}

template <typename Real>
void CuVectorBase<Real>::SetZero() {
  if (dim_ == 0) return;
  CU_SAFE_CALL(hipMemsetAsync(data_, 0, sizeof(Real) * dim_,
                              CuDevice::Instantiate().Stream()));
}
template <typename Real>
void CuVectorBase<Real>::Set(Real v) { CNSL_SAFE_CALL(kl_set(data_, VecDim(dim_), v, S())); }
template <typename Real>
void CuVectorBase<Real>::Add(Real v) { CNSL_SAFE_CALL(kl_add(data_, VecDim(dim_), v, S())); }
template <typename Real>
void CuVectorBase<Real>::Scale(Real v) { CNSL_SAFE_CALL(kl_scale(data_, VecDim(dim_), v, S())); }
template <typename Real>
void CuVectorBase<Real>::SetRandn() {
  Vector<Real> h(dim_);
  RandnFill(h.Data(), dim_);
  CopyFromVec(h);
}
template <typename Real>
void CuVectorBase<Real>::CopyFromVec(const CuVectorBase<Real> &v) {
  KALDI_ASSERT(v.Dim() == dim_);
  if (dim_ == 0) return;
  CU_SAFE_CALL(hipMemcpyAsync(data_, v.Data(), sizeof(Real) * dim_,
                              hipMemcpyDeviceToDevice,
                              CuDevice::Instantiate().Stream()));
}
template <typename Real>
void CuVectorBase<Real>::CopyFromVec(const VectorBase<Real> &v) {
  KALDI_ASSERT(v.Dim() == dim_);
  if (dim_ == 0) return;
  CU_SAFE_CALL(hipMemcpyAsync(data_, v.Data(), sizeof(Real) * dim_,
                              hipMemcpyHostToDevice,
                              CuDevice::Instantiate().Stream()));
  CuDevice::Instantiate().Synchronize();
}
template <typename Real>
void CuVectorBase<Real>::CopyToVec(VectorBase<Real> *v) const {
  if (v->Dim() != dim_) v->Resize(dim_);
  if (dim_ == 0) return;
  CU_SAFE_CALL(hipMemcpyAsync(v->Data(), data_, sizeof(Real) * dim_,
                              hipMemcpyDeviceToHost,
                              CuDevice::Instantiate().Stream()));
  CuDevice::Instantiate().Synchronize();
}
template <typename Real>
void CuVectorBase<Real>::AddVec(Real alpha, const CuVectorBase<Real> &v,
                                Real beta) {
  KALDI_ASSERT(v.Dim() == dim_);
  CNSL_SAFE_CALL(kl_add_mat(alpha, v.Data(), VecDim(dim_), 0, beta, data_,
                            VecDim(dim_), S()));
}
template <typename Real>
void CuVectorBase<Real>::AddRowSumMat(Real alpha, const CuMatrixBase<Real> &M,
                                      Real beta) {
  KALDI_ASSERT(M.NumCols() == dim_);
  CuDevice &dev = CuDevice::Instantiate();
  void *ws = dev.Malloc(kl_col_sum_workspace_bytes(M.Dim()));
  const int rc = kl_col_sum(M.Data(), M.Dim(), alpha, beta, data_, ws, S());
  dev.Free(ws);
  CNSL_SAFE_CALL(rc);
}
template <typename Real>
void CuVectorBase<Real>::CopyColFromMat(const CuMatrixBase<Real> &M,
                                        MatrixIndexT col) {
  KALDI_ASSERT(M.NumRows() == dim_ && col >= 0 && col < M.NumCols());
  if (dim_ == 0) return;
  CU_SAFE_CALL(hipMemcpy2DAsync(data_, sizeof(Real), M.Data() + col,
                                sizeof(Real) * M.Stride(), sizeof(Real), dim_,
                                hipMemcpyDeviceToDevice,
                                CuDevice::Instantiate().Stream()));
}
template <typename Real>
CuSubVector<Real> CuVectorBase<Real>::Range(MatrixIndexT o,
                                            MatrixIndexT l) const {
  KALDI_ASSERT(o >= 0 && l >= 0 && o + l <= dim_);
  return CuSubVector<Real>(data_ + o, l);
}
template <typename Real>
void CuVectorBase<Real>::Write(std::ostream &os, bool binary) const {
  Vector<Real> h;
  CopyToVec(&h);
  h.Write(os, binary);
}

template <typename Real>
void CuVector<Real>::Destroy() {
  if (this->data_ && !borrowed_) CuDevice::Instantiate().Free(this->data_);
  this->data_ = nullptr;
  this->dim_ = 0;
  borrowed_ = false;
}
template <typename Real>
void CuVector<Real>::Resize(MatrixIndexT d, MatrixResizeType t) {
  KALDI_ASSERT(d >= 0);
  if (d == this->dim_) {
    if (t == kSetZero) this->SetZero();
    return;
  }
  if (borrowed_) KALDI_ERR << "cannot resize a vector bound to external memory";
  Destroy();
  if (d == 0) return;
  this->data_ = static_cast<Real *>(CuDevice::Instantiate().Malloc(sizeof(Real) * d));
  this->dim_ = d;
  if (t == kSetZero) this->SetZero();
}
template <typename Real>
void CuVector<Real>::Borrow(Real *data, MatrixIndexT dim) {
  Destroy();
  this->data_ = data;
  this->dim_ = dim;
  borrowed_ = true;
}
template <typename Real>
CuVector<Real> &CuVector<Real>::operator=(const CuVectorBase<Real> &o) {
  if (static_cast<const CuVectorBase<Real> *>(this) == &o) return *this;
  Resize(o.Dim(), kUndefined);
  this->CopyFromVec(o);
  return *this;
}
template <typename Real>
CuVector<Real> &CuVector<Real>::operator=(const CuVector<Real> &o) {
// ... 56 lines not shown
```

### kaldi-cnn_amd/src/kaldi-lite/kcnn-knobs.cc

```cpp
#include "kcnn-knobs.h"

#include <stdlib.h>
#include <string.h>

#include <atomic>

namespace kcnn {
namespace {

struct FamilyInfo {
  const char *name, *env;
  int dflt, max;
};
const FamilyInfo kFamilies[kNumFamilies] = {
    {"fwd_x6", "KCNN_FWD_X6", 2, 2},
    {"bwd_x6", "KCNN_BWD_X6", 1, 1},
    {"igemm_x6", "KCNN_IGEMM_X6", 2, 3},
    {"wgrad_x6", "KCNN_WGRAD_X6", 2, 3},
    {"gemm", "KCNN_GEMM", 2, 2},
};

int from_env(const FamilyInfo &f) {
  const char *e = getenv(f.env);
  if (!e || !*e) return f.dflt;
  const int v = atoi(e);
  return v < 0 ? 0 : v > f.max ? f.max : v;
}

std::atomic<int> *values() {
  static std::atomic<int> v[kNumFamilies];
  static const bool init = [] {
    for (int i = 0; i < kNumFamilies; ++i) v[i].store(from_env(kFamilies[i]));
    return true;
  }();
  (void)init;
  return v;
}

}

int family(Family f) { return values()[f].load(std::memory_order_relaxed); }

int set_family(Family f, int value) {
  if (f < 0 || f >= kNumFamilies || value < 0 || value > kFamilies[f].max) return -1;
  values()[f].store(value);
  return 0;
}

int family_by_name(const char *name) {
  if (!name) return -1;
  for (int i = 0; i < kNumFamilies; ++i)
    if (strcmp(name, kFamilies[i].name) == 0) return i;
  return -1;
}

#ifdef KCNN_PHASE_TIMING
int phase_timing() {
  static const int on = [] {
    const char *s = getenv("KCNN_PHASE_TIMING");
    return s && atoi(s) != 0 ? 1 : 0;
  }();
  return on;
}
#endif

}
```

Baseline: 3.009 million frames/sec.

## Add a 256-wide N tile variant to the f16x3 GEMM with plan selection

Templates the fast f16x3 GEMM kernel on the N tile width and adds a 256x256 tile variant with its own loader path and a generalized epilogue. A planner picks tile width and k-split per shape, based on the gemm family knob, whose maximum rises to 4. The wider tile raises operand reuse per block and cuts the number of tiles for the large FC GEMMs. In exchange it uses more LDS and registers per block and fills the GPU with fewer blocks. Debug entry points for plan inspection and tile counting are also added.

Measured after the change: 3.060 million frames/sec (median of 6 runs). 1.02x the previous value.

```diff
diff --git a/experiments/fc_shapes.py b/experiments/fc_shapes.py
--- a/experiments/fc_shapes.py
+++ b/experiments/fc_shapes.py
@@ -6,13 +6,16 @@
 
 SHAPES = [("fwd", 4096, 1024, 11616, False, True),
           ("dgrad", 4096, 11616, 1024, False, False),
-          ("wgrad", 1024, 11616, 4096, True, False)]
+          ("wgrad", 1024, 11616, 4096, True, False),
+          ("cal_k1024", 4096, 4096, 1024, False, True),
+          ("cal_k2016", 4096, 4096, 2016, False, True),
+          ("cal_k4096", 4096, 4096, 4096, False, True)]
 
 
 def main():
     calls = int(sys.argv[1]) if len(sys.argv) > 1 else 20
     kcnn.init(0)
-    kcnn.set_gemm_mode(2)
+    kcnn.set_gemm_mode(int(sys.argv[2]) if len(sys.argv) > 2 else 2)
     g = torch.Generator(device="cuda").manual_seed(5)
     for name, m, n, k, ta, tb in SHAPES:
         a = torch.randn((k, m) if ta else (m, k), device="cuda", generator=g)
@@ -28,7 +31,8 @@
         e1.record()
         torch.cuda.synchronize()
         us = e0.elapsed_time(e1) * 1e3 / calls
-        print(f"{name} {m}x{n}x{k}: {us:.1f} us per call, "
+        plan = kcnn.gemm_plan(ta, tb, m, n, k) if hasattr(kcnn.lib(), "kcnn_gemm_plan") else None
+        print(f"{name} {m}x{n}x{k} plan {plan}: {us:.1f} us per call, "
               f"{2 * m * n * k / us / 1e6:.1f} TFLOP/s", flush=True)
 
 
diff --git a/include/kcnn.h b/include/kcnn.h
--- a/include/kcnn.h
+++ b/include/kcnn.h
@@ -21,6 +21,8 @@
 int kcnn_set_profiling(int on);
 int kcnn_set_fusion(int mode);
 int kcnn_set_gemm_mode(int mode);
+int kcnn_gemm_tile_counts(unsigned long long *out, int reset);
+int kcnn_gemm_plan(int trans_a, int trans_b, int m, int n, int k, int lda, int ldb, int *out);
 int kcnn_set_kernel_family(const char *name, int value);
 int kcnn_get_kernel_family(const char *name);
 int kcnn_gemm(int trans_a, int trans_b, int m, int n, int k, float alpha,
diff --git a/kaldi-cnn_amd/kcnn.py b/kaldi-cnn_amd/kcnn.py
--- a/kaldi-cnn_amd/kcnn.py
+++ b/kaldi-cnn_amd/kcnn.py
@@ -138,6 +138,23 @@
     check(lib().kcnn_set_gemm_mode(int(mode)))
 
 
+def gemm_tile_counts(reset=False):
+    out = (ctypes.c_ulonglong * 2)()
+    check(lib().kcnn_gemm_tile_counts(out, int(bool(reset))))
+    return tuple(int(v) for v in out)
+
+
+def gemm_plan(trans_a, trans_b, m, n, k, lda=None, ldb=None):
+    if lda is None:
+        lda = m if trans_a else k
+    if ldb is None:
+        ldb = k if trans_b else n
+    out = (ctypes.c_int * 3)()
+    check(lib().kcnn_gemm_plan(int(bool(trans_a)), int(bool(trans_b)), int(m), int(n), int(k),
+                               int(lda), int(ldb), out))
+    return tuple(int(v) for v in out)
+
+
 def set_kernel_family(name: str, value: int):
     check(lib().kcnn_set_kernel_family(name.encode(), int(value)))
 
diff --git a/kaldi-cnn_amd/src/capi/kcnn-capi.cc b/kaldi-cnn_amd/src/capi/kcnn-capi.cc
--- a/kaldi-cnn_amd/src/capi/kcnn-capi.cc
+++ b/kaldi-cnn_amd/src/capi/kcnn-capi.cc
@@ -169,8 +169,19 @@
   return 0;
 }
 int kcnn_set_gemm_mode(int mode) {
-  if (mode < 0 || mode > 2) return fail("kcnn_set_gemm_mode: mode is 0, 1 or 2");
+  if (mode < 0 || mode > 4) return fail("kcnn_set_gemm_mode: mode is 0 to 4");
   CuDevice::Instantiate().SetGemmMode(mode);
+  return 0;
+}
+int kcnn_gemm_tile_counts(unsigned long long *out, int reset) {
+  if (!out) return fail("kcnn_gemm_tile_counts: out is NULL");
+  kl_gemm_f16x3_tile_counts(out, reset);
+  return 0;
+}
+int kcnn_gemm_plan(int trans_a, int trans_b, int m, int n, int k, int lda, int ldb, int *out) {
+  if (!out) return fail("kcnn_gemm_plan: out is NULL");
+  if (m <= 0 || n <= 0 || k <= 0) return fail("kcnn_gemm_plan: dimensions must be positive");
+  kl_gemm_f16x3_plan(trans_a, trans_b, m, n, k, lda, ldb, out);
   return 0;
 }
 int kcnn_set_kernel_family(const char *name, int value) {
diff --git a/kaldi-cnn_amd/src/kaldi-lite/cu-gemm-f16x3.hip b/kaldi-cnn_amd/src/kaldi-lite/cu-gemm-f16x3.hip
--- a/kaldi-cnn_amd/src/kaldi-lite/cu-gemm-f16x3.hip
+++ b/kaldi-cnn_amd/src/kaldi-lite/cu-gemm-f16x3.hip
@@ -12,6 +12,7 @@
 #include "cnslmat/pool-stats-dev.h"
 #include "cnslmat/pool-stats.h"
 #include "kaldi-lite/cu-kernels-lite.h"
+#include "kaldi-lite/kcnn-knobs.h"
 
 namespace {
 
@@ -30,12 +31,19 @@
 typedef short s16x8 __attribute__((ext_vector_type(8)));
 typedef __attribute__((address_space(3))) s16x4 lds_s16x4;
 
-constexpr int BM = 256, BN = 128, BK = 32, NT = 512;
+constexpr int BM = 256, BK = 32, NT = 512;
 constexpr int ROWB = BK * 2;
 constexpr int A_PLANE = BM * ROWB;
-constexpr int B_PLANE = BN * ROWB;
-constexpr int BUF = 2 * (A_PLANE + B_PLANE);
-constexpr int LDS_BYTES = 2 * BUF + (BM + BN) * 8;
+constexpr int BN_NARROW = 128, BN_WIDE = 256;
+template <int BN>
+struct Tile {
+  static constexpr int WN = BN / 64;
+  static constexpr int WR = BM / (8 / WN);
+  static constexpr int MI = WR / 32;
+  static constexpr int B_PLANE = BN * ROWB;
+  static constexpr int BUF = 2 * (A_PLANE + B_PLANE);
+  static constexpr int LDS_BYTES = 2 * BUF + (BM + BN) * 8;
+};
 
 struct GemmF16Args {
   const float *A, *B;
@@ -51,6 +59,7 @@
   int bvec;
   MomentumEpi mom;
   int kps, ksplit, tiles_m, tiles_n;
+  int bn;
   int nwhole;
   int fix_local;
   uint32_t *fix_report;
@@ -83,7 +92,7 @@
   return whole;
 }
 __device__ __forceinline__ bool in_split_tile(const GemmF16Args &p, int r, int c) {
-  return p.nwhole == 0 || tile_index(p, r / BM, c / BN) >= p.nwhole;
+  return p.nwhole == 0 || tile_index(p, r / BM, c / p.bn) >= p.nwhole;
 }
 
 __device__ __forceinline__ int swz(int r, int c) {
@@ -261,6 +270,31 @@
       }
     }
   }
+  static constexpr int NPART = MODE == LT ? KPT : UPT;
+  static constexpr int PPP = NPIECE / NPART;
+  __device__ __forceinline__ void load_part(__amdgpu_buffer_rsrc_t rs, int ld, int vrows, int kk,
+                                            int tid, int q) {
+    static_assert(MODE != LR, "the wide tile has no LR loader");
+    constexpr unsigned OOB = 0x80000000u;
+    if constexpr (MODE == LK) {
+      const int unit = tid + q * NT;
+      const int r = unit >> 2, k = kk + (unit & 3) * 8;
+      const unsigned off = r < vrows ? (unsigned)(r * ld + k) * 4u : OOB;
+      const auto a = __builtin_amdgcn_raw_buffer_load_b128(rs, off, 0, 0);
+      const auto b = __builtin_amdgcn_raw_buffer_load_b128(rs, off + 16u, 0, 0);
+#pragma unroll
+      for (int j = 0; j < 4; ++j) {
+        v[q][j] = __uint_as_float(a[j]);
+        v[q][4 + j] = __uint_as_float(b[j]);
+      }
+    } else {
+      const int rq = tid % (R / 4), k = kk + (tid / (R / 4)) * KPT;
+      const unsigned off = 4 * rq < vrows ? (unsigned)((k + q) * ld + 4 * rq) * 4u : OOB;
+      const auto a = __builtin_amdgcn_raw_buffer_load_b128(rs, off, 0, 0);
+#pragma unroll
+      for (int i = 0; i < 4; ++i) v[0][4 * q + i] = __uint_as_float(a[i]);
+    }
+  }
   static constexpr int NRD = MODE == LT ? 2 : 1;
 
   __device__ static __forceinline__ f16x8 frag(const char *plane, int rb, int s, int lane) {
@@ -281,6 +315,7 @@
 };
 
 
+template <int BN>
 __device__ __forceinline__ int tile_scales(const GemmF16Args &p, int *sexp, float *sw, int row0,
                                            int col0, int tid) {
   int skip = 0, spr = 0;
@@ -382,12 +417,14 @@
                [&](int, int, int row, int col, float v) { emit(p, row, col, v); });
 }
 
-template <bool A_KC, bool B_KC>
+template <bool A_KC, bool B_KC, int BN>
 __device__ __forceinline__ void tile_epilogue(const GemmF16Args &p, const int *sexp,
-                                              const float *sw, const f32x16 (&acc)[2][2],
-                                              int split, bool whole, int row0, int col0,
-                                              int flags, int tid, char *lds) {
-  const int lane = tid & 63, wave = tid >> 6, wm = wave >> 1, wn = wave & 1;
+                                              const float *sw,
+                                              const f32x16 (&acc)[Tile<BN>::MI][2], int split,
+                                              bool whole, int row0, int col0, int flags, int tid,
+                                              char *lds) {
+  constexpr int MI = Tile<BN>::MI, WR = Tile<BN>::WR, WN = Tile<BN>::WN;
+  const int lane = tid & 63, wave = tid >> 6, wm = wave / WN, wn = wave % WN;
   const int half2 = lane >> 5;
   const bool partial = p.ksplit > 1 && !whole;
   const bool skip = flags & 1;
@@ -395,13 +432,17 @@
   const int np4 = (p.N + 3) & ~3;
   float *slab = partial ? p.part + (int64_t)split * p.M * np4 : p.C;
   const int ldo = partial ? np4 : p.ldc;
-  uint64_t rej = 0;
+  uint64_t rej[MI / 2];
+#pragma unroll
+  for (int h = 0; h < MI / 2; ++h) rej[h] = 0;
   auto fix = [&]() {
-    fix_rejected(p, A_KC, B_KC, rej, lane, [&](int l, int n, int &row, int &col) {
-      const int i = n >> 5, j = (n >> 4) & 1, g = n & 15;
-      row = row0 + wm * 64 + i * 32 + (g & 3) + 8 * (g >> 2) + 4 * (l >> 5);
-      col = col0 + wn * 64 + j * 32 + (l & 31);
-    });
+#pragma unroll
+    for (int h = 0; h < MI / 2; ++h)
+      fix_rejected(p, A_KC, B_KC, rej[h], lane, [&](int l, int n, int &row, int &col) {
+        const int i = 2 * h + (n >> 5), j = (n >> 4) & 1, g = n & 15;
+        row = row0 + wm * WR + i * 32 + (g & 3) + 8 * (g >> 2) + 4 * (l >> 5);
+        col = col0 + wn * 64 + j * 32 + (l & 31);
+      });
   };
   const bool staged = row0 + BM <= p.M && col0 + BN <= p.N && !skip &&
                       (partial || p.mom.W || ((ldo & 3) | ((uintptr_t)slab & 15)) == 0);
@@ -410,34 +451,34 @@
     constexpr int SR = 68;
     float *st = reinterpret_cast<float *>(lds) + wave * 32 * SR;
 #pragma unroll
-    for (int i = 0; i < 2; ++i) {
+    for (int i = 0; i < MI; ++i) {
 #pragma unroll
       for (int j = 0; j < 2; ++j) {
         const int cl = wn * 64 + j * 32 + (lane & 31);
         const int ec = sexp[BM + cl];
         const float wc = check ? sw[BM + cl] : 0.0f;
         const bool bcheck =
-            check && (__ballot(wc > 0.0f || sw[wm * 64 + i * 32 + (lane & 31)] > 0.0f) != 0);
+            check && (__ballot(wc > 0.0f || sw[wm * WR + i * 32 + (lane & 31)] > 0.0f) != 0);
 #pragma unroll
         for (int g = 0; g < 16; ++g) {
           const int rr = (g & 3) + 8 * (g >> 2) + 4 * half2;
-          const int rl = wm * 64 + i * 32 + rr;
+          const int rl = wm * WR + i * 32 + rr;
           if (bcheck) {
             const float thr = wc + sw[rl];
             if (thr != 0.0f && !(fabsf(acc[i][j][g]) >= thr))
-              rej |= (uint64_t)1 << ((2 * i + j) * 16 + g);
+              rej[i >> 1] |= (uint64_t)1 << ((2 * (i & 1) + j) * 16 + g);
           }
           st[rr * SR + j * 32 + (lane & 31)] =
               __builtin_amdgcn_ldexpf(acc[i][j][g], -(sexp[rl] + ec));
         }
       }
       if (check) {
-        const uint64_t mine = (rej >> (32 * i)) & 0xffffffffull;
+        const uint64_t mine = (rej[i >> 1] >> (32 * (i & 1))) & 0xffffffffull;
         fix_rejected(
             p, A_KC, B_KC, mine, lane,
             [&](int l, int n, int &row, int &col) {
               const int j = (n >> 4) & 1, g = n & 15;
-              row = row0 + wm * 64 + i * 32 + (g & 3) + 8 * (g >> 2) + 4 * (l >> 5);
+              row = row0 + wm * WR + i * 32 + (g & 3) + 8 * (g >> 2) + 4 * (l >> 5);
               col = col0 + wn * 64 + j * 32 + (l & 31);
             },
             [&](int l, int n, int, int, float v) {
@@ -450,7 +491,7 @@
       for (int k = 0; k < 8; ++k) {
         const int f = lane + 64 * k, rr = f >> 4, c4 = f & 15;
         const float4 v = *reinterpret_cast<const float4 *>(st + rr * SR + 4 * c4);
-        const int row = row0 + wm * 64 + i * 32 + rr, col = col0 + wn * 64 + 4 * c4;
+        const int row = row0 + wm * WR + i * 32 + rr, col = col0 + wn * 64 + 4 * c4;
         if (!partial && p.mom.W) {
           float4 *wq = reinterpret_cast<float4 *>(p.mom.W + (int64_t)row * p.mom.ldw + col);
           float4 *pq = reinterpret_cast<float4 *>(p.mom.prev + (int64_t)row * p.mom.ldp + col);
@@ -487,7 +528,7 @@
     return;
   }
 #pragma unroll
-  for (int i = 0; i < 2; ++i)
+  for (int i = 0; i < MI; ++i)
 #pragma unroll
     for (int j = 0; j < 2; ++j) {
       const int cl = wn * 64 + j * 32 + (lane & 31);
@@ -496,17 +537,17 @@
       if (col >= p.N || ec == SKIP) continue;
       const float wc = check ? sw[BM + cl] : 0.0f;
       const bool bcheck =
-          check && (__ballot(wc > 0.0f || sw[wm * 64 + i * 32 + (lane & 31)] > 0.0f) != 0);
+          check && (__ballot(wc > 0.0f || sw[wm * WR + i * 32 + (lane & 31)] > 0.0f) != 0);
 #pragma unroll
       for (int g = 0; g < 16; ++g) {
-        const int rl = wm * 64 + i * 32 + (g & 3) + 8 * (g >> 2) + 4 * half2;
+        const int rl = wm * WR + i * 32 + (g & 3) + 8 * (g >> 2) + 4 * half2;
         const int row = row0 + rl;
         const int er = sexp[rl];
         if (row >= p.M || er == SKIP) continue;
         if (bcheck) {
           const float thr = wc + sw[rl];
           if (thr != 0.0f && !(fabsf(acc[i][j][g]) >= thr)) {
-            rej |= (uint64_t)1 << ((2 * i + j) * 16 + g);
+            rej[i >> 1] |= (uint64_t)1 << ((2 * (i & 1) + j) * 16 + g);
             continue;
           }
         }
@@ -536,6 +577,7 @@
 template <int AM, int BMODE, bool RAG>
 __global__ __launch_bounds__(NT, 1) void gemm_f16x3_kernel(GemmF16Args p) {
   constexpr bool A_KC = AM == LK, B_KC = BMODE == LK;
+  constexpr int BN = BN_NARROW, B_PLANE = Tile<BN>::B_PLANE, BUF = Tile<BN>::BUF;
   extern __shared__ __attribute__((aligned(16))) char lds[];
   int *sexp = reinterpret_cast<int *>(lds + 2 * BUF);
   float *sw = reinterpret_cast<float *>(sexp + BM + BN);
@@ -551,7 +593,7 @@
   const int T = kend > kbeg ? (kend - kbeg + BK - 1) / BK : 0;
   const int klast = kend - kbeg - (T - 1) * BK;
 
-  const int flags = tile_scales(p, sexp, sw, row0, col0, tid);
+  const int flags = tile_scales<BN>(p, sexp, sw, row0, col0, tid);
 
   const float *baseA = A_KC ? p.A + (int64_t)row0 * p.lda : p.A + (int64_t)kbeg * p.lda + row0;
   const float *baseB = B_KC ? p.B + (int64_t)col0 * p.ldb : p.B + (int64_t)kbeg * p.ldb + col0;
@@ -644,19 +686,20 @@
     }
   }
 
-  tile_epilogue<A_KC, B_KC>(p, sexp, sw, acc, split, whole, row0, col0, flags, tid, lds);
-}
-
-template <int AM, int BMODE, bool RAG>
+  tile_epilogue<A_KC, B_KC, BN>(p, sexp, sw, acc, split, whole, row0, col0, flags, tid, lds);
+}
+
+template <int AM, int BMODE, bool RAG, int BN = BN_NARROW>
 __global__ __launch_bounds__(NT, 1) void gemm_f16x3_fast_kernel(GemmF16Args p) {
   constexpr bool A_KC = AM == LK, B_KC = BMODE == LK;
+  constexpr int B_PLANE = Tile<BN>::B_PLANE, BUF = Tile<BN>::BUF, MI = Tile<BN>::MI;
   extern __shared__ __attribute__((aligned(16))) char lds[];
   int *sexp = reinterpret_cast<int *>(lds + 2 * BUF);
   float *sw = reinterpret_cast<float *>(sexp + BM + BN);
   const int tid = threadIdx.x;
   const float m1 = kcnn::f16x3::opaque_m1();
   const int lane = tid & 63, wave = __builtin_amdgcn_readfirstlane(tid >> 6);
-  const int wm = wave >> 1, wn = wave & 1;
+  const int wm = wave / Tile<BN>::WN, wn = wave % Tile<BN>::WN;
   int split, tm, tn;
   const bool whole = block_tile(p, split, tm, tn);
   const int row0 = tm * BM, col0 = tn * BN;
@@ -680,99 +723,180 @@
 
   using LA = Loader<BM, AM>;
   using LB = Loader<BN, BMODE>;
-  LA la[2];
-  LB lb[2];
-  f32x16 acc[2][2];
-#pragma unroll
-  for (int i = 0; i < 2; ++i)
+  f32x16 acc[MI][2];
+#pragma unroll
+  for (int i = 0; i < MI; ++i)
 #pragma unroll
     for (int j = 0; j < 2; ++j)
 #pragma unroll
       for (int g = 0; g < 16; ++g) acc[i][j][g] = 0.0f;
 
-  const int ar = wm * 64, br = wn * 64;
-  f16x8 fa0[2][2], fb0[2][2], fa1[2][2], fb1[2][2];
-  auto read_frag = [&](const char *buf, int s, int r, f16x8 (&fa)[2][2], f16x8 (&fb)[2][2]) {
-    if (r < 4) {
-      const int i = r >> 1, pl = r & 1;
-      fa[i][pl] = LA::frag(buf + pl * A_PLANE, ar + 32 * i, s, lane);
-    } else {
-      const int i = (r - 4) >> 1, pl = (r - 4) & 1;
-      fb[i][pl] = LB::frag(buf + 2 * A_PLANE + pl * B_PLANE, br + 32 * i, s, lane);
-    }
-  };
-  auto mfma_n = [&](int n, const f16x8 (&fa)[2][2], const f16x8 (&fb)[2][2]) {
-    const int i = n / 6, j = (n / 3) & 1, pr = n % 3;
-    constexpr int PA[3] = {1, 0, 0}, PB[3] = {0, 1, 0};
-    acc[i][j] = mfma(fa[i][PA[pr]], fb[j][PB[pr]], acc[i][j]);
-  };
-
+  const int ar = wm * Tile<BN>::WR, br = wn * 64;
   constexpr int PRIO = 1;
   if (PRIO && wave >= 4) __builtin_amdgcn_s_setprio(1);
-  if (T > 0) {
-    la[0].load(rsA, p.lda, vra, kk(0, A_KC), tid);
-    lb[0].load(rsB, p.ldb, vrb, kk(0, B_KC), tid);
-    la[1].load(rsA, p.lda, vra, kk(1, A_KC), tid);
-    lb[1].load(rsB, p.ldb, vrb, kk(1, B_KC), tid);
-  }
-  __builtin_amdgcn_sched_barrier(0);
-  const int flags = tile_scales(p, sexp, sw, row0, col0, tid);
-  la[0].init_exp(sexp, tid);
-  la[1].init_exp(sexp, tid);
-  lb[0].init_exp(sexp + BM, tid);
-  lb[1].init_exp(sexp + BM, tid);
-  if (T > 0) {
-    la[0].template store<A_PLANE, RAG>(lds, tid, T == 1 ? klast : BK, m1);
-    lb[0].template store<B_PLANE, RAG>(lds + 2 * A_PLANE, tid, T == 1 ? klast : BK, m1);
+  int flags = 0;
+  if constexpr (BN == BN_WIDE) {
+    LA la;
+    LB lb;
+    f16x8 fa[2][2], fb[2][2];
+    auto mfma_n = [&](int n) {
+      const int i = n / 6, j = (n / 3) & 1, pr = n % 3;
+      constexpr int PA[3] = {1, 0, 0}, PB[3] = {0, 1, 0};
+      acc[i][j] = mfma(fa[i & 1][PA[pr]], fb[j][PB[pr]], acc[i][j]);
+    };
+    auto reads_after = [&](int n, const char *buf, int s, const char *nb, int ns) {
+      constexpr int L = 6 * MI;
+      const int i = n / 6, r = (i + 1) % MI;
+      const char *src = i + 1 < MI ? buf : nb;
+      const int hs = i + 1 < MI ? s : ns;
+      if (n % 6 == 0) fa[r & 1][1] = LA::frag(src + A_PLANE, ar + 32 * r, hs, lane);
+      if (n % 6 == 1) fa[r & 1][0] = LA::frag(src, ar + 32 * r, hs, lane);
+      if (n == L - 5) fb[0][1] = LB::frag(nb + 2 * A_PLANE + B_PLANE, br, ns, lane);
+      if (n == L - 4) fb[0][0] = LB::frag(nb + 2 * A_PLANE, br, ns, lane);
+      if (n == L - 2) fb[1][1] = LB::frag(nb + 2 * A_PLANE + B_PLANE, br + 32, ns, lane);
+      if (n == L - 1) fb[1][0] = LB::frag(nb + 2 * A_PLANE, br + 32, ns, lane);
+    };
+    if (T > 0) {
+      la.load(rsA, p.lda, vra, kk(0, A_KC), tid);
+      lb.load(rsB, p.ldb, vrb, kk(0, B_KC), tid);
+    }
     __builtin_amdgcn_sched_barrier(0);
-    la[0].load(rsA, p.lda, vra, kk(2, A_KC), tid);
-    lb[0].load(rsB, p.ldb, vrb, kk(2, B_KC), tid);
-    __syncthreads();
-#pragma unroll
-    for (int r = 0; r < 8; ++r) read_frag(lds, 0, r, fa0, fb0);
-
-    auto step = [&](int t, LA &lan, LB &lbn, auto more_c) {
-      const char *buf = lds + (t & 1) * BUF;
-      char *nbuf = lds + ((t + 1) & 1) * BUF;
-      constexpr bool more = decltype(more_c)::value;
-      const int kv = t + 2 == T ? klast : BK;
-      uint32_t ph[4], pl[4];
-#pragma unroll
-      for (int n = 0; n < 12; ++n) {
-        mfma_n(n, fa0, fb0);
-        if (more) {
-          if (n < LA::NPIECE)
-            lan.template piece<A_PLANE, RAG>(nbuf, tid, n, kv, ph, pl, m1);
-          else if (n - LA::NPIECE < LB::NPIECE)
-            lbn.template piece<B_PLANE, RAG>(nbuf + 2 * A_PLANE, tid, n - LA::NPIECE, kv, ph, pl, m1);
-        }
-        if (n >= 2 && n < 10) read_frag(buf, 1, n - 2, fa1, fb1);
-        __builtin_amdgcn_sched_barrier(0);
-      }
+    flags = tile_scales<BN>(p, sexp, sw, row0, col0, tid);
+    la.init_exp(sexp, tid);
+    lb.init_exp(sexp + BM, tid);
+    if (T > 0) {
+      la.template store<A_PLANE, RAG>(lds, tid, T == 1 ? klast : BK, m1);
+      lb.template store<B_PLANE, RAG>(lds + 2 * A_PLANE, tid, T == 1 ? klast : BK, m1);
+      __builtin_amdgcn_sched_barrier(0);
+      la.load(rsA, p.lda, vra, kk(1, A_KC), tid);
+      lb.load(rsB, p.ldb, vrb, kk(1, B_KC), tid);
       __syncthreads();
 #pragma unroll
-      for (int n = 0; n < 12; ++n) {
-        mfma_n(n, fa1, fb1);
-        if (n == 1) lan.load(rsA, p.lda, vra, kk(t + 3, A_KC), tid);
-        if (n == 3) lbn.load(rsB, p.ldb, vrb, kk(t + 3, B_KC), tid);
-        if (more && n >= 2 && n < 10) read_frag(nbuf, 0, n - 2, fa0, fb0);
-        __builtin_amdgcn_sched_barrier(0);
+      for (int pl = 0; pl < 2; ++pl) fa[0][pl] = LA::frag(lds + pl * A_PLANE, ar, 0, lane);
+#pragma unroll
+      for (int j = 0; j < 2; ++j)
+#pragma unroll
+        for (int pl = 0; pl < 2; ++pl)
+          fb[j][pl] = LB::frag(lds + 2 * A_PLANE + pl * B_PLANE, br + 32 * j, 0, lane);
+
+      auto step = [&](int t) {
+        const char *buf = lds + (t & 1) * BUF;
+        char *nbuf = lds + ((t + 1) & 1) * BUF;
+        const int kv = t + 2 == T ? klast : BK;
+        uint32_t ph[4], pl[4];
+#pragma unroll
+        for (int n = 0; n < 6 * MI; ++n) {
+          mfma_n(n);
+          if (n < LA::NPIECE) {
+            la.template piece<A_PLANE, RAG>(nbuf, tid, n, kv, ph, pl, m1);
+            if ((n + 1) % LA::PPP == 0)
+              la.load_part(rsA, p.lda, vra, kk(t + 2, A_KC), tid, n / LA::PPP);
+          } else if (n - LA::NPIECE < LB::NPIECE) {
+            const int m = n - LA::NPIECE;
+            lb.template piece<B_PLANE, RAG>(nbuf + 2 * A_PLANE, tid, m, kv, ph, pl, m1);
+            if ((m + 1) % LB::PPP == 0)
+              lb.load_part(rsB, p.ldb, vrb, kk(t + 2, B_KC), tid, m / LB::PPP);
+          }
+          reads_after(n, buf, 0, buf, 1);
+          __builtin_amdgcn_sched_barrier(0);
+        }
+        __syncthreads();
+#pragma unroll
+        for (int n = 0; n < 6 * MI; ++n) {
+          mfma_n(n);
+          reads_after(n, buf, 1, nbuf, 0);
+          __builtin_amdgcn_sched_barrier(0);
+        }
+        __syncthreads();
+      };
+      static_assert(LA::NPIECE + LB::NPIECE <= 6 * MI, "a piece per MFMA of phase A");
+#pragma unroll 1
+      for (int t = 0; t < T; ++t) step(t);
+    }
+  } else {
+    LA la[2];
+    LB lb[2];
+    f16x8 fa0[2][2], fb0[2][2], fa1[2][2], fb1[2][2];
+    auto read_frag = [&](const char *buf, int s, int r, f16x8 (&fa)[2][2], f16x8 (&fb)[2][2]) {
+      if (r < 4) {
+        const int i = r >> 1, pl = r & 1;
+        fa[i][pl] = LA::frag(buf + pl * A_PLANE, ar + 32 * i, s, lane);
+      } else {
+        const int i = (r - 4) >> 1, pl = (r - 4) & 1;
+        fb[i][pl] = LB::frag(buf + 2 * A_PLANE + pl * B_PLANE, br + 32 * i, s, lane);
       }
     };
-    int t = 0;
-    for (; t + 2 < T; t += 2) {
-      step(t, la[1], lb[1], std::true_type{});
-      step(t + 1, la[0], lb[0], std::true_type{});
-    }
-    if (t + 1 < T) {
-      step(t, la[1], lb[1], std::true_type{});
-      step(t + 1, la[0], lb[0], std::false_type{});
-    } else {
-      step(t, la[1], lb[1], std::false_type{});
-    }
-  }
-
-  tile_epilogue<A_KC, B_KC>(p, sexp, sw, acc, split, whole, row0, col0, flags, tid, lds);
+    auto mfma_n = [&](int n, const f16x8 (&fa)[2][2], const f16x8 (&fb)[2][2]) {
+      const int i = n / 6, j = (n / 3) & 1, pr = n % 3;
+      constexpr int PA[3] = {1, 0, 0}, PB[3] = {0, 1, 0};
+      acc[i][j] = mfma(fa[i][PA[pr]], fb[j][PB[pr]], acc[i][j]);
+    };
+
+    if (T > 0) {
+      la[0].load(rsA, p.lda, vra, kk(0, A_KC), tid);
+      lb[0].load(rsB, p.ldb, vrb, kk(0, B_KC), tid);
+      la[1].load(rsA, p.lda, vra, kk(1, A_KC), tid);
+      lb[1].load(rsB, p.ldb, vrb, kk(1, B_KC), tid);
+    }
+    __builtin_amdgcn_sched_barrier(0);
+    flags = tile_scales<BN>(p, sexp, sw, row0, col0, tid);
+    la[0].init_exp(sexp, tid);
+    la[1].init_exp(sexp, tid);
+    lb[0].init_exp(sexp + BM, tid);
+    lb[1].init_exp(sexp + BM, tid);
+    if (T > 0) {
+      la[0].template store<A_PLANE, RAG>(lds, tid, T == 1 ? klast : BK, m1);
+      lb[0].template store<B_PLANE, RAG>(lds + 2 * A_PLANE, tid, T == 1 ? klast : BK, m1);
+      __builtin_amdgcn_sched_barrier(0);
+      la[0].load(rsA, p.lda, vra, kk(2, A_KC), tid);
+      lb[0].load(rsB, p.ldb, vrb, kk(2, B_KC), tid);
+      __syncthreads();
+#pragma unroll
+      for (int r = 0; r < 8; ++r) read_frag(lds, 0, r, fa0, fb0);
+
+      auto step = [&](int t, LA &lan, LB &lbn, auto more_c) {
+        const char *buf = lds + (t & 1) * BUF;
+        char *nbuf = lds + ((t + 1) & 1) * BUF;
+        constexpr bool more = decltype(more_c)::value;
+        const int kv = t + 2 == T ? klast : BK;
+        uint32_t ph[4], pl[4];
+#pragma unroll
+        for (int n = 0; n < 12; ++n) {
+          mfma_n(n, fa0, fb0);
+          if (more) {
+            if (n < LA::NPIECE)
+              lan.template piece<A_PLANE, RAG>(nbuf, tid, n, kv, ph, pl, m1);
+            else if (n - LA::NPIECE < LB::NPIECE)
+              lbn.template piece<B_PLANE, RAG>(nbuf + 2 * A_PLANE, tid, n - LA::NPIECE, kv, ph, pl, m1);
+          }
+          if (n >= 2 && n < 10) read_frag(buf, 1, n - 2, fa1, fb1);
+          __builtin_amdgcn_sched_barrier(0);
+        }
+        __syncthreads();
+#pragma unroll
+        for (int n = 0; n < 12; ++n) {
+          mfma_n(n, fa1, fb1);
+          if (n == 1) lan.load(rsA, p.lda, vra, kk(t + 3, A_KC), tid);
+          if (n == 3) lbn.load(rsB, p.ldb, vrb, kk(t + 3, B_KC), tid);
+          if (more && n >= 2 && n < 10) read_frag(nbuf, 0, n - 2, fa0, fb0);
+          __builtin_amdgcn_sched_barrier(0);
+        }
+      };
+      int t = 0;
+      for (; t + 2 < T; t += 2) {
+        step(t, la[1], lb[1], std::true_type{});
+        step(t + 1, la[0], lb[0], std::true_type{});
+      }
+      if (t + 1 < T) {
+        step(t, la[1], lb[1], std::true_type{});
+        step(t + 1, la[0], lb[0], std::false_type{});
+      } else {
+        step(t, la[1], lb[1], std::false_type{});
+      }
+    }
+  }
+
+  tile_epilogue<A_KC, B_KC, BN>(p, sexp, sw, acc, split, whole, row0, col0, flags, tid, lds);
 }
 
 struct StatOp {
@@ -1345,35 +1469,60 @@
   }
 }
 
-int choose_ksplit(int64_t tiles, int M, int N, int K, int *nwhole = nullptr) {
-  auto round = [](int k) { return 0.0458 * k + 11.1; };
-  int best = 1, best_w = 0;
-  double best_t = (double)((tiles + 255) / 256) * round(K);
+struct GemmPlan {
+  int bn, ksplit, nwhole;
+  double us;
+};
+constexpr double NARROW_A = 0.0458, NARROW_B = 11.1;
+constexpr double WIDE_A = 0.0793, WIDE_B = 21.4;
+GemmPlan plan_tile(int bn, int M, int N, int K) {
+  const int64_t tiles = (int64_t)((M + BM - 1) / BM) * ((N + bn - 1) / bn);
+  const double ca = bn == BN_WIDE ? WIDE_A : NARROW_A, cb = bn == BN_WIDE ? WIDE_B : NARROW_B;
+  auto round = [&](int k) { return ca * k + cb; };
+  GemmPlan best{bn, 1, 0, (double)((tiles + 255) / 256) * round(K)};
   for (int s = 2; s <= 4 && K / s >= 1024; ++s) {
     const int ks = (K + s - 1) / s;
     for (int64_t w = 0; w < tiles; w += 256) {
       const int64_t rest = tiles - w;
       const double t = (double)(w / 256) * round(K) + (double)((rest * s + 255) / 256) * round(ks) +
                        (double)(s + 1) * M * N * 4.0 / 4.0e6 * (double)rest / (double)tiles;
-      if (t < best_t) { best_t = t; best = s; best_w = (int)w; }
-    }
-  }
-  if (nwhole) *nwhole = best > 1 ? best_w : 0;
+      if (t < best.us) best = GemmPlan{bn, s, (int)w, t};
+    }
+  }
   return best;
 }
-
+GemmPlan choose_plan(int M, int N, int K, bool wide_ok, int family) {
+  const GemmPlan narrow = plan_tile(BN_NARROW, M, N, K);
+  if (!wide_ok || family == 4) return narrow;
+  const GemmPlan wide = plan_tile(BN_WIDE, M, N, K);
+  if (family == 3) return wide;
+  return wide.us < narrow.us ? wide : narrow;
+}
+int loader_mode(bool kc, const void *ptr, int ld) {
+  if (kc) return (int)LK;
+  return ld % 4 == 0 && (uintptr_t)ptr % 16 == 0 ? (int)LT : (int)LR;
+}
+std::atomic<unsigned long long> g_tile_calls[2];
+
+template <int AM, int BMODE, bool RAG, int BN>
+void launch_fast(const GemmF16Args &a, unsigned blocks, hipStream_t st) {
+  constexpr int LDS_BYTES = Tile<BN>::LDS_BYTES;
+  static bool attr = [] {
+    return hipFuncSetAttribute(
+               reinterpret_cast<const void *>(&gemm_f16x3_fast_kernel<AM, BMODE, RAG, BN>),
+               hipFuncAttributeMaxDynamicSharedMemorySize, LDS_BYTES) == hipSuccess;
+  }();
+  (void)attr;
+  hipLaunchKernelGGL((gemm_f16x3_fast_kernel<AM, BMODE, RAG, BN>), dim3(blocks), dim3(NT),
+                     LDS_BYTES, st, a);
+}
 template <int AM, int BMODE, bool RAG>
 void launch_t(const GemmF16Args &a, unsigned blocks, hipStream_t st) {
   if constexpr (AM != LR && BMODE != LR) {
-    static bool attr = [] {
-      return hipFuncSetAttribute(
-                 reinterpret_cast<const void *>(&gemm_f16x3_fast_kernel<AM, BMODE, RAG>),
-                 hipFuncAttributeMaxDynamicSharedMemorySize, LDS_BYTES) == hipSuccess;
-    }();
-    (void)attr;
-    hipLaunchKernelGGL((gemm_f16x3_fast_kernel<AM, BMODE, RAG>), dim3(blocks), dim3(NT),
-                       LDS_BYTES, st, a);
+    if (a.bn == BN_WIDE) launch_fast<AM, BMODE, RAG, BN_WIDE>(a, blocks, st);
+    else launch_fast<AM, BMODE, RAG, BN_NARROW>(a, blocks, st);
   } else {
+    constexpr int LDS_BYTES = Tile<BN_NARROW>::LDS_BYTES;
     static bool attr = [] {
       return hipFuncSetAttribute(
                  reinterpret_cast<const void *>(&gemm_f16x3_kernel<AM, BMODE, RAG>),
@@ -1409,8 +1558,7 @@
   return align16(sizeof(uint32_t) * (((size_t)M * ((N + 3) / 4) + 63) / 64 + 1));
 }
 size_t partial_bytes(int M, int N, int K) {
-  const int64_t tiles = (int64_t)((M + BM - 1) / BM) * ((N + BN - 1) / BN);
-  const int s = choose_ksplit(tiles, M, N, K);
+  const int s = std::max(plan_tile(BN_NARROW, M, N, K).ksplit, plan_tile(BN_WIDE, M, N, K).ksplit);
   return s > 1 ? slab_bytes(s, M, N) + flag_bytes(M, N) : 0;
 }
 
@@ -1482,6 +1630,23 @@
 
 extern "C" size_t kl_gemm_f16x3_workspace_bytes(int M, int N, int K) {
   return partial_bytes(M, N, K);
+}
+extern "C" void kl_gemm_f16x3_tile_counts(unsigned long long *out, int reset) {
+  for (int i = 0; i < 2; ++i) {
+    out[i] = g_tile_calls[i].load(std::memory_order_relaxed);
+    if (reset) g_tile_calls[i].store(0, std::memory_order_relaxed);
+  }
+}
+extern "C" size_t kl_gemm_f16x3_plan(int transA, int transB, int M, int N, int K, int lda,
+                                     int ldb, int *out) {
+  out[0] = out[1] = out[2] = 0;
+  if (M <= 0 || N <= 0 || K <= 0) return 0;
+  const int am = loader_mode(!transA, nullptr, lda), bm = loader_mode(transB != 0, nullptr, ldb);
+  const GemmPlan plan = choose_plan(M, N, K, am != LR && bm != LR, kcnn::family(kcnn::kFamGemm));
+  out[0] = plan.bn;
+  out[1] = plan.ksplit;
+  out[2] = plan.ksplit > 1 ? plan.nwhole : 0;
+  return plan.ksplit > 1 ? slab_bytes(plan.ksplit, M, N) + flag_bytes(M, N) : 0;
 }
 constexpr int FIX_SITES = 256;
 struct FixSites {
@@ -1542,11 +1707,16 @@
   a.bvec = N % 4 == 0 && (uintptr_t)a.bmax % 16 == 0 && (uintptr_t)a.bcnt % 16 == 0;
   a.M = M; a.N = N; a.K = K; a.lda = lda; a.ldb = ldb; a.ldc = ldc;
   a.alpha = alpha; a.beta = beta;
+  const int am = loader_mode(a_kc, A, lda), bm = loader_mode(b_kc, B, ldb);
+  const GemmPlan plan =
+      choose_plan(M, N, K, am != LR && bm != LR, kcnn::family(kcnn::kFamGemm));
+  const int BN = plan.bn;
+  a.bn = BN;
   a.tiles_m = (M + BM - 1) / BM;
   a.tiles_n = (N + BN - 1) / BN;
   const int64_t tiles = (int64_t)a.tiles_m * a.tiles_n;
-  int nwhole = 0;
-  int s = choose_ksplit(tiles, M, N, K, &nwhole);
+  int nwhole = plan.nwhole;
+  int s = plan.ksplit;
   const size_t need = s > 1 ? slab_bytes(s, M, N) + flag_bytes(M, N) : 0;
   if (need > ws_bytes || !ws) s = 1;
   if (s > 1) {
@@ -1567,10 +1737,6 @@
   a.nwhole = nwhole;
   const int64_t nb = nwhole + (tiles - nwhole) * s;
   if (nb >= ((int64_t)1 << 31)) return (int)hipErrorNotSupported;
-  auto mode = [](bool kc, const float *ptr, int ld) {
-    if (kc) return (int)LK;
-    return ld % 4 == 0 && (uintptr_t)ptr % 16 == 0 ? (int)LT : (int)LR;
-  };
   bool fix_launch = true;
   if (s > 1) {
     uint32_t *dev = nullptr;
@@ -1582,8 +1748,9 @@
       a.fix_local = fix_launch ? 0 : 1;
     }
   }
-  launch(mode(a_kc, A, lda), mode(b_kc, B, ldb), a, (unsigned)nb, st);
+  launch(am, bm, a, (unsigned)nb, st);
   int rc = kcnn::launch_status();
+  if (!rc) g_tile_calls[BN == BN_WIDE ? 1 : 0].fetch_add(1, std::memory_order_relaxed);
   if (rc || s == 1) return rc;
   hipLaunchKernelGGL(gemm_f16x3_reduce_kernel, dim3(kcnn::grid_for((int64_t)M * ((N + 3) / 4))),
                      dim3(256), 0, st, a, a_kc ? 1 : 0, b_kc ? 1 : 0);
diff --git a/kaldi-cnn_amd/src/kaldi-lite/cu-kernels-lite.h b/kaldi-cnn_amd/src/kaldi-lite/cu-kernels-lite.h
--- a/kaldi-cnn_amd/src/kaldi-lite/cu-kernels-lite.h
+++ b/kaldi-cnn_amd/src/kaldi-lite/cu-kernels-lite.h
@@ -39,6 +39,9 @@
                    int ld2, int mode2, uint32_t *out2, uint32_t *part2, void *pool_cols,
                    kcnn_stream_t stream);
 size_t kl_gemm_f16x3_workspace_bytes(int M, int N, int K);
+void kl_gemm_f16x3_tile_counts(unsigned long long *out, int reset);
+size_t kl_gemm_f16x3_plan(int transA, int transB, int M, int N, int K, int lda, int ldb,
+                          int *out);
 int kl_gemm_f16x3_st(int transA, int transB, int M, int N, int K, float alpha,
                      const float *A, int lda, const float *B, int ldb, float beta, float *C,
                      int ldc, const uint32_t *amax, const uint32_t *bmax, void *ws,
diff --git a/kaldi-cnn_amd/src/kaldi-lite/cu-matrix.cc b/kaldi-cnn_amd/src/kaldi-lite/cu-matrix.cc
--- a/kaldi-cnn_amd/src/kaldi-lite/cu-matrix.cc
+++ b/kaldi-cnn_amd/src/kaldi-lite/cu-matrix.cc
@@ -284,7 +284,7 @@
                                          const CuMatrixBase<float> *in) {
   CuDevice &dev = CuDevice::Instantiate();
   const int N = dy.NumRows(), O = dy.NumCols(), I = W.NumCols();
-  if (dev.GemmMode() != 2 || N == 0 || O == 0 || I == 0 || W.NumRows() != O) return;
+  if (dev.GemmMode() < 2 || N == 0 || O == 0 || I == 0 || W.NumRows() != O) return;
   {
     const CuGemmStatsHint *hd = CuGemmStatsHint::Find(dy.Data(), N, O, dy.Stride());
     const CuGemmStatsHint *hw = CuGemmStatsHint::Find(W.Data(), O, I, W.Stride());
@@ -353,7 +353,7 @@
   auto aligned = [](const CuMatrixBase<Real> &X) {
     return X.Stride() % 4 == 0 && reinterpret_cast<uintptr_t>(X.Data()) % 16 == 0;
   };
-  if (dev0.GemmMode() != 2 || m == 0 || n == 0 || k == 0 || !aligned(A) || !aligned(B) ||
+  if (dev0.GemmMode() < 2 || m == 0 || n == 0 || k == 0 || !aligned(A) || !aligned(B) ||
       !aligned(*this) || !aligned(*prev))
     return false;
   KALDI_ASSERT((transA == kNoTrans ? A.NumRows() : A.NumCols()) == m &&
@@ -390,7 +390,7 @@
   auto aligned = [](const CuMatrixBase<Real> &X) {
     return X.Stride() % 4 == 0 && reinterpret_cast<uintptr_t>(X.Data()) % 16 == 0;
   };
-  if (dev0.GemmMode() == 2 && num_rows_ > 0 && num_cols_ > 0 && k > 0 && aligned(A) &&
+  if (dev0.GemmMode() >= 2 && num_rows_ > 0 && num_cols_ > 0 && k > 0 && aligned(A) &&
       aligned(B)) {
     KALDI_ASSERT((transA == kNoTrans ? A.NumRows() : A.NumCols()) == num_rows_ &&
                  (transB == kNoTrans ? B.NumCols() : B.NumRows()) == num_cols_ &&
@@ -423,9 +423,9 @@
     };
     CuMatrix<Real> Acopy, Bcopy;
     const CuMatrixBase<Real> *Ap = &A, *Bp = &B;
-    if ((transA == kNoTrans || mode == 2) && !aligned(A)) { Acopy = A; Ap = &Acopy; }
-    if ((transB == kTrans || mode == 2) && !aligned(B)) { Bcopy = B; Bp = &Bcopy; }
-    if (mode == 2 && GemmF16x3(alpha, A, *Ap, transA, B, *Bp, transB, beta, nullptr)) return;
+    if ((transA == kNoTrans || mode >= 2) && !aligned(A)) { Acopy = A; Ap = &Acopy; }
+    if ((transB == kTrans || mode >= 2) && !aligned(B)) { Bcopy = B; Bp = &Bcopy; }
+    if (mode >= 2 && GemmF16x3(alpha, A, *Ap, transA, B, *Bp, transB, beta, nullptr)) return;
     const size_t wsb = kl_gemm_x6_workspace_bytes(m, n, k);
     void *ws = wsb ? dev0.Malloc(wsb) : nullptr;
     const int rc = kl_gemm_x6(transA == kTrans, transB == kTrans, m, n, k, alpha,
diff --git a/kaldi-cnn_amd/src/kaldi-lite/kcnn-knobs.cc b/kaldi-cnn_amd/src/kaldi-lite/kcnn-knobs.cc
--- a/kaldi-cnn_amd/src/kaldi-lite/kcnn-knobs.cc
+++ b/kaldi-cnn_amd/src/kaldi-lite/kcnn-knobs.cc
@@ -17,7 +17,7 @@
     {"bwd_x6", "KCNN_BWD_X6", 1, 1},
     {"igemm_x6", "KCNN_IGEMM_X6", 2, 3},
     {"wgrad_x6", "KCNN_WGRAD_X6", 2, 3},
-    {"gemm", "KCNN_GEMM", 2, 2},
+    {"gemm", "KCNN_GEMM", 2, 4},
 };
 
 int from_env(const FamilyInfo &f) {
```
